# AIM-SE/AC-TSR

Measured on AMD Instinct MI355X. Metric: user-sequences/sec fwd+bwd, AC-SASRec L=50 d=64, 1/2/4/8 MI355X, higher is better.
Workload: dtype f32; 1 GPU; ACSASRec full training step (spatial + adversarial calibrators, BASELINE configs[2]), synthetic 100000-item catalogue, B=512/GPU L=50 d=64 h=2 2 layers inner=256, CE loss, two-pass backward + Adam; global_batch=512, seq_len=50, hidden=64, heads=2, parallelism=dp1, launch=hipGraph replay per step, backward=two walks (reference protocol, trainer.py:672-686)

## Files before the change

### ac_tsr_amd/_lib.py

```python
from __future__ import annotations

import ctypes as C
import os
import subprocess

_HERE = os.path.dirname(os.path.abspath(__file__))
CSRC = os.path.join(_HERE, "csrc")
LIB_PATH = os.environ.get("ACATTN_LIB") or os.path.join(CSRC, "libacattn.so")
HEADER_PATH = os.path.join(os.path.dirname(_HERE), "include", "acattn.h")

ABI_VERSION = 32
MAX_MASKS = 8
NSTAT = 8
MASK_STRUCTURED, MASK_DENSE_LL, MASK_DENSE_L = 0, 1, 2
COMBINE = {"fixed": 0, "gate": 1, "annealing": 2}
RICH = {"none": 0, "fixed": 1, "trainable": 2}
RNG_EXPLICIT, RNG_COUNTER = 0, 1
FWD_AUTO, FWD_STREAM, FWD_STAGED, FWD_GENERAL = 0, 1, 2, 3
BWD_AUTO, BWD_STREAM, BWD_ROW = 0, 1, 2

_f = C.c_void_p


class Problem(C.Structure):
    _fields_ = [
        ("B", C.c_int32), ("L", C.c_int32), ("H", C.c_int32), ("n_heads", C.c_int32),
        ("q", _f), ("k", _f), ("v", _f), ("qa", _f), ("ka", _f), ("gate_logits", _f),
        ("mask_mode", C.c_int32), ("causal", C.c_int32), ("key_valid", _f), ("mask", _f),
        ("w_order", _f), ("b_order", _f), ("w_dist", _f), ("b_dist", _f), ("scalar", _f),
        ("adversarial", C.c_int32), ("combine_option", C.c_int32), ("anneal_rate", C.c_float),
        ("two_level", C.c_int32), ("rich_combine", C.c_int32), ("rich_ratio", _f),
        ("rng_mode", C.c_int32), ("p_drop", C.c_float), ("noise", _f), ("keep_after", _f), ("keep_before", _f),
        ("keep_mask", _f), ("seed", C.c_uint64), ("seed_device", _f), ("affine", _f), ("gate_is_prob", C.c_int32),
    ]


class FwdOut(C.Structure):
    _fields_ = [
        ("ctx_attacked", _f), ("ctx_calibrated", _f), ("attack_mask", _f), ("row_stats", _f),
        ("after_spatial", _f), ("before_spatial", _f), ("perturbed_attention", _f), ("calibrated_attention", _f),
        ("penalty_part", _f),
    ]


class BwdIO(C.Structure):
    _fields_ = [
        ("attack_mask", _f), ("row_stats", _f),
        ("d_ctx_attacked", _f), ("d_ctx_calibrated", _f), ("d_attack_mask", _f),
        ("dq", _f), ("dk", _f), ("dv", _f), ("dqa", _f), ("dka", _f), ("dgate_logits", _f),
        ("dw_order_part", _f), ("dw_dist_part", _f), ("dsmall_part", _f), ("part_stride", C.c_int32),
        ("active_qblocks", _f), ("attack_only", C.c_int32), ("workspace", _f), ("read_rows", _f),
        ("n_read_rows", C.c_int32), ("d_penalty_part", _f), ("dgate_summed", C.c_int32),
        ("d_ctx_calibrated2", _f), ("d_penalty_part2", _f), ("dqa2", _f), ("dka2", _f),
    ]


class SpatialBwdIO(C.Structure):
    _fields_ = [
        ("d_ctx", _f), ("dq", _f), ("dk", _f), ("dv", _f),
        ("dw_order_part", _f), ("dw_dist_part", _f), ("dsmall_part", _f), ("part_stride", C.c_int32),
        ("n_read_rows", C.c_int32), ("read_rows", _f), ("workspace", _f),
    ]


class CeProblem(C.Structure):
    _fields_ = [("B", C.c_int32), ("N", C.c_int32), ("H", C.c_int32), ("out", _f), ("table", _f), ("target", _f),
                ("coef_is_scalar", C.c_int32), ("coef_scale", C.c_float)]


class LnProblem(C.Structure):
    _fields_ = [("rows", C.c_int32), ("H", C.c_int32), ("residual_rows", C.c_int32), ("z", _f), ("residual", _f),
                ("gamma", _f), ("beta", _f), ("eps", C.c_float), ("p_drop", C.c_float), ("keep", _f),
                ("seed", C.c_uint64), ("seed_device", _f)]


LN_BWD_GRID = 512


class ProjProblem(C.Structure):
    _fields_ = [("rows", C.c_int32), ("H", C.c_int32), ("G", C.c_int32), ("x", _f), ("wq", _f), ("bq", _f), ("wk", _f),
                ("bk", _f), ("wv", _f), ("bv", _f), ("waq", _f), ("baq", _f), ("wak", _f), ("bak", _f), ("wg", _f),
                ("bg", _f), ("w_order", _f), ("b_order", _f), ("w_dist", _f), ("b_dist", _f), ("n_heads", C.c_int32),
                ("L", C.c_int32)]


class ProjOut(C.Structure):
    _fields_ = [("mq", _f), ("mk", _f), ("mv", _f), ("qa", _f), ("ka", _f), ("gate", _f), ("affine", _f),
                ("gate_prob", C.c_int32)]


class ProjBwdIO(C.Structure):
    _fields_ = [("dmq", _f), ("dmk", _f), ("dmv", _f), ("dqa", _f), ("dka", _f), ("dgate", _f), ("dmq_total", _f),
                ("dmk_total", _f), ("dx", _f), ("dx_init", _f), ("workspace", _f)]


ADAM_MAX_TENSORS = 64


class AdamGroup(C.Structure):
    _fields_ = [("n_tensors", C.c_int32), ("param", _f * ADAM_MAX_TENSORS), ("grad", _f * ADAM_MAX_TENSORS),
                ("exp_avg", _f * ADAM_MAX_TENSORS), ("exp_avg_sq", _f * ADAM_MAX_TENSORS), ("step", _f * ADAM_MAX_TENSORS),
                ("numel", C.c_int64 * ADAM_MAX_TENSORS)]


class TailProblem(C.Structure):
    _fields_ = [("rows", C.c_int32), ("H", C.c_int32), ("I", C.c_int32), ("ctx", _f), ("x", _f), ("wd", _f), ("bd", _f),
                ("g1", _f), ("b1", _f), ("w1", _f), ("bb1", _f), ("w2", _f), ("bb2", _f), ("g2", _f), ("b2", _f),
                ("eps1", C.c_float), ("eps2", C.c_float), ("p1", C.c_float), ("p2", C.c_float), ("keep1", _f),
                ("keep2", _f), ("seed1", C.c_uint64), ("seed2", C.c_uint64), ("seed_device", _f), ("src_index", _f),
                ("src_R", C.c_int32), ("src_L", C.c_int32), ("split_planes", _f)]


class TailSaved(C.Structure):
    _fields_ = [("h1", _f), ("st1", _f), ("a", _f), ("act", _f), ("h3", _f), ("st2", _f), ("out", _f),
                ("gelu_grad", _f)]


class TailBwdIO(C.Structure):
    _fields_ = [("d_out", _f), ("d_ctx", _f), ("d_x", _f), ("d_h1", _f), ("d_h2", _f), ("d_h3", _f), ("dgb_part", _f),
                ("workspace", _f)]


class EmbedProblem(C.Structure):
    _fields_ = [("rows", C.c_int32), ("L", C.c_int32), ("H", C.c_int32), ("n_table_rows", C.c_int64), ("idx", _f),
                ("table", _f), ("pos", _f), ("gamma", _f), ("beta", _f), ("eps", C.c_float), ("p_drop", C.c_float),
                ("keep", _f), ("seed", C.c_uint64), ("seed_device", _f), ("nonzero_out", _f), ("hot_id_plus1", C.c_int64)]


EMBED_BWD_CHUNKS = 8
PENALTY_WS_FLOATS = 1024
WGRAD_MAX_GROUP = 8
WGRAD_MAX_REDUCE = 32
SUMROWS_MAX_DEFER = 8

SYMBOLS = {
    "acattn_abi_version": (C.c_int, []),
    "acattn_calibrated_attention_bwd_gate_summed": (C.c_int, [C.POINTER(Problem), C.POINTER(BwdIO)]),
    "acattn_calibrated_attention_bwd_pair_supported": (C.c_int, [C.POINTER(Problem), C.POINTER(BwdIO)]),
    "acattn_last_error": (C.c_char_p, []),
    "acattn_fwd_algorithmic_bytes": (C.c_int64, [C.POINTER(Problem)]),
    "acattn_calibrated_attention_fwd": (C.c_int, [C.POINTER(Problem), C.POINTER(FwdOut), C.c_void_p]),
    "acattn_calibrated_attention_bwd": (C.c_int, [C.POINTER(Problem), C.POINTER(BwdIO), C.c_void_p]),
    "acattn_spatial_attention_bwd": (C.c_int, [C.POINTER(Problem), C.POINTER(SpatialBwdIO), C.c_void_p]),
    "acattn_spatial_attention_bwd_workspace_bytes": (C.c_int64, [C.POINTER(Problem)]),
    "acattn_spatial_affines": (C.c_int, [C.POINTER(Problem), _f, C.c_void_p]),
    "acattn_full_sort_ce_workspace_bytes": (C.c_int64, [C.POINTER(CeProblem)]),
    "acattn_full_sort_ce_fwd": (C.c_int, [C.POINTER(CeProblem), _f, _f, _f, C.c_void_p]),
    "acattn_full_sort_ce_fwd_dir": (C.c_int, [C.POINTER(CeProblem), _f, _f, _f, _f, C.c_void_p]),
    "acattn_full_sort_ce_bwd": (C.c_int, [C.POINTER(CeProblem), _f, _f, _f, _f, _f, C.c_void_p]),
    "acattn_full_sort_ce_products": (C.c_int, [C.c_int]),
    "acattn_linear_products": (C.c_int, [C.c_int]),
    "acattn_dropout_add_layernorm_fwd": (C.c_int, [C.POINTER(LnProblem), _f, _f, C.c_void_p]),
    "acattn_dropout_add_layernorm_bwd": (C.c_int, [C.POINTER(LnProblem), _f, _f, _f, _f, _f, C.c_void_p]),
    "acattn_embed_layernorm_fwd": (C.c_int, [C.POINTER(EmbedProblem), _f, _f, C.c_void_p]),
    "acattn_embed_layernorm_bwd": (C.c_int, [C.POINTER(EmbedProblem), _f, _f, C.c_int64, _f, _f, _f, C.c_void_p]),
    "acattn_projections_supported": (C.c_int, [C.c_int32, C.c_int32]),
    "acattn_projections_bwd_workspace_bytes": (C.c_int64, [C.POINTER(ProjProblem)]),
    "acattn_projections_fwd": (C.c_int, [C.POINTER(ProjProblem), C.POINTER(ProjOut), C.c_void_p]),
    "acattn_projections_qkv_supported": (C.c_int, [C.c_int32]),
    "acattn_projections_qkv_fwd": (C.c_int, [C.POINTER(ProjProblem), C.POINTER(ProjOut), C.c_void_p]),
    "acattn_projections_bwd": (C.c_int, [C.POINTER(ProjProblem), C.POINTER(ProjBwdIO), C.c_void_p]),
    "acattn_layer_tail_supported": (C.c_int, [C.c_int32, C.c_int32]),
    "acattn_layer_tail_fwd": (C.c_int, [C.POINTER(TailProblem), C.POINTER(TailSaved), C.c_void_p]),
    "acattn_layer_tail_bwd": (C.c_int, [C.POINTER(TailProblem), C.POINTER(TailSaved), C.POINTER(TailBwdIO), C.c_void_p]),
    "acattn_layer_tail_bwd_partial_rows": (C.c_int32, [C.c_int32]),
    "acattn_layer_tail_bwd_partial_rows_for": (C.c_int32, [C.c_int32, C.c_int32]),
    "acattn_layer_tail_bwd_workspace_bytes": (C.c_int64, [C.c_int32, C.c_int32]),
    "acattn_select_layer_tail_blocks": (C.c_int, [C.c_int]),
    "acattn_layer_tail_split_bytes": (C.c_int64, [C.c_int32, C.c_int32, C.c_int32]),
    "acattn_layer_tail_split_weights": (C.c_int, [C.POINTER(TailProblem), C.c_void_p, C.c_void_p]),
    "acattn_adam_step": (C.c_int, [C.POINTER(AdamGroup), C.c_double, C.c_double, C.c_double, C.c_double, C.c_double, _f,
                                   C.c_void_p]),
    "acattn_dense_ce_fwd": (C.c_int, [_f, C.c_int64, C.c_int64, _f, _f, _f, C.c_void_p]),
    "acattn_dense_ce_bwd": (C.c_int, [_f, _f, _f, _f, C.c_int64, C.c_int64, _f, C.c_void_p]),
    "acattn_step_inputs": (C.c_int, [C.POINTER(C.c_void_p), C.POINTER(C.c_void_p), C.POINTER(C.c_int64), C.c_int32, C.c_void_p,
                                     C.c_void_p, C.c_void_p, C.c_int32, C.c_void_p]),
    "acattn_sum_rows": (C.c_int, [_f, _f, C.c_int32, C.c_int32, C.c_int32, C.c_void_p]),
    "acattn_sum_rows_pair": (C.c_int, [_f, _f, C.c_int32, C.c_int32, C.c_int32, _f, _f, C.c_int32, C.c_int32, C.c_int32, C.c_void_p]),
    "acattn_mask_penalty_fwd": (C.c_int, [_f, C.c_int64, _f, _f, C.c_void_p]),
    "acattn_mask_penalty_partial": (C.c_int, [_f, C.c_int64, _f, C.c_void_p]),
    "acattn_mask_penalty_partial_multi": (C.c_int, [C.c_void_p, C.c_int32, C.c_int64, _f, C.c_void_p]),
    "acattn_mask_penalty_bwd_scaled_multi": (C.c_int, [C.c_void_p, _f, _f, C.c_float, C.c_int64, C.c_void_p, C.c_int32,
                                                       C.c_void_p]),
    "acattn_attacked_loss_finish": (C.c_int, [_f, C.c_int32, _f, C.c_int32, C.c_int64, C.c_float, _f, _f, C.c_int32,
                                              C.c_void_p]),
    "acattn_mask_penalty_rows": (C.c_int, [_f, C.c_int32, C.c_int32, C.c_int32, _f, C.c_void_p]),
    "acattn_attacked_loss_finish_rows": (C.c_int, [_f, C.c_int32, C.c_void_p, C.c_int32, C.c_int32, C.c_float, _f, _f, C.c_int32,
                                                  C.c_void_p]),
    "acattn_mask_penalty_drows": (C.c_int, [_f, _f, C.c_float, C.c_int32, C.c_void_p, C.c_int32, C.c_void_p]),
    "acattn_mask_penalty_drows_dir": (C.c_int, [_f, _f, C.c_float, C.c_int32, C.c_void_p, C.c_int32, _f, _f, C.c_int32, C.c_void_p]),
    "acattn_mask_penalty_bwd_scaled": (C.c_int, [_f, _f, _f, C.c_float, C.c_int64, _f, C.c_void_p]),
    "acattn_mask_penalty_bwd": (C.c_int, [_f, _f, _f, C.c_int64, _f, C.c_void_p]),
    "acattn_linear_wgrad_workspace_bytes": (C.c_int64, [C.c_int64, C.c_int32, C.c_int32]),
    "acattn_linear_wgrad_grouped": (C.c_int, [C.c_void_p, C.c_void_p, C.c_void_p, C.c_void_p, C.c_void_p, C.c_void_p,
                                               C.c_int32, C.c_int64, _f, C.c_void_p]),
    "acattn_linear_wgrad": (C.c_int, [_f, _f, C.c_int64, C.c_int32, C.c_int32, _f, _f, _f, C.c_void_p]),
    "acattn_linear_wgrad_grouped_partial": (C.c_int, [C.c_void_p, C.c_void_p, C.c_void_p, C.c_void_p, C.c_void_p, C.c_int32,
                                                       C.c_int64, C.c_void_p, C.c_void_p, C.c_void_p, C.c_void_p, C.c_void_p]),
    "acattn_linear_wgrad_reduce_many": (C.c_int, [C.c_void_p, C.c_void_p, C.c_void_p, C.c_void_p, C.c_void_p, C.c_void_p,
                                                   C.c_void_p, C.c_int32, C.c_void_p, C.c_void_p, C.c_void_p, C.c_void_p,
                                                   C.c_int32, C.c_void_p]),
    "acattn_select_forward_kernel": (C.c_int, [C.c_int]),
    "acattn_select_backward_kernel": (C.c_int, [C.c_int]),
    "acattn_calibrated_attention_bwd_workspace_bytes": (C.c_int64, [C.POINTER(Problem)]),
    "acattn_rng_materialize": (C.c_int, [C.c_int32, C.c_int32, C.c_int32, C.c_uint64, C.c_float, _f, _f, _f, _f,
                                         C.c_void_p]),
}

_lib = None


class AcattnError(RuntimeError):
    pass


def build(verbose: bool = False) -> str:
    jobs = str(min(8, os.cpu_count() or 1))
    res = subprocess.run(["make", "-C", CSRC, "-j", jobs], capture_output=not verbose, text=True)
    if res.returncode != 0:
        raise AcattnError("building libacattn.so failed:\n" + (res.stdout or "") + (res.stderr or ""))
    return LIB_PATH


def load() -> C.CDLL:
    global _lib
    if _lib is not None:
        return _lib
    if not os.path.exists(LIB_PATH):
        raise AcattnError(
            f"{LIB_PATH} is missing: the HIP extension has not been built. Run "
            "`make -C ac_tsr_amd/csrc` (or __graft_entry__.build()). There is no CPU / eager fallback.")
    lib = C.CDLL(LIB_PATH)
    for name, (res, args) in SYMBOLS.items():
        fn = getattr(lib, name)
        fn.restype = res
        fn.argtypes = args
    got = lib.acattn_abi_version()
    if got != ABI_VERSION:
        raise AcattnError(f"libacattn.so ABI {got} != binding ABI {ABI_VERSION}; rebuild")
    _lib = lib
    return lib


def check(rc: int, what: str) -> None:
    if rc == 0:
        return
    msg = load().acattn_last_error().decode()
    if rc < 0 and "not a multiple of the number of attention" in msg:
        raise ValueError(msg)
    if rc < 0 and ("unknown combine_option" in msg or "unknown rich_calibrated_combine" in msg):
        raise KeyError(msg)
    raise AcattnError(f"{what} failed (rc={rc}): {msg}")
```

### ac_tsr_amd/csrc/acattn_api.hip

```cpp
#include <stdint.h>
#include <stdio.h>
#include <string.h>

#include <algorithm>

#include "acattn_common.h"

namespace {
thread_local char g_err[256] = "";

int fail(const char* msg) {
  snprintf(g_err, sizeof(g_err), "%s", msg);
  return -1;
}

int check_problem(const acattn_problem* p) {
  if (!p) return fail("problem is NULL");
  if (p->B < 1 || p->L < 1 || p->H < 1 || p->n_heads < 1) return fail("B, L, H, n_heads must be positive");
  if (p->H % p->n_heads != 0)
    return fail("The hidden size is not a multiple of the number of attention heads");
  const int dh = p->H / p->n_heads;
  if (dh != 16 && dh != 32 && dh != 64 && dh != 128) return fail("unsupported head size: dh must be 16, 32, 64 or 128");
  if (p->L > 208) return fail("unsupported sequence length: L must be <= 208");
  if (!p->q || !p->k || !p->v) return fail("q, k, v must be non-NULL");
// ... 133 lines not shown
                                   (hipStream_t)stream);
  if (rc > 0) snprintf(g_err, sizeof(g_err), "HIP launch failed: %s", hipGetErrorString((hipError_t)rc));
  return rc;
}

static int check_ce(const acattn_ce_problem* p) {
  if (!p) return fail("ce problem is NULL");
  if (p->B < 1 || p->N < 1) return fail("B and N must be positive");
  if (p->H != 64 && p->H != 128 && p->H != 256) return fail("unsupported hidden size for the fused cross-entropy: H must be 64, 128 or 256");
  if (!p->out || !p->table || !p->target) return fail("out, table, target must be non-NULL");
  return 0;
}

int64_t acattn_full_sort_ce_workspace_bytes(const acattn_ce_problem* p) {
  if (!p || (p->H != 64 && p->H != 128 && p->H != 256)) return -1;
  return acattn_ce_ws_bytes(*p);
}

int acattn_full_sort_ce_fwd(const acattn_ce_problem* p, void* workspace, float* lse, float* row_loss, void* stream) {
  if (int rc = check_ce(p)) return rc;
  if (!workspace || !lse || !row_loss) return fail("workspace, lse, row_loss must be non-NULL");
  const int rc = acattn_launch_ce_fwd(*p, workspace, lse, row_loss, (hipStream_t)stream);
  if (rc > 0) snprintf(g_err, sizeof(g_err), "HIP launch failed: %s", hipGetErrorString((hipError_t)rc));
  return rc;
}

int acattn_full_sort_ce_fwd_dir(const acattn_ce_problem* p, void* workspace, float* lse, float* row_loss, float* dir,
                                void* stream) {
  if (int rc = check_ce(p)) return rc;
  if (!workspace || !lse || !row_loss || !dir) return fail("workspace, lse, row_loss, dir must be non-NULL");
  const int rc = acattn_launch_ce_fwd_dir(*p, workspace, lse, row_loss, dir, (hipStream_t)stream);
  if (rc > 0) snprintf(g_err, sizeof(g_err), "HIP launch failed: %s", hipGetErrorString((hipError_t)rc));
  return rc;
}

int acattn_full_sort_ce_bwd(const acattn_ce_problem* p, const float* lse, const float* coef, void* workspace,
                            float* d_out, float* d_table, void* stream) {
  if (int rc = check_ce(p)) return rc;
  if (!workspace || !lse || !coef || !d_out) return fail("workspace, lse, coef, d_out must be non-NULL");
  const int rc = acattn_launch_ce_bwd(*p, lse, coef, workspace, d_out, d_table, (hipStream_t)stream);
  if (rc > 0) snprintf(g_err, sizeof(g_err), "HIP launch failed: %s", hipGetErrorString((hipError_t)rc));
  return rc;
}

int acattn_full_sort_ce_products(int mode) { return acattn_ce_products_choice(mode); }

int acattn_linear_products(int mode) { return acattn_linear_products_choice(mode); }

static int check_ln(const acattn_ln_problem* p) {
  if (!p) return fail("ln problem is NULL");
  if (p->rows < 1) return fail("rows must be positive");
  if (p->H != 64 && p->H != 128 && p->H != 256) return fail("unsupported hidden size for the fused LayerNorm: H must be 64, 128 or 256");
  if (p->residual_rows < 1 || p->rows % p->residual_rows != 0) return fail("residual_rows must divide rows");
  if (!p->z || !p->residual || !p->gamma || !p->beta) return fail("z, residual, gamma, beta must be non-NULL");
  if (p->p_drop < 0.f || p->p_drop >= 1.f) return fail("p_drop must lie in [0, 1)");
  return 0;
}

int acattn_dropout_add_layernorm_fwd(const acattn_ln_problem* p, float* y, float* stats, void* stream) {
  if (int rc = check_ln(p)) return rc;
  if (!y || !stats) return fail("y and stats must be non-NULL");
  const int rc = acattn_launch_ln_fwd(*p, y, stats, (hipStream_t)stream);
  if (rc > 0) snprintf(g_err, sizeof(g_err), "HIP launch failed: %s", hipGetErrorString((hipError_t)rc));
  return rc;
}

int acattn_dropout_add_layernorm_bwd(const acattn_ln_problem* p, const float* dy, const float* stats, float* dz,
                                     float* dres, float* dgb_part, void* stream) {
  if (int rc = check_ln(p)) return rc;
  if (!dy || !stats) return fail("dy and stats must be non-NULL");
  const int rc = acattn_launch_ln_bwd(*p, dy, stats, dz, dres, dgb_part, (hipStream_t)stream);
  if (rc > 0) snprintf(g_err, sizeof(g_err), "HIP launch failed: %s", hipGetErrorString((hipError_t)rc));
  return rc;
}

static int check_proj(const acattn_proj_problem* p) {
  if (!p) return fail("problem must be non-NULL");
  if (p->rows < 1) return fail("rows must be positive");
  if (!acattn_proj_supported(p->H, p->G)) return fail("projections: hidden_size must be 64, 128 or 256 and the gate at most 256 wide");
  if (!p->x || !p->wq || !p->bq || !p->wk || !p->bk || !p->wv || !p->bv || !p->waq || !p->baq || !p->wak || !p->bak)
    return fail("projections: input and parameters must be non-NULL");
  if ((p->wg != nullptr) != (p->bg != nullptr) || (p->wg != nullptr) != (p->G > 0))
    return fail("projections: gate weight, bias and width go together");
  return 0;
}

int acattn_projections_supported(int32_t H, int32_t G) { return acattn_proj_supported(H, G) ? 1 : 0; }

int64_t acattn_projections_bwd_workspace_bytes(const acattn_proj_problem* p) {
  if (!p || !acattn_proj_supported(p->H, p->G)) return -1;
  return acattn_proj_bwd_ws_bytes(*p);
}

int acattn_projections_fwd(const acattn_proj_problem* p, const acattn_proj_out* out, void* stream) {
  if (int rc = check_proj(p)) return rc;
  if (!out || !out->mq || !out->mk || !out->mv || !out->qa || !out->ka) return fail("projections: outputs must be non-NULL");
  if ((p->wg != nullptr) != (out->gate != nullptr)) return fail("projections: gate output goes with the gate parameters");
  if (out->affine) {
    if (!p->w_order || !p->b_order || !p->w_dist || !p->b_dist) return fail("projections: affine planes need the spatial calibrator's parameters");
    if (p->n_heads < 1 || p->H % p->n_heads != 0 || (p->H / p->n_heads) % 16 != 0) return fail("projections: affine planes need a head size that is a multiple of 16");
    if (p->L < 1 || p->rows % p->L != 0) return fail("projections: affine planes need rows = B * L");
  }
  const int rc = acattn_launch_proj_fwd(*p, *out, (hipStream_t)stream);
  if (rc > 0) snprintf(g_err, sizeof(g_err), "HIP launch failed: %s", hipGetErrorString((hipError_t)rc));
  return rc;
}

int acattn_projections_qkv_supported(int32_t H) { return acattn_proj_qkv_supported(H) ? 1 : 0; }

int acattn_projections_qkv_fwd(const acattn_proj_problem* p, const acattn_proj_out* out, void* stream) {
  if (!p) return fail("problem must be non-NULL");
  if (p->rows < 1) return fail("rows must be positive");
  if (!acattn_proj_qkv_supported(p->H)) return fail("projections (q, k, v only): hidden_size must be 64 with the split products on");
  if (!p->x || !p->wq || !p->bq || !p->wk || !p->bk || !p->wv || !p->bv) return fail("projections: input and parameters must be non-NULL");
  if (!out || !out->mq || !out->mk || !out->mv) return fail("projections: outputs must be non-NULL");
  if (out->qa || out->ka || out->gate) return fail("projections (q, k, v only): qa, ka and gate outputs must be NULL");
  if (out->affine) {
    if (!p->w_order || !p->b_order || !p->w_dist || !p->b_dist) return fail("projections: affine planes need the spatial calibrator's parameters");
    if (p->n_heads < 1 || p->H % p->n_heads != 0 || (p->H / p->n_heads) % 16 != 0) return fail("projections: affine planes need a head size that is a multiple of 16");
    if (p->L < 1 || p->rows % p->L != 0) return fail("projections: affine planes need rows = B * L");
  }
  const int rc = acattn_launch_proj_qkv_fwd(*p, *out, (hipStream_t)stream);
  if (rc > 0) snprintf(g_err, sizeof(g_err), "HIP launch failed: %s", hipGetErrorString((hipError_t)rc));
  return rc;
}

int acattn_projections_bwd(const acattn_proj_problem* p, const acattn_proj_bwd_io* io, void* stream) {
  if (int rc = check_proj(p)) return rc;
  if (!io) return fail("io must be non-NULL");
  if (!io->dmq_total && !io->dmk_total && !io->dx) return fail("projections backward: nothing to compute");
  const int rc = acattn_launch_proj_bwd(*p, *io, (hipStream_t)stream);
  if (rc > 0) snprintf(g_err, sizeof(g_err), "HIP launch failed: %s", hipGetErrorString((hipError_t)rc));
  return rc;
}

static int check_tail(const acattn_tail_problem* p, const acattn_tail_saved* s) {
  if (!p || !s) return fail("problem and saved must be non-NULL");
  if (p->rows < 1) return fail("rows must be positive");
  if (!acattn_tail_supported(p->H, p->I)) return fail("layer tail: (hidden_size, inner_size) must be (64, 256), (64, 128), (128, 512), (128, 256) or (256, 1024)");
  if (!p->ctx || !p->x || !p->wd || !p->bd || !p->g1 || !p->b1 || !p->w1 || !p->bb1 || !p->w2 || !p->bb2 || !p->g2 || !p->b2)
    return fail("layer tail: inputs and parameters must be non-NULL");
  if (!(p->p1 >= 0.f && p->p1 < 1.f) || !(p->p2 >= 0.f && p->p2 < 1.f)) return fail("dropout probabilities must be in [0, 1)");
  if (!s->h1 || !s->st1 || !s->a || !s->h3 || !s->st2) return fail("layer tail: saved tensors must be non-NULL");
  if (p->src_index && (p->src_R < 1 || p->src_L < 1)) return fail("layer tail: src_index needs src_R, src_L >= 1");
  if (p->split_planes && p->H != 64) return fail("layer tail: split_planes is for hidden 64 only");
  if (((uintptr_t)p->split_planes & 15) != 0) return fail("layer tail: split_planes must be 16-byte aligned");
  return 0;
}

int acattn_layer_tail_supported(int32_t H, int32_t I) { return acattn_tail_supported(H, I) ? 1 : 0; }

int32_t acattn_layer_tail_bwd_partial_rows(int32_t rows) { return acattn_tail_bwd_partial_rows(rows); }
int32_t acattn_layer_tail_bwd_partial_rows_for(int32_t rows, int32_t H) { return acattn_tail_bwd_partial_rows_h(rows, H); }
int64_t acattn_layer_tail_bwd_workspace_bytes(int32_t H, int32_t I) {
  return acattn_tail_supported(H, I) ? acattn_tail_bwd_ws_bytes(H, I) : -1;
}

int64_t acattn_layer_tail_split_bytes(int32_t H, int32_t I, int32_t rows) {
  return acattn_tail_supported(H, I) && rows > 0 ? acattn_tail_split_bytes(H, I, rows) : 0;
}

int acattn_layer_tail_split_weights(const acattn_tail_problem* p, void* planes, void* stream) {
  if (!p || !planes || !p->wd || !p->w1 || !p->w2) return fail("layer tail split planes: problem, weights and planes must be non-NULL");
  if (p->H != 64 || (p->I != 256 && p->I != 128)) return fail("layer tail split planes: hidden 64, inner 256 or 128 only");
  if (((uintptr_t)planes & 15) != 0) return fail("layer tail split planes: planes must be 16-byte aligned");
  const int rc = acattn_launch_tail_split(*p, planes, (hipStream_t)stream);
  if (rc > 0) snprintf(g_err, sizeof(g_err), "HIP launch failed: %s", hipGetErrorString((hipError_t)rc));
  return rc;
}

int acattn_select_layer_tail_blocks(int nb) {
  if (nb < 0 || nb > 2) return fail("rows per wave: 0 (automatic), 1 or 2 blocks of 16");
  return acattn_select_tail_nb(nb);
}

int acattn_layer_tail_fwd(const acattn_tail_problem* p, const acattn_tail_saved* saved, void* stream) {
  if (int rc = check_tail(p, saved)) return rc;
  if (!saved->act || !saved->out) return fail("layer tail forward: act and out must be non-NULL");
  const int rc = acattn_launch_tail_fwd(*p, *saved, (hipStream_t)stream);
  if (rc > 0) snprintf(g_err, sizeof(g_err), "HIP launch failed: %s", hipGetErrorString((hipError_t)rc));
  return rc;
}

int acattn_layer_tail_bwd(const acattn_tail_problem* p, const acattn_tail_saved* saved, const acattn_tail_bwd_io* io,
                          void* stream) {
  if (int rc = check_tail(p, saved)) return rc;
  if (!io || !io->d_out) return fail("layer tail backward: d_out must be non-NULL");
  const int rc = acattn_launch_tail_bwd(*p, *saved, *io, (hipStream_t)stream);
  if (rc > 0) snprintf(g_err, sizeof(g_err), "HIP launch failed: %s", hipGetErrorString((hipError_t)rc));
  return rc;
}

int acattn_dense_ce_fwd(const float* logits, int64_t rows, int64_t N, const int64_t* target, float* lse, float* row_loss,
                        void* stream) {
  if (!logits || !target || !lse || !row_loss) return fail("dense CE: logits, target, lse, row_loss must be non-NULL");
  if (rows < 1 || N < 1) return fail("dense CE: rows and N must be positive");
  const int rc = acattn_launch_dense_ce_fwd(logits, rows, N, target, lse, row_loss, (hipStream_t)stream);
  if (rc > 0) snprintf(g_err, sizeof(g_err), "HIP launch failed: %s", hipGetErrorString((hipError_t)rc));
  return rc;
}
int acattn_dense_ce_bwd(const float* logits, const float* lse, const int64_t* target, const float* coef, int64_t rows, int64_t N,
                        float* d_logits, void* stream) {
  if (!logits || !lse || !target || !coef || !d_logits) return fail("dense CE backward: every pointer must be non-NULL");
  if (rows < 1 || N < 1) return fail("dense CE: rows and N must be positive");
  const int rc = acattn_launch_dense_ce_bwd(logits, lse, target, coef, rows, N, d_logits, (hipStream_t)stream);
  if (rc > 0) snprintf(g_err, sizeof(g_err), "HIP launch failed: %s", hipGetErrorString((hipError_t)rc));
  return rc;
}

int acattn_step_inputs(const void* const* src, void* const* dst, const int64_t* bytes, int32_t n_copies, int64_t* counter,
                       const int64_t* item_length, int64_t* last_row, int32_t n_rows, void* stream) {
  if (n_copies < 0 || n_copies > ACATTN_MAX_COPIES) return fail("step inputs: 0 .. ACATTN_MAX_COPIES copies");
  if (n_copies > 0 && (!src || !dst || !bytes)) return fail("step inputs: src, dst, bytes must be non-NULL");
  for (int k = 0; k < n_copies; ++k)
    if (bytes[k] > 0 && (!src[k] || !dst[k])) return fail("step inputs: NULL copy operand");
  if ((item_length == nullptr) != (last_row == nullptr)) return fail("step inputs: item_length and last_row come together");
  if (last_row && n_rows < 1) return fail("step inputs: n_rows must be positive");
  const int rc = acattn_launch_step_inputs(src, dst, bytes, n_copies, counter, item_length, last_row, n_rows, (hipStream_t)stream);
  if (rc > 0) snprintf(g_err, sizeof(g_err), "HIP launch failed: %s", hipGetErrorString((hipError_t)rc));
  return rc;
}

int acattn_sum_rows(const float* x, float* out, int32_t batch, int32_t R, int32_t C, void* stream) {
  if (!x || !out) return fail("x and out must be non-NULL");
  if (batch < 1 || R < 1 || C < 1) return fail("batch, R, C must be positive");
  const int rc = acattn_launch_sum_rows(x, out, batch, R, C, (hipStream_t)stream);
  if (rc > 0) snprintf(g_err, sizeof(g_err), "HIP launch failed: %s", hipGetErrorString((hipError_t)rc));
  return rc;
}

int acattn_sum_rows_pair(const float* x1, float* out1, int32_t batch1, int32_t R1, int32_t C1, const float* x2, float* out2,
                         int32_t batch2, int32_t R2, int32_t C2, void* stream) {
  if (!x1 || !out1 || !x2 || !out2) return fail("x and out must be non-NULL");
  if (batch1 < 1 || R1 < 1 || C1 < 1 || batch2 < 1 || R2 < 1 || C2 < 1) return fail("batch, R, C must be positive");
  const int rc = acattn_launch_sum_rows_pair(x1, out1, batch1, R1, C1, x2, out2, batch2, R2, C2, (hipStream_t)stream);
  if (rc > 0) snprintf(g_err, sizeof(g_err), "HIP launch failed: %s", hipGetErrorString((hipError_t)rc));
  return rc;
}

static int check_embed(const acattn_embed_problem* p) {
  if (!p) return fail("embed problem is NULL");
  if (p->rows < 1 || p->L < 1 || p->rows % p->L != 0) return fail("rows must be a positive multiple of L");
  if (p->H != 64 && p->H != 128 && p->H != 256) return fail("unsupported hidden size for the fused embedding front end: H must be 64, 128 or 256");
  if (p->n_table_rows < 1) return fail("n_table_rows must be positive");
  if (!p->idx || !p->table || !p->gamma || !p->beta) return fail("idx, table, gamma, beta must be non-NULL");
  if (p->p_drop < 0.f || p->p_drop >= 1.f) return fail("p_drop must lie in [0, 1)");
  return 0;
}

int acattn_embed_layernorm_fwd(const acattn_embed_problem* p, float* y, float* stats, void* stream) {
  if (const int rc = check_embed(p)) return rc;
  if (!y || !stats) return fail("y and stats must be non-NULL");
  const int rc = acattn_launch_embed_fwd(*p, y, stats, (hipStream_t)stream);
  if (rc > 0) snprintf(g_err, sizeof(g_err), "HIP launch failed: %s", hipGetErrorString((hipError_t)rc));
  return rc;
}

int acattn_embed_layernorm_bwd(const acattn_embed_problem* p, const float* dy, const float* stats, int64_t padding_idx,
                               float* d_table, float* d_pos_part, float* dgb_part, void* stream) {
  if (const int rc = check_embed(p)) return rc;
  if (!dy || !stats) return fail("dy and stats must be non-NULL");
  const int rc = acattn_launch_embed_bwd(*p, dy, stats, padding_idx, d_table, d_pos_part, dgb_part, (hipStream_t)stream);
  if (rc > 0) snprintf(g_err, sizeof(g_err), "HIP launch failed: %s", hipGetErrorString((hipError_t)rc));
  return rc;
}

int acattn_mask_penalty_fwd(const float* m, int64_t n, float* workspace, float* norm, void* stream) {
  if (!m || !workspace || !norm) return fail("m, workspace and norm must be non-NULL");
  if (n < 1) return fail("n must be positive");
  if (((uintptr_t)m & 15) != 0) return fail("m must be 16-byte aligned");
  const int rc = acattn_launch_penalty_fwd(m, n, workspace, norm, (hipStream_t)stream);
  if (rc > 0) snprintf(g_err, sizeof(g_err), "HIP launch failed: %s", hipGetErrorString((hipError_t)rc));
  return rc;
}

int acattn_mask_penalty_bwd(const float* m, const float* norm, const float* d_norm, int64_t n, float* d_m, void* stream) {
  if (!m || !norm || !d_norm || !d_m) return fail("m, norm, d_norm and d_m must be non-NULL");
  if (n < 1) return fail("n must be positive");
  if ((((uintptr_t)m | (uintptr_t)d_m) & 15) != 0) return fail("m and d_m must be 16-byte aligned");
  const int rc = acattn_launch_penalty_bwd(m, norm, d_norm, n, d_m, (hipStream_t)stream);
  if (rc > 0) snprintf(g_err, sizeof(g_err), "HIP launch failed: %s", hipGetErrorString((hipError_t)rc));
  return rc;
}

int acattn_mask_penalty_partial(const float* m, int64_t n, float* part, void* stream) {
  if (!m || !part) return fail("m and part must be non-NULL");
  if (n < 1) return fail("n must be positive");
  if (((uintptr_t)m & 15) != 0) return fail("m must be 16-byte aligned");
  const int rc = acattn_launch_penalty_partial(m, n, part, (hipStream_t)stream);
  if (rc > 0) snprintf(g_err, sizeof(g_err), "HIP launch failed: %s", hipGetErrorString((hipError_t)rc));
  return rc;
}

int acattn_attacked_loss_finish(const float* row_loss, int32_t B, const float* part, int32_t n_masks, int64_t mask_numel,
                                float weight, float* out, float* scale_buf, int32_t n_scale, void* stream) {
  if (!row_loss || !part || !out) return fail("row_loss, part and out must be non-NULL");
  if (B < 1 || n_masks < 1 || mask_numel < 1) return fail("B, n_masks and mask_numel must be positive");
  if (n_scale < 0 || (n_scale > 0 && !scale_buf)) return fail("scale_buf must be given with n_scale > 0");
  const int rc = acattn_launch_attacked_loss_finish(row_loss, B, part, n_masks, mask_numel, weight, out, scale_buf, n_scale,
                                                    (hipStream_t)stream);
  if (rc > 0) snprintf(g_err, sizeof(g_err), "HIP launch failed: %s", hipGetErrorString((hipError_t)rc));
  return rc;
}

int acattn_mask_penalty_rows(const float* m, int32_t B, int32_t n_heads, int32_t L, float* pen, void* stream) {
  if (!m || !pen) return fail("m and pen must be non-NULL");
// ... 172 lines not shown
```

### ac_tsr_amd/csrc/acattn_bwd_stream.hip

```cpp
#include <stdlib.h>

#include <algorithm>

#include "acattn_common.h"

namespace {

constexpr float kLog2e = 1.44269504088896340736f;
constexpr float kLn2 = 0.69314718055994530942f;

__device__ __forceinline__ float ex2(float x) { return __builtin_amdgcn_exp2f(x); }
__device__ __forceinline__ float and_bits(float x, int m) { return __uint_as_float(__float_as_uint(x) & (uint32_t)m); }
__device__ __forceinline__ float hsum(const f4 v) { return (v[0] + v[1]) + (v[2] + v[3]); }
__device__ __forceinline__ float row16_sum(float v) {
  v += __builtin_bit_cast(float, __builtin_amdgcn_update_dpp(0, __builtin_bit_cast(int, v), 0xB1, 0xF, 0xF, false));
  v += __builtin_bit_cast(float, __builtin_amdgcn_update_dpp(0, __builtin_bit_cast(int, v), 0x4E, 0xF, 0xF, false));
  v += __builtin_bit_cast(float, __builtin_amdgcn_update_dpp(0, __builtin_bit_cast(int, v), 0x141, 0xF, 0xF, false));
  v += __builtin_bit_cast(float, __builtin_amdgcn_update_dpp(0, __builtin_bit_cast(int, v), 0x140, 0xF, 0xF, false));
  return v;
}

#ifndef ACATTN_BWD_ONE_WAVE_DH
#define ACATTN_BWD_ONE_WAVE_DH 64
#endif
// ... 692 lines not shown
      load_mask_row<DH>(P, IO, F, rowbase, bh, hoff, qb, c, g, R);
      float qac[4][DT];
      col_frag<DH>(P.qa, rowbase, H, hoff, i0, L, c, g, qac);
      const float sM = ws[(bh * L + (R.row_ok ? R.i : 0)) * NSC + 4];
      const uint32_t prow = prow_base + (uint32_t)(R.row_ok ? R.i : 0) * (uint32_t)L;
      const int j0 = 16 * t + 4 * g;
      f4 aM = {0.f, 0.f, 0.f, 0.f};
#pragma unroll
      for (int s4 = 0; s4 < KS / 4; ++s4)
#pragma unroll
        for (int e = 0; e < 4; ++e) aM = mfma16(ka4[s4][e], R.qaf[4 * s4 + e], aM);
      uint32_t eb4, ab4;
      tile_bits(F, t, g, R.i, L, causal, R.row_ok, R.dead, eb4, ab4);
      const f4 dMext = IO.d_attack_mask ? load_seg(IO.d_attack_mask + prow, j0, L, R.row_ok) : f4{0.f, 0.f, 0.f, 0.f};
      const float dpen2 = IO.d_penalty_part ? 2.0f * IO.d_penalty_part[(size_t)bh * nT + qb] : 0.f;
      f4 Mt, dM;
      mask_tile(R, K, aM, t, g, eb4, dMext, dpen2, Mt, dM);
      const f4 dSa = (Mt * (dM - sM)) * K.inv_sqrt;
      asm volatile("s_waitcnt lgkmcnt(0)" ::: "memory");
      *(f4*)(&tr[1][c * TS + 4 * g]) = dSa;
      asm volatile("s_waitcnt lgkmcnt(0)" ::: "memory");
#pragma unroll
      for (int s = 0; s < 4; ++s) {
        const float b_sa = tr[1][(4 * g + s) * TS + c];
#pragma unroll
        for (int dt = 0; dt < DT; ++dt) aKa[dt] = mfma16(qac[s][dt], b_sa, aKa[dt]);
      }
      continue;
    }
#endif
    Row<DH> R;
    load_row<DH>(P, IO, F, rowbase, bh, hoff, qb, c, g, R);
    const bool order_select = !causal || __ballot(R.dead) != 0ull;
    const float* wrow = ws + (bh * L + (R.row_ok ? R.i : 0)) * NSC;
    const f4 w0 = *(const f4*)wrow;
    const float sM = wrow[4];
    const uint32_t prow = prow_base + (uint32_t)(R.row_ok ? R.i : 0) * (uint32_t)L;
    const int j0 = 16 * t + 4 * g;
    const f4 gl = load_seg(P.gate_logits + (rowbase + (R.row_ok ? R.i : 0)) * L, j0, L, R.row_ok);
    f4 dMout = IO.d_attack_mask ? load_seg(IO.d_attack_mask + prow, j0, L, R.row_ok) : f4{0.f, 0.f, 0.f, 0.f};
    uint32_t eb4, ab4;
    tile_bits(F, t, g, R.i, L, causal, R.row_ok, R.dead, eb4, ab4);
    Tile T;
    tile_forward<DH, DCA, TWO>(R, K, k4, ka4, v4, co4, cd4, gl, t, g, eb4, ab4, order_select, T);
    if (IO.d_penalty_part) dMout += (T.M - 1.0f) * (2.0f * IO.d_penalty_part[(size_t)bh * nT + qb]);
    f4 dS, dSa, dgl, d_o, d_d;
    float dsc;
    tile_backward<DCA>(T, K, w0[0], w0[1], w0[2], w0[3], sM, dMout, R.i, j0, dS, dSa, dgl, d_o, d_d, dsc);
    dco += d_o;
    dcd += d_d;
    asm volatile("s_waitcnt lgkmcnt(0)" ::: "memory");
    *(f4*)(&tr[0][c * TS + 4 * g]) = dS;
    *(f4*)(&tr[1][c * TS + 4 * g]) = dSa;
    if constexpr (DCA) *(f4*)(&tr[2][c * TS + 4 * g]) = T.Ap;
    if constexpr (TWO && !DCA) {
      const float dpen2_2 = IO.d_penalty_part2 ? 2.0f * IO.d_penalty_part2[(size_t)bh * nT + qb] : 0.f;
      *(f4*)(&tr[2][c * TS + 4 * g]) = second_set_dsa(T, K, wrow[5], wrow[6], wrow[7], (T.M - 1.0f) * dpen2_2);
    }
    *(f4*)(&tr[3][c * TS + 4 * g]) = T.Aw;
    float qc[4][DT], qac[4][DT], gac[4][DT], gcc[4][DT];
    if (full) col_frag<DH>(P.q, rowbase, H, hoff, i0, L, c, g, qc);
    col_frag<DH>(P.qa, rowbase, H, hoff, i0, L, c, g, qac);
    if constexpr (DCA)
      if (full) col_frag<DH>(IO.d_ctx_attacked, rowbase, H, hoff, i0, L, c, g, gac);
    if (full) col_frag<DH>(IO.d_ctx_calibrated, rowbase, H, hoff, i0, L, c, g, gcc);
    asm volatile("s_waitcnt lgkmcnt(0)" ::: "memory");
#pragma unroll
    for (int s = 0; s < 4; ++s) {
      const float b_s = tr[0][(4 * g + s) * TS + c], b_sa = tr[1][(4 * g + s) * TS + c];
      const float b_aw = tr[3][(4 * g + s) * TS + c];
      float b_ap = 0.f;
      if constexpr (DCA) b_ap = tr[2][(4 * g + s) * TS + c];
#pragma unroll
      for (int dt = 0; dt < DT; ++dt) {
        if (full) {
          aK[dt] = mfma16(qc[s][dt], b_s, aK[dt]);
          if constexpr (DCA) aV[dt] = mfma16(gac[s][dt], b_ap, aV[dt]);
          aV[dt] = mfma16(gcc[s][dt], b_aw, aV[dt]);
        }
        aKa[dt] = mfma16(qac[s][dt], b_sa, aKa[dt]);
        if constexpr (TWO && !DCA) aKa2[dt] = mfma16(qac[s][dt], tr[2][(4 * g + s) * TS + c], aKa2[dt]);
      }
    }
  }

  asm volatile("s_waitcnt lgkmcnt(0)" ::: "memory");
#pragma unroll
  for (int r = 0; r < 4; ++r) {
    const float so = row16_sum(dco[r]), sd = row16_sum(dcd[r]);
    if (c == 0) {
      tr[0][4 * g + r] = so;
      tr[1][4 * g + r] = sd;
    }
  }
  asm volatile("s_waitcnt lgkmcnt(0)" ::: "memory");
  const float dco_c = tr[0][c], dcd_c = tr[1][c];
  const int key = 16 * t + c;
  if (key < L) {
    const size_t o = (rowbase + key) * H + hoff + 4 * g;
#pragma unroll
    for (int dt = 0; dt < DT; ++dt) {
      *(f4*)(IO.dka + o + 16 * dt) = aKa[dt];
      if constexpr (TWO) *(f4*)(IO.dka2 + o + 16 * dt) = aKa2[dt];
      if (full) {
        const f4 wo_hi = *(const f4*)(P.w_order + DH + 16 * dt + 4 * g), wd_hi = *(const f4*)(P.w_dist + DH + 16 * dt + 4 * g);
        *(f4*)(IO.dk + o + 16 * dt) = aK[dt] + dco_c * wo_hi + dcd_c * wd_hi;
        *(f4*)(IO.dv + o + 16 * dt) = aV[dt];
      }
    }
  }
  if (!full) return;
  const int stride_w = IO.part_stride ? IO.part_stride : 2 * DH;
  const float okk = key < L ? 1.0f : 0.0f;
#pragma unroll
  for (int s4 = 0; s4 < KS / 4; ++s4)
#pragma unroll
    for (int e = 0; e < 4; ++e) {
      const float vo = row16_sum(dco_c * k4[s4][e] * okk), vd = row16_sum(dcd_c * k4[s4][e] * okk);
      if (c == 0) {
        atomicAdd(IO.dw_order_part + bh * stride_w + DH + KS * g + 4 * s4 + e, vo);
        atomicAdd(IO.dw_dist_part + bh * stride_w + DH + KS * g + 4 * s4 + e, vd);
      }
    }
}

struct RowScalars {
  float ao2, ad, lx2, ly2, lu2, lv2, lw2;
  int i;
  uint32_t rng_row;
};

__device__ __forceinline__ float wave_sum(float v) {
  v = row16_sum(v);
  v += __shfl_xor(v, 16);
  v += __shfl_xor(v, 32);
  return v;
}

#ifdef ACATTN_ONEROW_STAMPS
__device__ unsigned long long g_onerow_stamps[2048 * 8];
#define OR_STAMP(k)                                                                \
  do {                                                                             \
    __builtin_amdgcn_sched_barrier(0);                                             \
    unsigned long long now_;                                                       \
    asm volatile("s_waitcnt vmcnt(0) lgkmcnt(0)\n\ts_memtime %0\n\ts_waitcnt lgkmcnt(0)" : "=s"(now_)::"memory"); \
    if ((k) >= 0) cyc_[(k) >= 0 ? (k) : 0] += now_ - last_;                        \
    last_ = now_;                                                                  \
    __builtin_amdgcn_sched_barrier(0);                                             \
  } while (0)
#else
#define OR_STAMP(k)
#endif

template <int DH, bool ACC, bool SLICED>
__global__ void __launch_bounds__(64) acattn_bwd_onerow_kernel(const acattn_problem P, const acattn_bwd_io IO) {
#ifdef ACATTN_ONEROW_STAMPS
  unsigned long long cyc_[8] = {}, last_ = 0;
#endif
  OR_STAMP(-1);
  constexpr int D4 = DH / 4;
  __shared__ __attribute__((aligned(16))) float vec[8][DH];
  __shared__ __attribute__((aligned(16))) float col[4][256];
  const int L = P.L, H = P.H, nh = P.n_heads;
  const int nT = (L + 15) >> 4;
  const bool causal = P.causal != 0;
  int b, h;
  decode_block(blockIdx.x, P.B, nh, b, h);
  const int lane = threadIdx.x;
  const size_t rowbase = (size_t)b * L, bh = (size_t)b * nh + h;
  const int hoff = h * DH;
  const int i = min(max((int)IO.read_rows[b], 0), L - 1);
  const KeyFlags F = load_key_flags(P.key_valid, rowbase, L, nT, lane);
  const Consts K = make_consts(P, DH);

  for (int d = lane; d < DH; d += 64) {
    const size_t o = (rowbase + i) * H + hoff + d;
    vec[0][d] = P.q[o];
    vec[1][d] = P.qa[o];
    vec[2][d] = IO.d_ctx_attacked ? IO.d_ctx_attacked[o] : 0.f;
    vec[3][d] = IO.d_ctx_calibrated ? IO.d_ctx_calibrated[o] : 0.f;
    vec[4][d] = P.w_order[DH + d] * -kLog2e;
    vec[5][d] = P.w_dist[DH + d];
    vec[6][d] = P.w_order[d];
    vec[7][d] = P.w_dist[d];
  }
  __syncthreads();
  OR_STAMP(0);
  RowScalars R;
  {
    float ao = 0.f, adv = 0.f;
#pragma unroll
    for (int d = 0; d < DH; ++d) {
      ao += vec[0][d] * vec[6][d];
      adv += vec[0][d] * vec[7][d];
    }
    R.ao2 = -kLog2e * (ao + P.b_order[0]);
    R.ad = adv + P.b_dist[0];
  }
  const bool dead = causal ? F.first_valid > i : !F.any_valid;
  {
    const float sh = dead ? ACATTN_MASK_FILL : 0.f;
    const float* sp = IO.row_stats + (bh * L + i) * ACATTN_NSTAT;
    R.lx2 = (sp[0] - sh) * kLog2e;
    R.ly2 = (sp[1] - sh) * kLog2e;
    R.lu2 = (sp[2] - sh) * kLog2e;
    R.lv2 = (sp[3] - sh) * kLog2e;
    R.lw2 = (sp[4] - sh) * kLog2e;
  }
  R.i = i;
  R.rng_row = (uint32_t)(bh * L + i);
  const bool order_select = !causal || dead;

  constexpr bool sliced = SLICED;
  constexpr int N4 = SLICED ? D4 / 4 : D4;
  const int kgrp = sliced ? (lane & 15) : lane;
  const int slice = sliced ? (lane >> 4) : 0;
  const int d_lo = slice * N4;
  const float lead = slice == 0 ? 1.0f : 0.0f;
  const int t = kgrp >> 2, g = kgrp & 3, j0 = 4 * kgrp;
  f4 aS = {0.f, 0.f, 0.f, 0.f}, aM = aS, aP = aS, aW = aS, co4 = aS, cd4 = aS;
  if constexpr (SLICED) {
#pragma unroll
    for (int r = 0; r < 4; ++r) {
      const size_t o = (rowbase + min(j0 + r, L - 1)) * H + hoff;
#pragma unroll
      for (int k4 = 0; k4 < N4; ++k4) {
        const int d4 = d_lo + k4;
        const f4 kv = *(const f4*)(P.k + o + 4 * d4), kav = *(const f4*)(P.ka + o + 4 * d4), vv = *(const f4*)(P.v + o + 4 * d4);
        const f4 q4 = *(const f4*)(&vec[0][4 * d4]), qa4 = *(const f4*)(&vec[1][4 * d4]);
        const f4 ga4 = *(const f4*)(&vec[2][4 * d4]), gc4 = *(const f4*)(&vec[3][4 * d4]);
        const f4 wo4 = *(const f4*)(&vec[4][4 * d4]), wd4 = *(const f4*)(&vec[5][4 * d4]);
        aS[r] += hsum(kv * q4);
        aM[r] += hsum(kav * qa4);
        aP[r] += hsum(vv * ga4);
        aW[r] += hsum(vv * gc4);
        co4[r] += hsum(kv * wo4);
        cd4[r] += hsum(kv * wd4);
      }
    }
  } else {
    size_t o4[4];
#pragma unroll
    for (int r = 0; r < 4; ++r) o4[r] = (rowbase + min(j0 + r, L - 1)) * H + hoff;
#pragma unroll 2
    for (int k4 = 0; k4 < N4; ++k4) {
      const f4 q4 = *(const f4*)(&vec[0][4 * k4]), qa4 = *(const f4*)(&vec[1][4 * k4]);
      const f4 ga4 = *(const f4*)(&vec[2][4 * k4]), gc4 = *(const f4*)(&vec[3][4 * k4]);
      const f4 wo4 = *(const f4*)(&vec[4][4 * k4]), wd4 = *(const f4*)(&vec[5][4 * k4]);
      f4 kv[4], kav[4], vv[4];
#pragma unroll
      for (int r = 0; r < 4; ++r) {
        kv[r] = *(const f4*)(P.k + o4[r] + 4 * k4);
        kav[r] = *(const f4*)(P.ka + o4[r] + 4 * k4);
        vv[r] = *(const f4*)(P.v + o4[r] + 4 * k4);
      }
#pragma unroll
      for (int r = 0; r < 4; ++r) {
        aS[r] += hsum(kv[r] * q4);
        aM[r] += hsum(kav[r] * qa4);
        aP[r] += hsum(vv[r] * ga4);
        aW[r] += hsum(vv[r] * gc4);
        co4[r] += hsum(kv[r] * wo4);
        cd4[r] += hsum(kv[r] * wd4);
      }
    }
    __builtin_amdgcn_sched_barrier(0);
  }
  if (sliced) {
#pragma unroll
    for (int r = 0; r < 4; ++r) {
      aS[r] = quad_sum(aS[r]);
      aM[r] = quad_sum(aM[r]);
      aP[r] = quad_sum(aP[r]);
      aW[r] = quad_sum(aW[r]);
      co4[r] = quad_sum(co4[r]);
      cd4[r] = quad_sum(cd4[r]);
    }
  }
  OR_STAMP(1);
  const f4 gl = load_seg(P.gate_logits + (rowbase + i) * L, j0, L, true);
  uint32_t eb4, ab4;
  tile_bits(F, t, g, i, L, causal, true, dead, eb4, ab4);
  if (j0 >= 16 * nT) eb4 = 0u;
  Tile T;
  tile_elementwise(R, K, aS, aM, aP, aW, co4, cd4, gl, t, g, eb4, ab4, order_select, T);

  const float da = wave_sum(lead * hsum(T.Ap * T.dAp)), dc = wave_sum(lead * hsum(T.Aw * T.dAw));
  const f4 dw = T.Aw * (T.dAw - dc);
  const f4 dac = (1.0f - T.gt) * dw;
  const float r1 = wave_sum(lead * hsum(T.Ac * dac));
  const f4 du = T.Ap * (T.dAp - da), dv = T.Ac * (dac - r1);
  f4 dP = T.gt * dw + dv * T.ex1 + du * T.M;
  f4 dM = du * (T.P - T.nz) - dv * (T.P * T.ex1);
#pragma unroll
  for (int r = 0; r < 4; ++r) {
    dP[r] = keep_and(dP[r] * K.keep_scale, T.ka, r);
    dM[r] = keep_and(dM[r] * K.keep_scale, T.km, r);
  }
  const float sP = wave_sum(lead * hsum(T.Pt * dP)), sM = wave_sum(lead * hsum(T.Mt * dM));
  f4 dS, dSa, dgl, d_o, d_d;
  float dsc;
  tile_backward(T, K, da, dc, r1, sP, sM, f4{0.f, 0.f, 0.f, 0.f}, i, j0, dS, dSa, dgl, d_o, d_d, dsc);
  const float da_o = wave_sum(lead * hsum(d_o)), da_d = wave_sum(lead * hsum(d_d)), dsc_sum = wave_sum(lead * dsc);
  if (slice == 0) {
    *(f4*)(&col[0][j0]) = dS;
    *(f4*)(&col[1][j0]) = dSa;
    *(f4*)(&col[2][j0]) = d_o;
    *(f4*)(&col[3][j0]) = d_d;
  }

  OR_STAMP(2);
  if constexpr (SLICED) {
#pragma unroll
    for (int r = 0; r < 4; ++r) {
      const int j = j0 + r;
      if (j < L) {
        const size_t o = (rowbase + j) * H + hoff;
#pragma unroll
        for (int k4 = 0; k4 < N4; ++k4) {
          const int d4 = d_lo + k4;
          const f4 q4 = *(const f4*)(&vec[0][4 * d4]), qa4 = *(const f4*)(&vec[1][4 * d4]);
          const f4 ga4 = *(const f4*)(&vec[2][4 * d4]), gc4 = *(const f4*)(&vec[3][4 * d4]);
          const f4 wo_hi = *(const f4*)(P.w_order + DH + 4 * d4), wd_hi = *(const f4*)(P.w_dist + DH + 4 * d4);
          *(f4*)(IO.dk + o + 4 * d4) = q4 * dS[r] + wo_hi * d_o[r] + wd_hi * d_d[r];
          if (ACC)
            *(f4*)(IO.dka + o + 4 * d4) += qa4 * dSa[r];
          else
            *(f4*)(IO.dka + o + 4 * d4) = qa4 * dSa[r];
          *(f4*)(IO.dv + o + 4 * d4) = ga4 * T.Ap[r] + gc4 * T.Aw[r];
        }
      }
    }
  } else {
#pragma unroll 2
    for (int k4 = 0; k4 < N4; ++k4) {
      const f4 q4 = *(const f4*)(&vec[0][4 * k4]), qa4 = *(const f4*)(&vec[1][4 * k4]);
      const f4 ga4 = *(const f4*)(&vec[2][4 * k4]), gc4 = *(const f4*)(&vec[3][4 * k4]);
      const f4 wo_hi = *(const f4*)(P.w_order + DH + 4 * k4), wd_hi = *(const f4*)(P.w_dist + DH + 4 * k4);
#pragma unroll
      for (int r = 0; r < 4; ++r) {
        const int j = j0 + r;
        if (j < L) {
          const size_t o = (rowbase + j) * H + hoff;
          *(f4*)(IO.dk + o + 4 * k4) = q4 * dS[r] + wo_hi * d_o[r] + wd_hi * d_d[r];
          if (ACC)
            *(f4*)(IO.dka + o + 4 * k4) += qa4 * dSa[r];
          else
            *(f4*)(IO.dka + o + 4 * k4) = qa4 * dSa[r];
          *(f4*)(IO.dv + o + 4 * k4) = ga4 * T.Ap[r] + gc4 * T.Aw[r];
        }
      }
    }
    __builtin_amdgcn_sched_barrier(0);
  }
  OR_STAMP(3);
  if (IO.dgate_logits && IO.dgate_summed) {
    if (slice == 0) {
      float* grow = IO.dgate_logits + ((size_t)b * L + i) * L;
#pragma unroll
      for (int r = 0; r < 4; ++r)
        if (j0 + r < L) atomicAdd(grow + j0 + r, dgl[r]);
    }
  } else if (IO.dgate_logits) {
    float* gbase = IO.dgate_logits + bh * (size_t)L * L;
    for (int row = 0; row < L; ++row) {
      if (row == i) continue;
      for (int j = lane; j < L; j += 64) gbase[(size_t)row * L + j] = 0.f;
    }
    if (slice == 0) store_seg(gbase + (size_t)i * L, j0, L, true, dgl);
  }
  __syncthreads();
  OR_STAMP(4);

  const int stride_w = IO.part_stride ? IO.part_stride : 2 * DH, stride_s = IO.part_stride ? IO.part_stride : 4;
  constexpr int PARTS = DH <= 32 ? 64 / DH : 1;
  constexpr int NCH = DH > 64 ? DH / 64 : 1;
#pragma unroll 1
  for (int ch = 0; ch < NCH; ++ch) {
    const int d = (DH > 64 ? lane : lane % DH) + 64 * ch, part = DH > 64 ? 0 : lane / DH;
    float sq = 0.f, sqa = 0.f, so = 0.f, sd = 0.f;
    constexpr int UJ = 8;
    for (int jb = part; jb < L; jb += PARTS * UJ) {
      float kv[UJ], kav[UJ];
#pragma unroll
      for (int u = 0; u < UJ; ++u) {
        const int j = min(jb + u * PARTS, L - 1);
        const size_t o = (rowbase + j) * H + hoff + d;
        kv[u] = P.k[o];
        kav[u] = P.ka[o];
      }
#pragma unroll
      for (int u = 0; u < UJ; ++u) {
        const int j = jb + u * PARTS;
        const float w = j < L ? 1.0f : 0.0f;
        const int jc = min(j, L - 1);
        sq += w * col[0][jc] * kv[u];
        sqa += w * col[1][jc] * kav[u];
        so += w * col[2][jc] * kv[u];
        sd += w * col[3][jc] * kv[u];
      }
    }
#pragma unroll
    for (int off = DH; off < 64; off <<= 1) {
      sq += __shfl_xor(sq, off);
      sqa += __shfl_xor(sqa, off);
      so += __shfl_xor(so, off);
      sd += __shfl_xor(sd, off);
    }
    if (ch == 0) {
      constexpr int LPR = DH / 4, RPI = 64 / LPR;
      const f4 z4 = {0.f, 0.f, 0.f, 0.f};
      for (int row = lane / LPR; row < L; row += RPI) {
        if (row == i) continue;
        const size_t o = (rowbase + row) * H + hoff + 4 * (lane % LPR);
        *(f4*)(IO.dq + o) = z4;
        if (!ACC) *(f4*)(IO.dqa + o) = z4;
      }
    }
    if (part == 0) {
      const size_t o = (rowbase + i) * H + hoff + d;
      IO.dq[o] = sq + da_o * vec[6][d] + da_d * vec[7][d];
      if (ACC) IO.dqa[o] += sqa;
      else IO.dqa[o] = sqa;
    }
    if (part != 0) continue;
    IO.dw_order_part[bh * stride_w + d] = da_o * vec[0][d];
    IO.dw_dist_part[bh * stride_w + d] = da_d * vec[0][d];
    IO.dw_order_part[bh * stride_w + DH + d] = so;
    IO.dw_dist_part[bh * stride_w + DH + d] = sd;
  }
  if (lane == 0) {
    float* sm = IO.dsmall_part + bh * stride_s;
    sm[0] = da_o;
    sm[1] = da_d;
    sm[2] = dsc_sum;
    sm[3] = 0.f;
  }
  OR_STAMP(5);
#ifdef ACATTN_ONEROW_STAMPS
  if (lane == 0 && blockIdx.x < 2048)
    for (int k = 0; k < 8; ++k) g_onerow_stamps[blockIdx.x * 8 + k] = cyc_[k];
#endif
}

#ifdef ACATTN_ONEROW_STAMPS
extern "C" int acattn_debug_onerow_stamps(unsigned long long* host, int n_words) {
  return (int)hipMemcpyFromSymbol(host, HIP_SYMBOL(g_onerow_stamps), (size_t)n_words * 8);
}
#endif

template <int DH>
int launch_onerow(const acattn_problem& p, const acattn_bwd_io& io, bool accumulate, hipStream_t stream) {
  const dim3 grid(p.B * p.n_heads), block(64);
  if (io.dgate_logits && io.dgate_summed) {
    const int rc = acattn_launch_zero(io.dgate_logits, (size_t)p.B * p.L * p.L, stream);
    if (rc) return rc;
  }
  if (p.L <= 64) {
    if (accumulate)
      hipLaunchKernelGGL((acattn_bwd_onerow_kernel<DH, true, true>), grid, block, 0, stream, p, io);
    else
      hipLaunchKernelGGL((acattn_bwd_onerow_kernel<DH, false, true>), grid, block, 0, stream, p, io);
  } else if (accumulate) {
    hipLaunchKernelGGL((acattn_bwd_onerow_kernel<DH, true, false>), grid, block, 0, stream, p, io);
  } else {
    hipLaunchKernelGGL((acattn_bwd_onerow_kernel<DH, false, false>), grid, block, 0, stream, p, io);
  }
  return (int)hipGetLastError();
}

template <int DH>
int launch_stream(const acattn_problem& p, const acattn_bwd_io& io, float* ws, hipStream_t stream) {
  const int nT = (p.L + 15) / 16, dh = DH;
  const size_t rows = (size_t)p.B * p.n_heads;
  if (!io.attack_only) {
    int rc = 0;
    auto zero = [&](float* ptr, size_t n) { if (!rc) rc = acattn_launch_zero(ptr, n, stream); };
    if (io.part_stride) {
      float* lo = std::min(io.dw_order_part, std::min(io.dw_dist_part, io.dsmall_part));
      zero(lo, rows * io.part_stride);
    } else {
      zero(io.dw_order_part, rows * 2 * dh);
      zero(io.dw_dist_part, rows * 2 * dh);
      zero(io.dsmall_part, rows * 4);
    }
    if (rc) return rc;
  }
  const dim3 grid(p.B * p.n_heads * nT), block(64);
  static const bool no_dca_form = getenv("ACATTN_BWD_DCA_ALWAYS") ? atoi(getenv("ACATTN_BWD_DCA_ALWAYS")) == 0 : true;
  if (io.d_ctx_attacked || !no_dca_form) {
    hipLaunchKernelGGL((acattn_bwd_row_kernel<DH, true>), grid, block, 0, stream, p, io, ws);
    hipLaunchKernelGGL((acattn_bwd_key_kernel<DH, true>), grid, block, 0, stream, p, io, (const float*)ws);
  } else if (io.dqa2) {
    hipLaunchKernelGGL((acattn_bwd_row_kernel<DH, false, true>), grid, block, 0, stream, p, io, ws);
    hipLaunchKernelGGL((acattn_bwd_key_kernel<DH, false, true>), grid, block, 0, stream, p, io, (const float*)ws);
  } else {
    hipLaunchKernelGGL((acattn_bwd_row_kernel<DH, false>), grid, block, 0, stream, p, io, ws);
    hipLaunchKernelGGL((acattn_bwd_key_kernel<DH, false>), grid, block, 0, stream, p, io, (const float*)ws);
  }
  return (int)hipGetLastError();
}

}

int64_t acattn_bwd_stream_ws_bytes(const acattn_problem& p) { return (int64_t)p.B * p.n_heads * p.L * NSC * sizeof(float); }

bool acattn_bwd_onerow_applies(const acattn_problem& p, const acattn_bwd_io& io) {
  static const bool enabled = getenv("ACATTN_ONEROW") ? atoi(getenv("ACATTN_ONEROW")) != 0 : true;
  const int dh = p.n_heads > 0 ? p.H / p.n_heads : 0;
  return enabled && io.read_rows && io.n_read_rows == 1 && !io.active_qblocks && !io.d_attack_mask && !io.d_penalty_part && !io.attack_only &&
         p.L <= 208 && (int64_t)p.B * p.n_heads * p.L * p.L < (1LL << 30) && (int64_t)p.B * p.L * p.H < (1LL << 30) &&
         p.mask_mode == ACATTN_MASK_STRUCTURED && p.rng_mode == ACATTN_RNG_COUNTER && p.w_order && p.w_dist &&
         p.adversarial && p.combine_option == ACATTN_COMBINE_GATE && p.two_level && (dh == 16 || dh == 32 || dh == 64 || dh == 128);
}

int acattn_launch_bwd_onerow(const acattn_problem& p, const acattn_bwd_io& io, bool accumulate, hipStream_t stream) {
  if (!acattn_bwd_onerow_applies(p, io)) return -100;
  switch (p.H / p.n_heads) {
    case 16: return launch_onerow<16>(p, io, accumulate, stream);
    case 32: return launch_onerow<32>(p, io, accumulate, stream);
    case 64: return launch_onerow<64>(p, io, accumulate, stream);
    case 128: return launch_onerow<128>(p, io, accumulate, stream);
  }
  return -100;
}

bool acattn_bwd_stream_pair_applies(const acattn_problem& p, const acattn_bwd_io& io) {
  const int dh = p.n_heads > 0 ? p.H / p.n_heads : 0;
  return io.workspace && p.L <= 208 && (int64_t)p.B * p.n_heads * p.L * p.L < (1LL << 30) && (int64_t)p.B * p.L * p.H < (1LL << 30) &&
         p.mask_mode == ACATTN_MASK_STRUCTURED && p.rng_mode == ACATTN_RNG_COUNTER && p.w_order && p.w_dist && p.adversarial &&
         p.combine_option == ACATTN_COMBINE_GATE && p.two_level && (dh == 16 || dh == 32 || dh == 64) && !io.d_ctx_attacked &&
         !io.attack_only && !io.read_rows && !io.active_qblocks && io.dqa2 && io.dka2 &&
         (io.d_ctx_calibrated2 || io.d_penalty_part2);
}

int acattn_launch_bwd_stream(const acattn_problem& p, const acattn_bwd_io& io, hipStream_t stream) {
  const bool ok = io.workspace && p.L <= 208 && (int64_t)p.B * p.n_heads * p.L * p.L < (1LL << 30) &&
                  (int64_t)p.B * p.L * p.H < (1LL << 30) && p.mask_mode == ACATTN_MASK_STRUCTURED &&
                  p.rng_mode == ACATTN_RNG_COUNTER && p.w_order && p.w_dist && p.adversarial &&
                  p.combine_option == ACATTN_COMBINE_GATE && p.two_level;
  if (!ok) return -100;
  float* ws = (float*)io.workspace;
  switch (p.H / p.n_heads) {
    case 16: return launch_stream<16>(p, io, ws, stream);
    case 32: return launch_stream<32>(p, io, ws, stream);
    case 64: return launch_stream<64>(p, io, ws, stream);
    case 128: return launch_stream<128>(p, io, ws, stream);
  }
  return -100;
}
```

### ac_tsr_amd/csrc/acattn_common.h

```cpp
#pragma once
#include <hip/hip_runtime.h>
#include <stdint.h>

#include <type_traits>

#include "acattn.h"

typedef float f4 __attribute__((ext_vector_type(4)));
typedef float f4u __attribute__((ext_vector_type(4), aligned(4)));

#define ACATTN_NEG_INF (-__builtin_inff())
#define ACATTN_MASK_FILL (-10000.0f)
#define ACATTN_LOG_EPS (1e-24f)

__device__ __forceinline__ float quad_sum(float x) {
  auto r = __builtin_amdgcn_permlane16_swap(__float_as_uint(x), __float_as_uint(x), false, false);
  x = __uint_as_float(r[0]) + __uint_as_float(r[1]);
  auto s = __builtin_amdgcn_permlane32_swap(__float_as_uint(x), __float_as_uint(x), false, false);
  return __uint_as_float(s[0]) + __uint_as_float(s[1]);
}

__device__ __forceinline__ float quad_max(float x) {
  auto r = __builtin_amdgcn_permlane16_swap(__float_as_uint(x), __float_as_uint(x), false, false);
  x = fmaxf(__uint_as_float(r[0]), __uint_as_float(r[1]));
// ... 113 lines not shown
}

__device__ __forceinline__ RngGroup rng_group_half(const RngKey key, uint32_t row_id, uint32_t grp) {
  uint32_t x = (row_id * 64u + grp) ^ key.a;
  x *= 0x7feb352dU;
  x ^= x >> 15;
  x *= 0x846ca68bU;
  x ^= x >> 16;
  x += key.b;
  const uint32_t wn[2] = {x, rng_word(x, 0x68E31DA4u, 0x9E3779B1u)};
  RngGroup o;
#pragma unroll
  for (int pair = 0; pair < 2; ++pair) {
    const float u1 = fmaf((float)(wn[pair] >> 16), 1.0f / 65536.0f, 0.5f / 65536.0f);
    const float u2 = (float)(wn[pair] & 0xFFFFu) * (1.0f / 65536.0f);
    const float rad = __builtin_amdgcn_sqrtf(__builtin_amdgcn_logf(u1) * (-2.0f * 0.69314718055994530942f));
    o.n[2 * pair] = rad * __builtin_amdgcn_cosf(u2);
    o.n[2 * pair + 1] = rad * __builtin_amdgcn_sinf(u2);
  }
  const uint32_t w2 = rng_word(x, 0xB5297A4Du, 0x85EBCA77u);
  o.keep_after = (w2 >> 4) & 0xFu;
  o.keep_mask = (w2 >> 12) & 0xFu;
  o.keep_before = (w2 >> 20) & 0xFu;
  return o;
}

typedef float acattn_f2 __attribute__((ext_vector_type(2)));
struct RngDraw {
  acattn_f2 n01, n23;
  uint32_t keep_after, keep_mask, keep_before;
};
__device__ __forceinline__ RngDraw rng_draw_half(const RngKey key, uint32_t row_id, uint32_t grp, float scale) {
  uint32_t x = (row_id * 64u + grp) ^ key.a;
  x *= 0x7feb352dU;
  x ^= x >> 15;
  x *= 0x846ca68bU;
  x ^= x >> 16;
  x += key.b;
  const uint32_t wn[2] = {x, rng_word(x, 0x68E31DA4u, 0x9E3779B1u)};
  RngDraw o;
  acattn_f2 n[2];
#pragma unroll
  for (int pair = 0; pair < 2; ++pair) {
    const float u1 = fmaf((float)(wn[pair] >> 16), 1.0f / 65536.0f, 0.5f / 65536.0f);
    const float u2 = (float)(wn[pair] & 0xFFFFu) * (1.0f / 65536.0f);
    const float rad = __builtin_amdgcn_sqrtf(__builtin_amdgcn_logf(u1) * (-2.0f * 0.69314718055994530942f)) * scale;
    acattn_f2 cs = {__builtin_amdgcn_cosf(u2), __builtin_amdgcn_sinf(u2)};
    asm("" : "+v"(cs));
    n[pair] = cs * rad;
  }
  o.n01 = n[0];
  o.n23 = n[1];
  const uint32_t w2 = rng_word(x, 0xB5297A4Du, 0x85EBCA77u);
  o.keep_after = (w2 >> 4) & 0xFu;
  o.keep_mask = (w2 >> 12) & 0xFu;
  o.keep_before = (w2 >> 20) & 0xFu;
  return o;
}

__device__ __forceinline__ uint32_t rng_keep_mask_half(const RngKey key, uint32_t row_id, uint32_t grp) {
  uint32_t x = (row_id * 64u + grp) ^ key.a;
  x *= 0x7feb352dU;
  x ^= x >> 15;
  x *= 0x846ca68bU;
  x ^= x >> 16;
  x += key.b;
  return (rng_word(x, 0xB5297A4Du, 0x85EBCA77u) >> 12) & 0xFu;
}

__device__ __forceinline__ f4 keep_scale4(uint32_t bits, float keep_scale) {
  f4 s;
#pragma unroll
  for (int r = 0; r < 4; ++r) s[r] = ((bits >> r) & 1u) ? keep_scale : 0.f;
  return s;
}
__device__ __forceinline__ int sbit(uint32_t bits, int idx) {
  int m = __builtin_amdgcn_sbfe(bits, idx, 1);
  asm("" : "+v"(m));
  return m;
}
__device__ __forceinline__ float keep_and(float x, uint32_t bits, int r) {
  return __uint_as_float(__float_as_uint(x) & (uint32_t)sbit(bits, r));
}

__device__ __forceinline__ void store_out4(float* p, const f4 v) { __builtin_nontemporal_store(v, (f4*)p); }
__device__ __forceinline__ void store_out1(float* p, const float v) { __builtin_nontemporal_store(v, p); }

__device__ __forceinline__ bool qblock_has_ctx(const acattn_bwd_io& IO, int b, int qb) {
  if (IO.active_qblocks) return (IO.active_qblocks[b] >> qb) & 1u;
  if (IO.read_rows) {
    for (int r = 0; r < IO.n_read_rows; ++r)
      if ((int)(IO.read_rows[(size_t)b * IO.n_read_rows + r] >> 4) == qb) return true;
    return false;
  }
  return true;
}

__device__ __forceinline__ bool qblock_active(const acattn_bwd_io& IO, int b, int qb) {
  if (IO.d_attack_mask || IO.d_penalty_part) return true;
  if (IO.active_qblocks) return (IO.active_qblocks[b] >> qb) & 1u;
  if (IO.read_rows) {
    for (int r = 0; r < IO.n_read_rows; ++r)
      if ((int)(IO.read_rows[(size_t)b * IO.n_read_rows + r] >> 4) == qb) return true;
    return false;
  }
  return true;
}

__device__ __forceinline__ void decode_block(int bid, int B, int nh, int& b, int& h) {
  if ((B & 7) == 0) {
    const int grp = bid / (8 * nh), rem = bid - grp * 8 * nh;
    h = rem >> 3;
    b = grp * 8 + (rem & 7);
  } else {
    b = bid / nh;
    h = bid - b * nh;
  }
}

int acattn_launch_fwd(const acattn_problem& p, const acattn_fwd_out& o, hipStream_t stream);
int acattn_fwd_kernel_choice(int which);
int acattn_bwd_kernel_choice(int which);
int64_t acattn_bwd_stream_ws_bytes(const acattn_problem& p);
int acattn_launch_bwd(const acattn_problem& p, const acattn_bwd_io& io, hipStream_t stream);
bool acattn_bwd_gate_summed(const acattn_problem& p, const acattn_bwd_io& io);
bool acattn_bwd_pair_supported(const acattn_problem& p, const acattn_bwd_io& io);
int64_t acattn_spatial_bwd_ws_bytes(const acattn_problem& p);
int acattn_launch_spatial_bwd(const acattn_problem& p, const acattn_spatial_bwd_io& io, hipStream_t stream);
int acattn_launch_spatial_affines(const acattn_problem& p, float* affine, hipStream_t stream);
int acattn_launch_rng(int B, int nh, int L, uint64_t seed, float p_drop, float* noise, uint8_t* keep_after,
                      uint8_t* keep_mask, uint8_t* keep_before, hipStream_t stream);
int64_t acattn_ce_ws_bytes(const acattn_ce_problem& p);
int acattn_launch_ce_fwd(const acattn_ce_problem& p, void* ws, float* lse, float* row_loss, hipStream_t stream);
int acattn_launch_ce_fwd_dir(const acattn_ce_problem& p, void* ws, float* lse, float* row_loss, float* dir,
                             hipStream_t stream);
int acattn_launch_ce_bwd(const acattn_ce_problem& p, const float* lse, const float* coef, void* ws, float* d_out,
                         float* d_table, hipStream_t stream);
int acattn_launch_ln_fwd(const acattn_ln_problem& p, float* y, float* stats, hipStream_t stream);
int acattn_launch_ln_bwd(const acattn_ln_problem& p, const float* dy, const float* stats, float* dz, float* dres,
                         float* dgb_part, hipStream_t stream);
int acattn_launch_sum_rows(const float* x, float* out, int batch, int R, int C, hipStream_t stream);
int acattn_launch_sum_rows_pair(const float* x1, float* out1, int batch1, int R1, int C1, const float* x2, float* out2,
                                int batch2, int R2, int C2, hipStream_t stream);
void acattn_set_error(const char* msg);
bool acattn_proj_supported(int H, int G);
int64_t acattn_proj_bwd_ws_bytes(const acattn_proj_problem& p);
int acattn_launch_proj_fwd(const acattn_proj_problem& p, const acattn_proj_out& o, hipStream_t stream);
bool acattn_proj_qkv_supported(int H);
int acattn_launch_proj_qkv_fwd(const acattn_proj_problem& p, const acattn_proj_out& o, hipStream_t stream);
int acattn_launch_proj_bwd(const acattn_proj_problem& p, const acattn_proj_bwd_io& io, hipStream_t stream);
bool acattn_tail_supported(int H, int I);
int acattn_tail_bwd_partial_rows(int rows);
int acattn_tail_bwd_partial_rows_h(int rows, int H);
int64_t acattn_tail_bwd_ws_bytes(int H, int I);
int acattn_select_tail_nb(int nb);
int64_t acattn_tail_split_bytes(int H, int I, int rows);
int acattn_launch_tail_split(const acattn_tail_problem& p, void* planes, hipStream_t stream);
int acattn_launch_tail_fwd(const acattn_tail_problem& p, const acattn_tail_saved& s, hipStream_t stream);
int acattn_launch_tail_bwd(const acattn_tail_problem& p, const acattn_tail_saved& s, const acattn_tail_bwd_io& io,
                           hipStream_t stream);
int64_t acattn_linear_wgrad_ws_bytes(int64_t M, int K, int N);
int acattn_launch_linear_wgrad(const float* const* x, const float* const* dy, const int* K, const int* N,
                               float* const* dw, float* const* db, int n_items, int64_t M, void* ws, hipStream_t stream,
                               int* P_out = nullptr, long long* w_off_out = nullptr, long long* b_off_out = nullptr);
int acattn_launch_linear_wgrad_reduce_many(const float* const* part_w, const float* const* part_b, const int* K, const int* N,
                                           const int* P, float* const* dw, float* const* db, int n_items,
                                           const float* const* sr_x, float* const* sr_out, const int* sr_R, const int* sr_C,
                                           int n_sr, hipStream_t stream);
int acattn_launch_embed_fwd(const acattn_embed_problem& p, float* y, float* stats, hipStream_t stream);
int acattn_launch_embed_bwd(const acattn_embed_problem& p, const float* dy, const float* stats, int64_t padding_idx,
                            float* d_table, float* d_pos_part, float* dgb_part, hipStream_t stream);
int acattn_launch_penalty_fwd(const float* m, int64_t n, float* ws, float* norm, hipStream_t stream);
int acattn_launch_penalty_partial(const float* m, int64_t n, float* part, hipStream_t stream);
void acattn_penalty_written_set(bool v);
bool acattn_penalty_written();
int acattn_launch_penalty_rows(const float* m, int B, int nh, int L, float* pen, hipStream_t stream);
int acattn_launch_attacked_loss_finish_rows(const float* row_loss, int B, const float* const* pen, int n_masks, int count,
                                            float weight, float* out, float* scale_buf, int n_scale, hipStream_t stream);
int acattn_launch_penalty_drows(const float* norms, const float* d_loss, float scale, int count, float* const* d_pen,
                                int n_masks, hipStream_t stream, const float* dir = nullptr, float* d_out = nullptr, int n_dir = 0);
int acattn_launch_attacked_loss_finish(const float* row_loss, int B, const float* part, int n_masks, int64_t mask_numel,
                                       float weight, float* out, float* scale_buf, int n_scale, hipStream_t stream);
int acattn_launch_penalty_bwd_scaled(const float* m, const float* norm, const float* d_loss, float scale, int64_t n,
                                     float* d_m, hipStream_t stream);
int acattn_launch_penalty_bwd(const float* m, const float* norm, const float* d_norm, int64_t n, float* d_m,
                              hipStream_t stream);
int acattn_launch_zero(float* p, size_t n, hipStream_t stream);
int64_t acattn_ce6_rows_bytes(const acattn_ce_problem& p);
int acattn_launch_ce6_sweep(const acattn_ce_problem& p, const float* lse, const float* coef, float* slab, float* d_table,
                            float2* part, void* rows_ws, int n_wg, int n_left, bool dir, hipStream_t stream);
int acattn_launch_ce6_onehot_reduce(const acattn_ce_problem& p, const float* coef, const float* slab, int n_slabs, float* d_out,
                                    float* d_table, hipStream_t stream);
int acattn_launch_ce6_fwd_sweep(const acattn_ce_problem& p, float2* part, void* rows_ws, int n_wg, int n_left, hipStream_t stream);
int acattn_ce_products_choice(int mode);
int acattn_linear_products_choice(int mode);
int acattn_launch_dense_ce_fwd(const float* logits, int64_t rows, int64_t N, const int64_t* target, float* lse, float* row_loss,
                               hipStream_t stream);
int acattn_launch_dense_ce_bwd(const float* logits, const float* lse, const int64_t* target, const float* coef, int64_t rows,
                               int64_t N, float* d_logits, hipStream_t stream);
int acattn_launch_step_inputs(const void* const* src, void* const* dst, const int64_t* bytes, int n, int64_t* counter,
                              const int64_t* item_length, int64_t* last_row, int n_rows, hipStream_t stream);
int acattn_launch_penalty_partial_multi(const float* const* m, int n_masks, int64_t n, float* part, hipStream_t stream);
int acattn_launch_penalty_bwd_scaled_multi(const float* const* m, const float* norms, const float* d_loss, float scale,
                                           int64_t n, float* const* d_m, int n_masks, hipStream_t stream);
int acattn_launch_adam_step(const acattn_adam_group& g, double lr, double beta1, double beta2, double eps,
                            double weight_decay, int* done, hipStream_t stream);
```

### ac_tsr_amd/csrc/acattn_tail.hip

```cpp
#include <stdlib.h>
#include <string.h>

#include <algorithm>

#include "acattn_common.h"
#include "acattn_rowops.h"
#include "acattn_split.h"
#include "acattn_wstage.h"

int acattn_tail_bwd_partial_rows(int rows);
int acattn_tail_bwd_partial_rows_h(int rows, int H);

namespace {

int g_tail_nb = getenv("ACATTN_TAIL_BLOCKS") ? atoi(getenv("ACATTN_TAIL_BLOCKS")) : 0;
bool split_slabs(int rows) {
  static const int limit = getenv("ACATTN_TAIL_SPLIT_ROWS") ? atoi(getenv("ACATTN_TAIL_SPLIT_ROWS")) : 4096;
  return g_tail_nb == 0 && rows <= limit;
}
#ifndef ACATTN_TAIL64_WAVES
#define ACATTN_TAIL64_WAVES 3
#endif
bool staged64(int rows) {
  static const bool per_wave = getenv("ACATTN_TAIL_PER_WAVE") != nullptr;
// ... 147 lines not shown
  load_slab(wave + NW, sl[1]);
  PIN_ORDER();

  f4 h1[NB][DT], a[NB][DT];
#pragma unroll
  for (int nt = 0; nt < DT; ++nt)
#pragma unroll
    for (int nb = 0; nb < NB; ++nb) h1[nb][nt] = bd[nt];
#pragma unroll
  for (int t = 0; t < DT; ++t)
#pragma unroll
    for (int r = 0; r < 4; ++r)
#pragma unroll
      for (int nt = 0; nt < DT; ++nt)
#pragma unroll
        for (int nb = 0; nb < NB; ++nb) h1[nb][nt] = mfma16(wd[nt][t][r], cb[nb][t][r], h1[nb][nt]);
#pragma unroll
  for (int nb = 0; nb < NB; ++nb) {
    f4 keep[DT];
#pragma unroll
    for (int t = 0; t < DT; ++t) keep[t] = row_keep_scale(P.p1, P.keep1, P.seed1 + step, W.row[nb], 4 * t + g, H);
    float mean, rstd;
    ln_forward<DT>(h1[nb], res[nb], keep, g1, b1, P.eps1, a[nb], mean, rstd);
    if (W.ok[nb] && wave == 0) {
#pragma unroll
      for (int t = 0; t < DT; ++t) {
        const size_t o = (size_t)W.row[nb] * H + 16 * t + 4 * g;
        *(f4*)(S.h1 + o) = h1[nb][t];
        *(f4*)(S.a + o) = a[nb][t];
      }
      if (g == 0) *(float2*)(S.st1 + 2 * (size_t)W.row[nb]) = float2{mean, rstd};
    }
  }

  f4 h3[NB][DT], bb2[DT], g2[DT], b2[DT];
  load_cols<DT>(P.bb2, g, bb2);
  load_cols<DT>(P.g2, g, g2);
  load_cols<DT>(P.b2, g, b2);
  auto first_product = [&](const Slab& s, f4 (&h2)[NB][2]) {
#pragma unroll
    for (int nb = 0; nb < NB; ++nb) h2[nb][0] = h2[nb][1] = f4{0.f, 0.f, 0.f, 0.f};
#pragma unroll
    for (int t = 0; t < DT; ++t)
#pragma unroll
      for (int r = 0; r < 4; ++r)
#pragma unroll
        for (int nb = 0; nb < NB; ++nb) h2[nb][r & 1] = mfma16(s.w1[t][r], a[nb][t][r], h2[nb][r & 1]);
  };
  f4 h2[2][NB][2];
  first_product(sl[0], h2[0]);
#pragma unroll
  for (int nt = 0; nt < DT; ++nt)
#pragma unroll
    for (int nb = 0; nb < NB; ++nb) h3[nb][nt] = wave == 0 ? bb2[nt] : f4{0.f, 0.f, 0.f, 0.f};
  static_for<NS>([&](auto jc) {
    constexpr int J = decltype(jc)::value;
    const int mt = wave + NW * J;
    if (J + 2 < NS) load_slab(mt + 2 * NW, sl[(J + 2) % 3]);
    PIN_ORDER();
    const Slab& cur = sl[J % 3];
    if (J + 1 < NS) first_product(sl[(J + 1) % 3], h2[(J + 1) & 1]);
#pragma unroll
    for (int nb = 0; nb < NB; ++nb) {
      const f4 pre = (h2[J & 1][nb][0] + h2[J & 1][nb][1]) + cur.b1;
      f4 act;
#pragma unroll
      for (int r = 0; r < 4; ++r) act[r] = gelu_erf(pre[r]);
      if (W.ok[nb]) *(f4*)(S.act + (size_t)W.row[nb] * I + 16 * mt + 4 * g) = act;
#pragma unroll
      for (int r = 0; r < 4; ++r)
#pragma unroll
        for (int nt = 0; nt < DT; ++nt) h3[nb][nt] = mfma16(cur.w2[nt][r], act[r], h3[nb][nt]);
    }
    PIN_ORDER();
  });

  if (NW > 1) {
    __shared__ f4 red[NW > 1 ? NW - 1 : 1][DT][64];
    if (wave > 0) {
#pragma unroll
      for (int t = 0; t < DT; ++t) red[wave - 1][t][threadIdx.x & 63] = h3[0][t];
    }
    __syncthreads();
    if (wave > 0) return;
#pragma unroll
    for (int w = 0; w < NW - 1; ++w)
#pragma unroll
      for (int t = 0; t < DT; ++t) h3[0][t] += red[w][t][threadIdx.x & 63];
  }

#pragma unroll
  for (int nb = 0; nb < NB; ++nb) {
    f4 keep[DT], y[DT];
#pragma unroll
    for (int t = 0; t < DT; ++t) keep[t] = row_keep_scale(P.p2, P.keep2, P.seed2 + step, W.row[nb], 4 * t + g, H);
    float mean, rstd;
    ln_forward<DT>(h3[nb], a[nb], keep, g2, b2, P.eps2, y, mean, rstd);
    if (W.ok[nb]) {
#pragma unroll
      for (int t = 0; t < DT; ++t) {
        const size_t o = (size_t)W.row[nb] * H + 16 * t + 4 * g;
        *(f4*)(S.h3 + o) = h3[nb][t];
        *(f4*)(S.out + o) = y[t];
      }
      if (g == 0) *(float2*)(S.st2 + 2 * (size_t)W.row[nb]) = float2{mean, rstd};
    }
  }
}

template <int DT>
__device__ __forceinline__ void ln_backward(const f4 (&z)[DT], const f4 (&res)[DT], const f4 (&keep)[DT], const float* gamma,
                                            float mean, float rstd, const f4 (&dy)[DT], bool ok, int g, f4 (&dz)[DT],
                                            f4 (&acc_g)[DT], f4 (&acc_b)[DT]) {
  constexpr float inv_h = 1.0f / (16 * DT);
  f4 xh[DT], gg[DT];
  float m1 = 0.f, m2 = 0.f;
#pragma unroll
  for (int t = 0; t < DT; ++t) {
    xh[t] = ((z[t] * keep[t] + res[t]) - mean) * rstd;
    gg[t] = dy[t] * *(const f4*)(gamma + 16 * t + 4 * g);
    m1 += (gg[t][0] + gg[t][1]) + (gg[t][2] + gg[t][3]);
    m2 += (gg[t][0] * xh[t][0] + gg[t][1] * xh[t][1]) + (gg[t][2] * xh[t][2] + gg[t][3] * xh[t][3]);
    if (ok) {
      acc_g[t] += dy[t] * xh[t];
      acc_b[t] += dy[t];
    }
  }
  m1 = quad_sum(m1) * inv_h;
  m2 = quad_sum(m2) * inv_h;
#pragma unroll
  for (int t = 0; t < DT; ++t) dz[t] = (gg[t] - m1 - xh[t] * m2) * rstd;
}

template <int DT>
__device__ __forceinline__ void store_partial(float* part, const f4 (&acc)[DT], int c, int g) {
#pragma unroll
  for (int t = 0; t < DT; ++t) {
    f4 v;
#pragma unroll
    for (int r = 0; r < 4; ++r) v[r] = dpp_row_sum(acc[t][r]);
    if (c == 0) *(f4*)(part + 16 * t + 4 * g) = v;
  }
}

__device__ __forceinline__ void store_grad(float* dst, f4 v, bool accumulate) {
  if (accumulate) {
#pragma unroll
    for (int e = 0; e < 4; ++e) atomicAdd(dst + e, v[e]);
  } else {
    *(f4*)dst = v;
  }
}

template <int H, int I, int NB, int NW = 1>
__global__ void __launch_bounds__(64 * NW) tail_bwd_kernel(const acattn_tail_problem P, const acattn_tail_saved S,
                                                           const acattn_tail_bwd_io IO) {
  static_assert(NW == 1 || NB == 1, "the slab split works on one row block");
  constexpr int DT = H / 16, IT = I / 16;
  const int c = threadIdx.x & 15, g = (threadIdx.x >> 4) & 3;
  const int wave = NW > 1 ? __builtin_amdgcn_readfirstlane(threadIdx.x >> 6) : 0;
  const Rows<NB> W = wave_rows<NB>(P);
  const uint64_t step = P.seed_device ? *P.seed_device : 0ull;
  float* part = IO.dgb_part ? IO.dgb_part + (size_t)blockIdx.x * 4 * H : nullptr;

  f4 a[NB][DT], dh3[NB][DT], da[NB][DT];
  {
    f4 acc_g[DT], acc_b[DT];
#pragma unroll
    for (int t = 0; t < DT; ++t) acc_g[t] = acc_b[t] = f4{0.f, 0.f, 0.f, 0.f};
#pragma unroll
    for (int nb = 0; nb < NB; ++nb) {
      f4 z[DT], keep[DT], dy[DT];
#pragma unroll
      for (int t = 0; t < DT; ++t) {
        const size_t o = (size_t)W.row[nb] * H + 16 * t + 4 * g;
        z[t] = *(const f4*)(S.h3 + o);
        a[nb][t] = *(const f4*)(S.a + o);
        dy[t] = *(const f4*)(IO.d_out + o);
        keep[t] = row_keep_scale(P.p2, P.keep2, P.seed2 + step, W.row[nb], 4 * t + g, H);
      }
      const float2 st = *(const float2*)(S.st2 + 2 * (size_t)W.row[nb]);
      ln_backward<DT>(z, a[nb], keep, P.g2, st.x, st.y, dy, W.ok[nb], g, da[nb], acc_g, acc_b);
#pragma unroll
      for (int t = 0; t < DT; ++t) {
        dh3[nb][t] = da[nb][t] * keep[t];
        if (IO.d_h3 && W.ok[nb] && wave == 0) *(f4*)(IO.d_h3 + (size_t)W.row[nb] * H + 16 * t + 4 * g) = dh3[nb][t];
        if (wave > 0) da[nb][t] = f4{0.f, 0.f, 0.f, 0.f};
      }
    }
    if (part && wave == 0) {
      store_partial<DT>(part + 2 * H, acc_g, c, g);
      store_partial<DT>(part + 3 * H, acc_b, c, g);
    }
  }

  struct Slab {
    f4 w1[DT];
    f4 w2t[DT];
    f4 w1t[DT];
    f4 b1;
  };
  auto load_slab = [&](int mt, Slab& s) {
#pragma unroll
    for (int t = 0; t < DT; ++t) {
      s.w1[t] = *(const f4*)(P.w1 + (size_t)(16 * mt + c) * H + 16 * t + 4 * g);
#pragma unroll
      for (int r = 0; r < 4; ++r) {
        s.w2t[t][r] = P.w2[(size_t)(16 * t + 4 * g + r) * I + 16 * mt + c];
        s.w1t[t][r] = P.w1[(size_t)(16 * mt + 4 * g + r) * H + 16 * t + c];
      }
    }
    s.b1 = *(const f4*)(P.bb1 + 16 * mt + 4 * g);
  };
  Slab cur, nxt;
  load_slab(wave, cur);
#pragma unroll 2
  for (int mt = wave; mt < IT; mt += NW) {
    load_slab(mt + NW < IT ? mt + NW : mt, nxt);
#pragma unroll
    for (int nb = 0; nb < NB; ++nb) {
      f4 h2[2] = {f4{0.f, 0.f, 0.f, 0.f}, f4{0.f, 0.f, 0.f, 0.f}}, dact[2] = {f4{0.f, 0.f, 0.f, 0.f}, f4{0.f, 0.f, 0.f, 0.f}};
#pragma unroll
      for (int t = 0; t < DT; ++t)
#pragma unroll
        for (int r = 0; r < 4; ++r) {
          h2[r & 1] = mfma16(cur.w1[t][r], a[nb][t][r], h2[r & 1]);
          dact[r & 1] = mfma16(cur.w2t[t][r], dh3[nb][t][r], dact[r & 1]);
        }
      const f4 pre = (h2[0] + h2[1]) + cur.b1, dac = dact[0] + dact[1];
      f4 dh2;
#pragma unroll
      for (int r = 0; r < 4; ++r) dh2[r] = dac[r] * gelu_erf_grad(pre[r]);
      if (IO.d_h2 && W.ok[nb]) *(f4*)(IO.d_h2 + (size_t)W.row[nb] * I + 16 * mt + 4 * g) = dh2;
#pragma unroll
      for (int r = 0; r < 4; ++r)
#pragma unroll
        for (int nt = 0; nt < DT; ++nt) da[nb][nt] = mfma16(cur.w1t[nt][r], dh2[r], da[nb][nt]);
    }
    cur = nxt;
  }

  if (NW > 1) {
    __shared__ f4 red[NW > 1 ? NW - 1 : 1][DT][64];
    if (wave > 0) {
#pragma unroll
      for (int t = 0; t < DT; ++t) red[wave - 1][t][threadIdx.x & 63] = da[0][t];
    }
    __syncthreads();
    if (wave > 0) return;
#pragma unroll
    for (int w = 0; w < NW - 1; ++w)
#pragma unroll
      for (int t = 0; t < DT; ++t) da[0][t] += red[w][t][threadIdx.x & 63];
  }

  f4 dh1[NB][DT];
  {
    f4 acc_g[DT], acc_b[DT];
#pragma unroll
    for (int t = 0; t < DT; ++t) acc_g[t] = acc_b[t] = f4{0.f, 0.f, 0.f, 0.f};
#pragma unroll
    for (int nb = 0; nb < NB; ++nb) {
      f4 z[DT], res[DT], keep[DT], dz[DT];
#pragma unroll
      for (int t = 0; t < DT; ++t) {
        const size_t o = (size_t)W.row[nb] * H + 16 * t + 4 * g;
        z[t] = *(const f4*)(S.h1 + o);
        res[t] = *(const f4*)(P.x + (size_t)W.src[nb] * H + 16 * t + 4 * g);
        keep[t] = row_keep_scale(P.p1, P.keep1, P.seed1 + step, W.row[nb], 4 * t + g, H);
      }
      const float2 st = *(const float2*)(S.st1 + 2 * (size_t)W.row[nb]);
      ln_backward<DT>(z, res, keep, P.g1, st.x, st.y, da[nb], W.ok[nb], g, dz, acc_g, acc_b);
#pragma unroll
      for (int t = 0; t < DT; ++t) {
        const size_t o = (size_t)W.row[nb] * H + 16 * t + 4 * g;
        dh1[nb][t] = dz[t] * keep[t];
        if (W.ok[nb]) {
          if (IO.d_x) store_grad(IO.d_x + (size_t)W.src[nb] * H + 16 * t + 4 * g, dz[t], P.src_index != nullptr);
          if (IO.d_h1) *(f4*)(IO.d_h1 + o) = dh1[nb][t];
        }
      }
    }
    if (part) {
      store_partial<DT>(part, acc_g, c, g);
      store_partial<DT>(part + H, acc_b, c, g);
    }
  }
  if (IO.d_ctx) {
    f4 dc[NB][DT];
#pragma unroll
    for (int nb = 0; nb < NB; ++nb)
#pragma unroll
      for (int nt = 0; nt < DT; ++nt) dc[nb][nt] = f4{0.f, 0.f, 0.f, 0.f};
    f4 wdt[DT][DT];
#pragma unroll
    for (int nt = 0; nt < DT; ++nt)
#pragma unroll
      for (int t = 0; t < DT; ++t)
#pragma unroll
        for (int r = 0; r < 4; ++r) wdt[nt][t][r] = P.wd[(size_t)(16 * t + 4 * g + r) * H + 16 * nt + c];
#pragma unroll
    for (int t = 0; t < DT; ++t)
#pragma unroll
      for (int r = 0; r < 4; ++r)
#pragma unroll
        for (int nt = 0; nt < DT; ++nt)
#pragma unroll
          for (int nb = 0; nb < NB; ++nb) dc[nb][nt] = mfma16(wdt[nt][t][r], dh1[nb][t][r], dc[nb][nt]);
#pragma unroll
    for (int nb = 0; nb < NB; ++nb)
      if (W.ok[nb])
#pragma unroll
        for (int nt = 0; nt < DT; ++nt) store_grad(IO.d_ctx + (size_t)W.src[nb] * H + 16 * nt + 4 * g, dc[nb][nt], P.src_index != nullptr);
  }
}


template <int I>
struct TailPlanes {
  static constexpr int SQ = 64 * 64 * 3 / 8, RECT = I * 64 * 3 / 8;
  static constexpr int FWD_D = 0, FWD_1 = SQ, FWD_2 = SQ + RECT;
  static constexpr int BWD_D = SQ + 2 * RECT, BWD_1 = 2 * SQ + 2 * RECT, BWD_2 = 2 * SQ + 3 * RECT;
  static constexpr int TOTAL = 2 * SQ + 4 * RECT;
};

__device__ __forceinline__ int tail_kperm(int s, int g, int j) { return 32 * s + 16 * (j >> 2) + 4 * g + (j & 3); }

template <int I>
__global__ void __launch_bounds__(256) tail_split_planes_kernel(const float* wd, const float* w1, const float* w2, b8* planes) {
  using L = TailPlanes<I>;
  const int mtx = blockIdx.y, which = mtx % 3;
  const bool T = mtx >= 3;
  const float* w = which == 0 ? wd : which == 1 ? w1 : w2;
  const int M = which == 0 ? 64 : ((which == 1) != T ? I : 64), K = (which == 0 ? 64 * 64 : 64 * I) / M, KS = K / 32;
  b8* dst = planes + (mtx == 0 ? L::FWD_D : mtx == 1 ? L::FWD_1 : mtx == 2 ? L::FWD_2 : mtx == 3 ? L::BWD_D : mtx == 4 ? L::BWD_1 : L::BWD_2);
  const int idx = blockIdx.x * 256 + threadIdx.x;
  if (idx >= (M / 16) * KS * 64) return;
  const int lane = idx & 63, f = idx >> 6, mt = f / KS, s = f % KS, c = lane & 15, g = lane >> 4, m = 16 * mt + c;
  float x[8];
#pragma unroll
  for (int j = 0; j < 8; ++j) {
    const int k = tail_kperm(s, g, j);
    x[j] = T ? w[(size_t)k * M + m] : w[(size_t)m * K + k];
  }
  b8 p[3];
  split8(x, p[0], p[1], p[2]);
#pragma unroll
  for (int q = 0; q < 3; ++q) dst[((size_t)f * 3 + q) * 64 + lane] = p[q];
}

template <int KS>
__device__ __forceinline__ void load_frag(const b8* mat, int mt, int s, int lane, b8 (&a)[3]) {
#pragma unroll
  for (int q = 0; q < 3; ++q) a[q] = mat[((mt * KS + s) * 3 + q) * 64 + lane];
}

__device__ __forceinline__ void split_tiles(const f4 lo, const f4 hi, b8 (&b)[3]) {
  float x[8];
#pragma unroll
  for (int r = 0; r < 4; ++r) {
    x[r] = lo[r];
    x[4 + r] = hi[r];
  }
  split8(x, b[0], b[1], b[2]);
}

template <int NB>
__device__ __forceinline__ void split_rows64(const f4 (&v)[NB][4], b8 (&b)[NB][2][3]) {
#pragma unroll
  for (int nb = 0; nb < NB; ++nb)
#pragma unroll
    for (int s = 0; s < 2; ++s) split_tiles(v[nb][2 * s], v[nb][2 * s + 1], b[nb][s]);
}

template <int NB>
__device__ __forceinline__ void split_square(const b8* mat, int lane, const b8 (&b)[NB][2][3], f4 (&acc)[NB][4]) {
#pragma unroll
  for (int nt = 0; nt < 4; ++nt)
#pragma unroll
    for (int s = 0; s < 2; ++s) {
      b8 w[3];
      load_frag<2>(mat, nt, s, lane, w);
#pragma unroll
      for (int nb = 0; nb < NB; ++nb) acc[nb][nt] = mfma_split(w, b[nb][s], acc[nb][nt]);
    }
}

template <int H, int I, int NB, int NW = 1>
__global__ void __launch_bounds__(64 * NW) tail_split_fwd_kernel(const acattn_tail_problem P, const acattn_tail_saved S) {
  static_assert(H == 64 && (NW == 1 || NB == 1), "hidden 64; the slab split works on one row block");
  using L = TailPlanes<I>;
  constexpr int DT = 4, NP = I / 32, NJ = NP / NW;
  static_assert(NP % NW == 0 && NJ >= 1, "whole pairs per wave");
  const int lane = threadIdx.x & 63, c = lane & 15, g = lane >> 4;
  const int wave = NW > 1 ? __builtin_amdgcn_readfirstlane(threadIdx.x >> 6) : 0;
  const Rows<NB> W = wave_rows<NB>(P);
  const uint64_t step = P.seed_device ? *P.seed_device : 0ull;
  const b8* planes = (const b8*)P.split_planes;
  const b8 *pw1 = planes + L::FWD_1, *pw2 = planes + L::FWD_2;

  struct W1Pair {
    b8 w[2][2][3];
    f4 b[2];
  };
  auto load_w1 = [&](int p, W1Pair& d) {
#pragma unroll
    for (int tt = 0; tt < 2; ++tt) {
#pragma unroll
      for (int s = 0; s < 2; ++s) load_frag<2>(pw1, 2 * p + tt, s, lane, d.w[tt][s]);
      d.b[tt] = *(const f4*)(P.bb1 + 32 * p + 16 * tt + 4 * g);
    }
  };
  W1Pair w1b[2];
  load_w1(wave, w1b[0]);

  f4 h1[NB][DT], a[NB][DT];
  {
    f4 cb[NB][DT], res[NB][DT], bd[DT], g1[DT], b1[DT];
#pragma unroll
    for (int nb = 0; nb < NB; ++nb)
#pragma unroll
      for (int t = 0; t < DT; ++t) {
        cb[nb][t] = *(const f4*)(P.ctx + (size_t)W.src[nb] * H + 16 * t + 4 * g);
        res[nb][t] = *(const f4*)(P.x + (size_t)W.src[nb] * H + 16 * t + 4 * g);
      }
    load_cols<DT>(P.bd, g, bd);
    load_cols<DT>(P.g1, g, g1);
    load_cols<DT>(P.b1, g, b1);
    b8 cs[NB][2][3];
    split_rows64<NB>(cb, cs);
#pragma unroll
    for (int nb = 0; nb < NB; ++nb)
#pragma unroll
      for (int nt = 0; nt < DT; ++nt) h1[nb][nt] = bd[nt];
    split_square<NB>(planes + L::FWD_D, lane, cs, h1);
#pragma unroll
    for (int nb = 0; nb < NB; ++nb) {
      f4 keep[DT];
#pragma unroll
      for (int t = 0; t < DT; ++t) keep[t] = row_keep_scale(P.p1, P.keep1, P.seed1 + step, W.row[nb], 4 * t + g, H);
      float mean, rstd;
      ln_forward<DT>(h1[nb], res[nb], keep, g1, b1, P.eps1, a[nb], mean, rstd);
      if (W.ok[nb] && wave == 0) {
#pragma unroll
        for (int t = 0; t < DT; ++t) {
          const size_t o = (size_t)W.row[nb] * H + 16 * t + 4 * g;
          *(f4*)(S.h1 + o) = h1[nb][t];
          *(f4*)(S.a + o) = a[nb][t];
        }
        if (g == 0) *(float2*)(S.st1 + 2 * (size_t)W.row[nb]) = float2{mean, rstd};
      }
    }
  }

  b8 as[NB][2][3];
  split_rows64<NB>(a, as);
  f4 h3[NB][DT];
#pragma unroll
  for (int nt = 0; nt < DT; ++nt) {
    const f4 bb2 = *(const f4*)(P.bb2 + 16 * nt + 4 * g);
#pragma unroll
    for (int nb = 0; nb < NB; ++nb) h3[nb][nt] = wave == 0 ? bb2 : f4{0.f, 0.f, 0.f, 0.f};
  }
  static_for<NJ>([&](auto jc) {
    constexpr int J = decltype(jc)::value;
    const int p = wave + NW * J;
    b8 w2[DT][3];
#pragma unroll
    for (int nt = 0; nt < DT; ++nt) load_frag<NP>(pw2, nt, p, lane, w2[nt]);
    if constexpr (J + 1 < NJ) load_w1(p + NW, w1b[(J + 1) & 1]);
    PIN_ORDER();
    const W1Pair& cur = w1b[J & 1];
    f4 h2[NB][2];
#pragma unroll
    for (int tt = 0; tt < 2; ++tt)
#pragma unroll
      for (int nb = 0; nb < NB; ++nb) h2[nb][tt] = f4{0.f, 0.f, 0.f, 0.f};
#pragma unroll
    for (int tt = 0; tt < 2; ++tt)
#pragma unroll
      for (int s = 0; s < 2; ++s)
#pragma unroll
        for (int nb = 0; nb < NB; ++nb) h2[nb][tt] = mfma_split(cur.w[tt][s], as[nb][s], h2[nb][tt]);
#pragma unroll
    for (int nb = 0; nb < NB; ++nb) {
      f4 act[2];
#pragma unroll
      for (int tt = 0; tt < 2; ++tt) {
        const f4 pre = h2[nb][tt] + cur.b[tt];
#pragma unroll
        for (int r = 0; r < 4; ++r) act[tt][r] = gelu_erf(pre[r]);
        if (W.ok[nb]) *(f4*)(S.act + (size_t)W.row[nb] * I + 32 * p + 16 * tt + 4 * g) = act[tt];
      }
      b8 ap[3];
      split_tiles(act[0], act[1], ap);
#pragma unroll
      for (int nt = 0; nt < DT; ++nt) h3[nb][nt] = mfma_split(w2[nt], ap, h3[nb][nt]);
    }
    PIN_ORDER();
  });

  if (NW > 1) {
    __shared__ f4 red[NW > 1 ? NW - 1 : 1][DT][64];
    if (wave > 0) {
#pragma unroll
      for (int t = 0; t < DT; ++t) red[wave - 1][t][lane] = h3[0][t];
    }
    __syncthreads();
    if (wave > 0) return;
#pragma unroll
    for (int w = 0; w < NW - 1; ++w)
#pragma unroll
      for (int t = 0; t < DT; ++t) h3[0][t] += red[w][t][lane];
  }

  f4 g2[DT], b2[DT];
  load_cols<DT>(P.g2, g, g2);
  load_cols<DT>(P.b2, g, b2);
#pragma unroll
  for (int nb = 0; nb < NB; ++nb) {
    f4 keep[DT], y[DT];
#pragma unroll
    for (int t = 0; t < DT; ++t) keep[t] = row_keep_scale(P.p2, P.keep2, P.seed2 + step, W.row[nb], 4 * t + g, H);
    float mean, rstd;
    ln_forward<DT>(h3[nb], a[nb], keep, g2, b2, P.eps2, y, mean, rstd);
    if (W.ok[nb]) {
#pragma unroll
      for (int t = 0; t < DT; ++t) {
        const size_t o = (size_t)W.row[nb] * H + 16 * t + 4 * g;
        *(f4*)(S.h3 + o) = h3[nb][t];
        *(f4*)(S.out + o) = y[t];
      }
      if (g == 0) *(float2*)(S.st2 + 2 * (size_t)W.row[nb]) = float2{mean, rstd};
    }
  }
}

template <int H, int I, int NB, int NW = 1>
__global__ void __launch_bounds__(64 * NW) tail_split_bwd_kernel(const acattn_tail_problem P, const acattn_tail_saved S,
                                                                 const acattn_tail_bwd_io IO) {
  static_assert(H == 64 && (NW == 1 || NB == 1), "hidden 64; the slab split works on one row block");
  using L = TailPlanes<I>;
  constexpr int DT = 4, NP = I / 32, NJ = NP / NW;
  static_assert(NP % NW == 0 && NJ >= 1, "whole pairs per wave");
  const int lane = threadIdx.x & 63, c = lane & 15, g = lane >> 4;
  const int wave = NW > 1 ? __builtin_amdgcn_readfirstlane(threadIdx.x >> 6) : 0;
  const Rows<NB> W = wave_rows<NB>(P);
  const uint64_t step = P.seed_device ? *P.seed_device : 0ull;
  float* part = IO.dgb_part ? IO.dgb_part + (size_t)blockIdx.x * 4 * H : nullptr;
  const b8* planes = (const b8*)P.split_planes;
  const b8 *pw1 = planes + L::FWD_1, *pw1t = planes + L::BWD_1, *pw2t = planes + L::BWD_2;

  struct Pair {
    b8 w1[2][2][3], w2t[2][2][3];
    f4 b[2];
  };
  auto load_pair = [&](int p, Pair& d) {
#pragma unroll
    for (int tt = 0; tt < 2; ++tt) {
#pragma unroll
      for (int s = 0; s < 2; ++s) {
        load_frag<2>(pw1, 2 * p + tt, s, lane, d.w1[tt][s]);
        load_frag<2>(pw2t, 2 * p + tt, s, lane, d.w2t[tt][s]);
      }
      d.b[tt] = *(const f4*)(P.bb1 + 32 * p + 16 * tt + 4 * g);
    }
  };
  Pair pb[2];
  load_pair(wave, pb[0]);

  f4 a[NB][DT], dh3[NB][DT], da[NB][DT];
  {
    f4 acc_g[DT], acc_b[DT];
#pragma unroll
    for (int t = 0; t < DT; ++t) acc_g[t] = acc_b[t] = f4{0.f, 0.f, 0.f, 0.f};
#pragma unroll
    for (int nb = 0; nb < NB; ++nb) {
      f4 z[DT], keep[DT], dy[DT];
#pragma unroll
      for (int t = 0; t < DT; ++t) {
        const size_t o = (size_t)W.row[nb] * H + 16 * t + 4 * g;
        z[t] = *(const f4*)(S.h3 + o);
        a[nb][t] = *(const f4*)(S.a + o);
        dy[t] = *(const f4*)(IO.d_out + o);
        keep[t] = row_keep_scale(P.p2, P.keep2, P.seed2 + step, W.row[nb], 4 * t + g, H);
      }
      const float2 st = *(const float2*)(S.st2 + 2 * (size_t)W.row[nb]);
      ln_backward<DT>(z, a[nb], keep, P.g2, st.x, st.y, dy, W.ok[nb], g, da[nb], acc_g, acc_b);
#pragma unroll
      for (int t = 0; t < DT; ++t) {
        dh3[nb][t] = da[nb][t] * keep[t];
        if (IO.d_h3 && W.ok[nb] && wave == 0) *(f4*)(IO.d_h3 + (size_t)W.row[nb] * H + 16 * t + 4 * g) = dh3[nb][t];
        if (wave > 0) da[nb][t] = f4{0.f, 0.f, 0.f, 0.f};
      }
    }
    if (part && wave == 0) {
      store_partial<DT>(part + 2 * H, acc_g, c, g);
      store_partial<DT>(part + 3 * H, acc_b, c, g);
    }
  }

  {
    b8 as[NB][2][3], ds[NB][2][3];
    split_rows64<NB>(a, as);
    split_rows64<NB>(dh3, ds);
    static_for<NJ>([&](auto jc) {
      constexpr int J = decltype(jc)::value;
      const int p = wave + NW * J;
      b8 w1t[DT][3];
#pragma unroll
      for (int nt = 0; nt < DT; ++nt) load_frag<NP>(pw1t, nt, p, lane, w1t[nt]);
      if constexpr (J + 1 < NJ) load_pair(p + NW, pb[(J + 1) & 1]);
      PIN_ORDER();
      const Pair& cur = pb[J & 1];
      f4 h2[NB][2], dact[NB][2];
#pragma unroll
      for (int tt = 0; tt < 2; ++tt)
#pragma unroll
        for (int nb = 0; nb < NB; ++nb) h2[nb][tt] = dact[nb][tt] = f4{0.f, 0.f, 0.f, 0.f};
#pragma unroll
      for (int tt = 0; tt < 2; ++tt)
#pragma unroll
        for (int s = 0; s < 2; ++s)
#pragma unroll
          for (int nb = 0; nb < NB; ++nb) {
            h2[nb][tt] = mfma_split(cur.w1[tt][s], as[nb][s], h2[nb][tt]);
            dact[nb][tt] = mfma_split(cur.w2t[tt][s], ds[nb][s], dact[nb][tt]);
          }
#pragma unroll
      for (int nb = 0; nb < NB; ++nb) {
        f4 dh2[2];
#pragma unroll
        for (int tt = 0; tt < 2; ++tt) {
          const f4 pre = h2[nb][tt] + cur.b[tt];
#pragma unroll
          for (int r = 0; r < 4; ++r) dh2[tt][r] = dact[nb][tt][r] * gelu_erf_grad(pre[r]);
          if (IO.d_h2 && W.ok[nb]) *(f4*)(IO.d_h2 + (size_t)W.row[nb] * I + 32 * p + 16 * tt + 4 * g) = dh2[tt];
        }
        b8 dp[3];
        split_tiles(dh2[0], dh2[1], dp);
#pragma unroll
        for (int nt = 0; nt < DT; ++nt) da[nb][nt] = mfma_split(w1t[nt], dp, da[nb][nt]);
      }
      PIN_ORDER();
    });
  }

  if (NW > 1) {
    __shared__ f4 red[NW > 1 ? NW - 1 : 1][DT][64];
    if (wave > 0) {
#pragma unroll
      for (int t = 0; t < DT; ++t) red[wave - 1][t][lane] = da[0][t];
    }
    __syncthreads();
    if (wave > 0) return;
#pragma unroll
    for (int w = 0; w < NW - 1; ++w)
#pragma unroll
      for (int t = 0; t < DT; ++t) da[0][t] += red[w][t][lane];
  }

  f4 dh1[NB][DT];
  {
    f4 acc_g[DT], acc_b[DT];
#pragma unroll
    for (int t = 0; t < DT; ++t) acc_g[t] = acc_b[t] = f4{0.f, 0.f, 0.f, 0.f};
#pragma unroll
    for (int nb = 0; nb < NB; ++nb) {
      f4 z[DT], res[DT], keep[DT], dz[DT];
#pragma unroll
      for (int t = 0; t < DT; ++t) {
        const size_t o = (size_t)W.row[nb] * H + 16 * t + 4 * g;
        z[t] = *(const f4*)(S.h1 + o);
        res[t] = *(const f4*)(P.x + (size_t)W.src[nb] * H + 16 * t + 4 * g);
        keep[t] = row_keep_scale(P.p1, P.keep1, P.seed1 + step, W.row[nb], 4 * t + g, H);
      }
      const float2 st = *(const float2*)(S.st1 + 2 * (size_t)W.row[nb]);
      ln_backward<DT>(z, res, keep, P.g1, st.x, st.y, da[nb], W.ok[nb], g, dz, acc_g, acc_b);
#pragma unroll
      for (int t = 0; t < DT; ++t) {
        const size_t o = (size_t)W.row[nb] * H + 16 * t + 4 * g;
        dh1[nb][t] = dz[t] * keep[t];
        if (W.ok[nb]) {
          if (IO.d_x) store_grad(IO.d_x + (size_t)W.src[nb] * H + 16 * t + 4 * g, dz[t], P.src_index != nullptr);
          if (IO.d_h1) *(f4*)(IO.d_h1 + o) = dh1[nb][t];
        }
      }
    }
    if (part) {
      store_partial<DT>(part, acc_g, c, g);
      store_partial<DT>(part + H, acc_b, c, g);
    }
  }
  if (IO.d_ctx) {
    f4 dc[NB][DT];
#pragma unroll
    for (int nb = 0; nb < NB; ++nb)
#pragma unroll
      for (int nt = 0; nt < DT; ++nt) dc[nb][nt] = f4{0.f, 0.f, 0.f, 0.f};
    b8 hs[NB][2][3];
    split_rows64<NB>(dh1, hs);
    split_square<NB>(planes + L::BWD_D, lane, hs, dc);
#pragma unroll
    for (int nb = 0; nb < NB; ++nb)
      if (W.ok[nb])
#pragma unroll
        for (int nt = 0; nt < DT; ++nt) store_grad(IO.d_ctx + (size_t)W.src[nb] * H + 16 * nt + 4 * g, dc[nb][nt], P.src_index != nullptr);
  }
}

template <int DT, class Emit>
__device__ __forceinline__ void stream_square(const float* w, const float* bias, int c, int g, const f4 (&in)[DT], Emit&& emit) {
  constexpr int H = 16 * DT;
  f4 wbuf[2][DT], bb[2];
  auto load = [&](int nt, f4 (&dst)[DT], f4& b) {
    b = bias ? *(const f4*)(bias + 16 * nt + 4 * g) : f4{0.f, 0.f, 0.f, 0.f};
#pragma unroll
    for (int t = 0; t < DT; ++t) dst[t] = *(const f4*)(w + (size_t)(16 * nt + c) * H + 16 * t + 4 * g);
  };
  load(0, wbuf[0], bb[0]);
  static_for<DT>([&](auto k) {
    constexpr int NT = decltype(k)::value;
    if constexpr (NT + 1 < DT) load(NT + 1, wbuf[(NT + 1) & 1], bb[(NT + 1) & 1]);
    PIN_ORDER();
    f4 acc[2] = {bb[NT & 1], f4{0.f, 0.f, 0.f, 0.f}};
#pragma unroll
    for (int t = 0; t < DT; ++t)
#pragma unroll
      for (int r = 0; r < 4; ++r) acc[r & 1] = mfma16(wbuf[NT & 1][t][r], in[t][r], acc[r & 1]);
    emit(k, acc[0] + acc[1]);
  });
}

template <int H, int I, int NW>
__global__ void __launch_bounds__(64 * NW, NW == 1 ? 2 : 1) tail_wide_fwd_kernel(const acattn_tail_problem P, const acattn_tail_saved S) {
  constexpr int DT = H / 16, IT = I / 16, NS = IT / NW;
  static_assert(NS >= 2, "two slabs are requested ahead");
  const int c = threadIdx.x & 15, g = (threadIdx.x >> 4) & 3;
  const int wave = NW > 1 ? __builtin_amdgcn_readfirstlane(threadIdx.x >> 6) : 0;
  const Rows<1> W = wave_rows<1>(P);
  const uint64_t step = P.seed_device ? *P.seed_device : 0ull;
  const int row = W.row[0];
  const bool ok = W.ok[0];

  f4 a[DT];
  {
    f4 cb[DT], res[DT], h1[DT];
#pragma unroll
    for (int t = 0; t < DT; ++t) {
      cb[t] = *(const f4*)(P.ctx + (size_t)W.src[0] * H + 16 * t + 4 * g);
      res[t] = *(const f4*)(P.x + (size_t)W.src[0] * H + 16 * t + 4 * g);
    }
    stream_square<DT>(P.wd, P.bd, c, g, cb, [&](auto k, f4 v) { h1[decltype(k)::value] = v; });
    f4 keep[DT];
#pragma unroll
    for (int t = 0; t < DT; ++t) keep[t] = row_keep_scale(P.p1, P.keep1, P.seed1 + step, row, 4 * t + g, H);
    float mean, rstd;
    ln_forward_mem<DT>(h1, res, keep, P.g1, P.b1, g, P.eps1, a, mean, rstd);
    if (ok && wave == 0) {
#pragma unroll
      for (int t = 0; t < DT; ++t) {
        const size_t o = (size_t)row * H + 16 * t + 4 * g;
        *(f4*)(S.h1 + o) = h1[t];
        *(f4*)(S.a + o) = a[t];
      }
      if (g == 0) *(float2*)(S.st1 + 2 * (size_t)row) = float2{mean, rstd};
    }
  }

  f4 w1b[2][DT], w2b[DT], b1b[3];
  auto load_w1 = [&](int mt, f4 (&dst)[DT], f4& b) {
    b = *(const f4*)(P.bb1 + 16 * mt + 4 * g);
#pragma unroll
    for (int t = 0; t < DT; ++t) dst[t] = *(const f4*)(P.w1 + (size_t)(16 * mt + c) * H + 16 * t + 4 * g);
  };
  auto load_w2 = [&](int mt, f4 (&dst)[DT]) {
#pragma unroll
    for (int t = 0; t < DT; ++t) dst[t] = *(const f4*)(P.w2 + (size_t)(16 * t + c) * I + 16 * mt + 4 * g);
  };
  load_w1(wave, w1b[0], b1b[0]);
  load_w1(wave + NW, w1b[1], b1b[1]);
  load_w2(wave, w2b);
  f4 h3[DT];
#pragma unroll
  for (int nt = 0; nt < DT; ++nt) h3[nt] = wave == 0 ? *(const f4*)(P.bb2 + 16 * nt + 4 * g) : f4{0.f, 0.f, 0.f, 0.f};
  PIN_ORDER();
  auto first_product = [&](const f4 (&w1)[DT], f4 (&h2)[2]) {
    h2[0] = h2[1] = f4{0.f, 0.f, 0.f, 0.f};
#pragma unroll
    for (int t = 0; t < DT; ++t)
#pragma unroll
      for (int r = 0; r < 4; ++r) h2[r & 1] = mfma16(w1[t][r], a[t][r], h2[r & 1]);
  };
  f4 h2[2][2];
  first_product(w1b[0], h2[0]);
  static_for<NS>([&](auto jc) {
    constexpr int J = decltype(jc)::value;
    const int mt = wave + NW * J;
    if constexpr (J + 2 < NS) load_w1(mt + 2 * NW, w1b[J & 1], b1b[(J + 2) % 3]);
    PIN_ORDER();
    if constexpr (J + 1 < NS) first_product(w1b[(J + 1) & 1], h2[(J + 1) & 1]);
    const f4 pre = (h2[J & 1][0] + h2[J & 1][1]) + b1b[J % 3];
    f4 act, dact;
#pragma unroll
    for (int r = 0; r < 4; ++r) {
      const PhiExp pe = phi_exp(pre[r]);
      act[r] = pre[r] * pe.phi;
      dact[r] = fmaf(pre[r] * kInvSqrt2Pi, pe.e, pe.phi);
    }
    if (ok) {
      *(f4*)(S.act + (size_t)row * I + 16 * mt + 4 * g) = act;
      if (S.gelu_grad) *(f4*)(S.gelu_grad + (size_t)row * I + 16 * mt + 4 * g) = dact;
    }
#pragma unroll
    for (int r = 0; r < 4; ++r)
#pragma unroll
      for (int nt = 0; nt < DT; ++nt) h3[nt] = mfma16(w2b[nt][r], act[r], h3[nt]);
    PIN_ORDER();
    if constexpr (J + 1 < NS) load_w2(mt + NW, w2b);
  });

  if (NW > 1) {
    __shared__ f4 red[NW > 1 ? NW - 1 : 1][DT][64];
    if (wave > 0) {
#pragma unroll
      for (int t = 0; t < DT; ++t) red[wave - 1][t][threadIdx.x & 63] = h3[t];
    }
    __syncthreads();
    if (wave > 0) return;
#pragma unroll
    for (int w = 0; w < NW - 1; ++w)
#pragma unroll
      for (int t = 0; t < DT; ++t) h3[t] += red[w][t][threadIdx.x & 63];
  }

  {
    f4 keep[DT], y[DT];
#pragma unroll
    for (int t = 0; t < DT; ++t) keep[t] = row_keep_scale(P.p2, P.keep2, P.seed2 + step, row, 4 * t + g, H);
    float mean, rstd;
    ln_forward_mem<DT>(h3, a, keep, P.g2, P.b2, g, P.eps2, y, mean, rstd);
    if (ok) {
#pragma unroll
      for (int t = 0; t < DT; ++t) {
        const size_t o = (size_t)row * H + 16 * t + 4 * g;
        *(f4*)(S.h3 + o) = h3[t];
        *(f4*)(S.out + o) = y[t];
      }
      if (g == 0) *(float2*)(S.st2 + 2 * (size_t)row) = float2{mean, rstd};
    }
  }
}

__global__ void __launch_bounds__(256) tail_transpose_kernel(const float* w1, const float* w2, const float* wd, int H, int I, float* ws) {
  __shared__ float tile[16][17];
  const int mtx = blockIdx.z;
  const float* src = mtx == 0 ? w1 : mtx == 1 ? w2 : wd;
  const int R = mtx == 0 ? I : H, Cn = mtx == 1 ? I : H;
  float* dst = ws + (mtx == 0 ? 0 : mtx == 1 ? (size_t)H * I : 2 * (size_t)H * I);
  const int r0 = blockIdx.x * 16, c0 = blockIdx.y * 16;
// ... 741 lines not shown
      if constexpr (!last) st.commit();
    });
    if (IO.d_ctx && ok) store_grad(IO.d_ctx + (size_t)W.src[0] * H + 16 * NT + 4 * g, acc[0] + acc[1], P.src_index != nullptr);
  });
}

template <int H, int I>
int launch_wide_fwd(const acattn_tail_problem& p, const acattn_tail_saved& s, hipStream_t stream) {
  const int blocks = (p.rows + 15) / 16;
  static const bool per_wave = getenv("ACATTN_TAIL_PER_WAVE") != nullptr;
  static const bool chunked = getenv("ACATTN_TAIL_CHUNKED") != nullptr;
  if (H > 128 || chunked) {
    hipLaunchKernelGGL((tail_chunked_fwd_kernel<H, I>), dim3((blocks + NWV - 1) / NWV), dim3(64 * NWV), 0, stream, p, s);
    return (int)hipGetLastError();
  }
  if constexpr (H <= 128) {
  if (wide_split(p.rows))
    hipLaunchKernelGGL((tail_wide_fwd_kernel<H, I, 4>), dim3(blocks), dim3(256), 0, stream, p, s);
  else if (per_wave)
    hipLaunchKernelGGL((tail_wide_fwd_kernel<H, I, 1>), dim3(blocks), dim3(64), 0, stream, p, s);
  else
    hipLaunchKernelGGL((tail_staged_fwd_kernel<H, I>), dim3((blocks + NWV - 1) / NWV), dim3(64 * NWV), 0, stream, p, s);
  }
  return (int)hipGetLastError();
}

template <int H, int I>
int launch_wide_bwd(const acattn_tail_problem& p, const acattn_tail_saved& s, const acattn_tail_bwd_io& io, hipStream_t stream) {
  if (!io.workspace) {
    acattn_set_error("layer tail backward at hidden 128 / 256 needs acattn_tail_bwd_io.workspace");
    return -1;
  }
  float* ws = (float*)io.workspace;
  hipLaunchKernelGGL(tail_transpose_kernel, dim3(I / 16, I / 16, 3), dim3(256), 0, stream, p.w1, p.w2, p.wd, H, I, ws);
  const int blocks = (p.rows + 15) / 16;
  const bool split = wide_split(p.rows);
  static const bool per_wave = getenv("ACATTN_TAIL_PER_WAVE") != nullptr;
  static const bool chunked = getenv("ACATTN_TAIL_CHUNKED") != nullptr;
  if (H > 128 || chunked) {
    const int wgs = (blocks + NWV - 1) / NWV;
    if (s.gelu_grad)
      hipLaunchKernelGGL((tail_chunked_bwd_kernel<H, I, true>), dim3(wgs), dim3(64 * NWV), 0, stream, p, s, io, (const float*)ws);
    else
      hipLaunchKernelGGL((tail_chunked_bwd_kernel<H, I, false>), dim3(wgs), dim3(64 * NWV), 0, stream, p, s, io, (const float*)ws);
    return (int)hipGetLastError();
  }
  if constexpr (H <= 128) {
  if (!split && !per_wave) {
    const int wgs = (blocks + NWV - 1) / NWV;
    if (s.gelu_grad)
      hipLaunchKernelGGL((tail_staged_bwd_kernel<H, I, true>), dim3(wgs), dim3(64 * NWV), 0, stream, p, s, io, (const float*)ws);
    else
      hipLaunchKernelGGL((tail_staged_bwd_kernel<H, I, false>), dim3(wgs), dim3(64 * NWV), 0, stream, p, s, io, (const float*)ws);
    return (int)hipGetLastError();
  }
  if (s.gelu_grad) {
    if (split)
      hipLaunchKernelGGL((tail_wide_bwd_kernel<H, I, 4, true>), dim3(blocks), dim3(256), 0, stream, p, s, io, (const float*)ws);
    else
      hipLaunchKernelGGL((tail_wide_bwd_kernel<H, I, 1, true>), dim3(blocks), dim3(64), 0, stream, p, s, io, (const float*)ws);
  } else {
    if (split)
      hipLaunchKernelGGL((tail_wide_bwd_kernel<H, I, 4, false>), dim3(blocks), dim3(256), 0, stream, p, s, io, (const float*)ws);
    else
      hipLaunchKernelGGL((tail_wide_bwd_kernel<H, I, 1, false>), dim3(blocks), dim3(64), 0, stream, p, s, io, (const float*)ws);
  }
  }
  return (int)hipGetLastError();
}

bool tail_split_products(int H, int I, int rows) {
  static const char* e = getenv("ACATTN_TAIL_PRODUCTS");
  static const bool fp32 = e && !strcmp(e, "fp32");
  return H == 64 && (I == 256 || I == 128) && !fp32 && acattn_linear_products_choice(-1) == 1 && !staged64(rows);
}

template <int I>
int launch_split_planes(const acattn_tail_problem& p, void* planes, hipStream_t stream) {
  hipLaunchKernelGGL(tail_split_planes_kernel<I>, dim3(I / 32, 6), dim3(256), 0, stream, p.wd, p.w1, p.w2, (b8*)planes);
  return (int)hipGetLastError();
}

template <int H, int I>
int launch_fwd(const acattn_tail_problem& p, const acattn_tail_saved& s, hipStream_t stream) {
  if (staged64(p.rows)) {
    const int wgs = (p.rows + 16 * NWV - 1) / (16 * NWV);
    hipLaunchKernelGGL((tail_chunked_fwd_kernel<H, I>), dim3(wgs), dim3(64 * NWV), 0, stream, p, s);
    return (int)hipGetLastError();
  }
  const int nb = rows_per_wave(p.rows) / 16;
  const int blocks = (p.rows + 16 * nb - 1) / (16 * nb);
  if (p.split_planes) {
    if (nb == 1 && split_slabs(p.rows))
      hipLaunchKernelGGL((tail_split_fwd_kernel<H, I, 1, 4>), dim3(blocks), dim3(256), 0, stream, p, s);
    else if (nb == 2)
      hipLaunchKernelGGL((tail_split_fwd_kernel<H, I, 2>), dim3(blocks), dim3(64), 0, stream, p, s);
    else
      hipLaunchKernelGGL((tail_split_fwd_kernel<H, I, 1>), dim3(blocks), dim3(64), 0, stream, p, s);
    return (int)hipGetLastError();
  }
  if (nb == 1 && split_slabs(p.rows)) {
    hipLaunchKernelGGL((tail_fwd_kernel<H, I, 1, 4>), dim3(blocks), dim3(256), 0, stream, p, s);
    return (int)hipGetLastError();
  }
  if (nb == 2)
    hipLaunchKernelGGL((tail_fwd_kernel<H, I, 2>), dim3(blocks), dim3(64), 0, stream, p, s);
  else
    hipLaunchKernelGGL((tail_fwd_kernel<H, I, 1>), dim3(blocks), dim3(64), 0, stream, p, s);
  return (int)hipGetLastError();
}

template <int H, int I>
int launch_bwd(const acattn_tail_problem& p, const acattn_tail_saved& s, const acattn_tail_bwd_io& io, hipStream_t stream) {
  if (staged64(p.rows)) {
    if (!io.workspace) {
      acattn_set_error("layer tail backward: this row count needs acattn_tail_bwd_io.workspace (acattn_layer_tail_bwd_workspace_bytes)");
      return -1;
    }
    float* ws = (float*)io.workspace;
    hipLaunchKernelGGL(tail_transpose_kernel, dim3(I / 16, I / 16, 3), dim3(256), 0, stream, p.w1, p.w2, p.wd, H, I, ws);
    const int wgs = (p.rows + 16 * NWV - 1) / (16 * NWV);
    if (s.gelu_grad)
      hipLaunchKernelGGL((tail_chunked_bwd_kernel<H, I, true>), dim3(wgs), dim3(64 * NWV), 0, stream, p, s, io, (const float*)ws);
    else
      hipLaunchKernelGGL((tail_chunked_bwd_kernel<H, I, false>), dim3(wgs), dim3(64 * NWV), 0, stream, p, s, io, (const float*)ws);
    return (int)hipGetLastError();
  }
  const int nb = rows_per_wave(p.rows) / 16;
  const int blocks = acattn_tail_bwd_partial_rows(p.rows);
  if (p.split_planes && !(nb == 1 && split_slabs(p.rows))) {
    if (nb == 2)
      hipLaunchKernelGGL((tail_split_bwd_kernel<H, I, 2>), dim3(blocks), dim3(64), 0, stream, p, s, io);
    else
      hipLaunchKernelGGL((tail_split_bwd_kernel<H, I, 1>), dim3(blocks), dim3(64), 0, stream, p, s, io);
    return (int)hipGetLastError();
  }
  if (nb == 1 && split_slabs(p.rows)) {
    hipLaunchKernelGGL((tail_bwd_kernel<H, I, 1, 4>), dim3(blocks), dim3(256), 0, stream, p, s, io);
    return (int)hipGetLastError();
  }
  if (nb == 2)
    hipLaunchKernelGGL((tail_bwd_kernel<H, I, 2>), dim3(blocks), dim3(64), 0, stream, p, s, io);
  else
    hipLaunchKernelGGL((tail_bwd_kernel<H, I, 1>), dim3(blocks), dim3(64), 0, stream, p, s, io);
  return (int)hipGetLastError();
}

}

bool acattn_tail_supported(int H, int I) {
  return (H == 64 && (I == 256 || I == 128)) || (H == 128 && (I == 512 || I == 256)) || (H == 256 && I == 1024);
}

int acattn_tail_bwd_partial_rows(int rows) { return (rows + rows_per_wave(rows) - 1) / rows_per_wave(rows); }
int acattn_tail_bwd_partial_rows_h(int rows, int H) {
  return (H > 64 || staged64(rows)) ? (rows + 15) / 16 : acattn_tail_bwd_partial_rows(rows);
}
int64_t acattn_tail_bwd_ws_bytes(int H, int I) { return ((int64_t)2 * H * I + (int64_t)H * H) * (int64_t)sizeof(float); }

int64_t acattn_tail_split_bytes(int H, int I, int rows) {
  if (!tail_split_products(H, I, rows)) return 0;
  return (int64_t)(I == 256 ? TailPlanes<256>::TOTAL : TailPlanes<128>::TOTAL) * (int64_t)sizeof(b8);
}

int acattn_launch_tail_split(const acattn_tail_problem& p, void* planes, hipStream_t stream) {
  if (p.H == 64 && p.I == 256) return launch_split_planes<256>(p, planes, stream);
  if (p.H == 64 && p.I == 128) return launch_split_planes<128>(p, planes, stream);
  acattn_set_error("layer tail split planes: hidden 64, inner 256 or 128 only");
  return -1;
}

int acattn_select_tail_nb(int nb) {
  const int prev = g_tail_nb;
  g_tail_nb = nb;
  return prev;
}

int acattn_launch_tail_fwd(const acattn_tail_problem& p, const acattn_tail_saved& s, hipStream_t stream) {
  if (p.H == 64 && p.I == 256) return launch_fwd<64, 256>(p, s, stream);
  if (p.H == 64 && p.I == 128) return launch_fwd<64, 128>(p, s, stream);
  if (p.H == 128 && p.I == 512) return launch_wide_fwd<128, 512>(p, s, stream);
  if (p.H == 128 && p.I == 256) return launch_wide_fwd<128, 256>(p, s, stream);
  if (p.H == 256 && p.I == 1024) return launch_wide_fwd<256, 1024>(p, s, stream);
  acattn_set_error("layer tail: unsupported (hidden_size, inner_size)");
  return -1;
}

int acattn_launch_tail_bwd(const acattn_tail_problem& p, const acattn_tail_saved& s, const acattn_tail_bwd_io& io,
                           hipStream_t stream) {
  if (p.H == 64 && p.I == 256) return launch_bwd<64, 256>(p, s, io, stream);
  if (p.H == 64 && p.I == 128) return launch_bwd<64, 128>(p, s, io, stream);
  if (p.H == 128 && p.I == 512) return launch_wide_bwd<128, 512>(p, s, io, stream);
  if (p.H == 128 && p.I == 256) return launch_wide_bwd<128, 256>(p, s, io, stream);
  if (p.H == 256 && p.I == 1024) return launch_wide_bwd<256, 1024>(p, s, io, stream);
  acattn_set_error("layer tail: unsupported (hidden_size, inner_size)");
  return -1;
}
```

### ac_tsr_amd/csrc/acattn_util.hip

```cpp
#include <algorithm>

#include <stdlib.h>

#include "acattn_common.h"
#include "acattn_sumrows.h"

namespace {

template <bool ATOMIC>
__global__ void __launch_bounds__(256) sum_rows_kernel(const float* __restrict__ x, float* __restrict__ out, int R, int C,
                                                       int rows_per_chunk, int CT) {
  sum_rows_block<ATOMIC>(x, out, R, C, rows_per_chunk, CT, blockIdx.x, blockIdx.y, blockIdx.z);
}

__global__ void __launch_bounds__(256) sum_rows_pair_kernel(const SumRowsJob a, const SumRowsJob b) {
  const bool first = (int)blockIdx.x < a.n_wg;
  const SumRowsJob& j = first ? a : b;
  const int w = first ? blockIdx.x : blockIdx.x - a.n_wg;
  sum_rows_block<false>(j.x, j.out, j.R, j.C, j.R, j.CT, w % j.col_groups, 0, w / j.col_groups);
}

constexpr int kPenaltyGrid = 1024;

__global__ void __launch_bounds__(256) penalty_partial_kernel(const float* __restrict__ m, const int64_t n,
// ... 329 lines not shown
int acattn_launch_sum_rows_pair(const float* x1, float* out1, int batch1, int R1, int C1, const float* x2, float* out2,
                                int batch2, int R2, int C2, hipStream_t stream) {
  const SumRowsJob a = make_job(x1, out1, batch1, R1, C1), b = make_job(x2, out2, batch2, R2, C2);
  hipLaunchKernelGGL(sum_rows_pair_kernel, dim3(a.n_wg + b.n_wg), dim3(256), 0, stream, a, b);
  return (int)hipGetLastError();
}

int acattn_launch_sum_rows(const float* x, float* out, int batch, int R, int C, hipStream_t stream) {
  const int c4 = (C + 3) / 4;
  const int CT = pick_ct(batch, R, C);
  const int col_groups = (c4 + CT - 1) / CT;
  const dim3 grid(col_groups, 1, batch);
  hipLaunchKernelGGL(sum_rows_kernel<false>, grid, dim3(256), 0, stream, x, out, R, C, R, CT);
  return (int)hipGetLastError();
}

namespace {
__global__ void __launch_bounds__(256) zero_fill_kernel(float* __restrict__ p, size_t n) {
  const size_t i0 = ((size_t)blockIdx.x * 256 + threadIdx.x) * 4;
  if (i0 + 3 < n && (reinterpret_cast<uintptr_t>(p + i0) & 15) == 0) {
    *(f4*)(p + i0) = f4{0.f, 0.f, 0.f, 0.f};
  } else {
#pragma unroll
    for (int e = 0; e < 4; ++e)
      if (i0 + e < n) p[i0 + e] = 0.f;
  }
}
}

__global__ void __launch_bounds__(256) dense_ce_fwd_kernel(const float* __restrict__ logits, long long rows, long long N,
                                                           const long long* __restrict__ target, float* __restrict__ lse,
                                                           float* __restrict__ row_loss) {
  constexpr float kL2e = 1.44269504088896340736f, kLn2 = 0.69314718055994530942f;
  __shared__ float sm[256], ss[256];
  for (long long r = blockIdx.x; r < rows; r += gridDim.x) {
    const float* x = logits + r * N;
    float m = -__builtin_inff(), s = 0.f;
    for (long long n0 = threadIdx.x; n0 < N; n0 += 1024) {
      float v[4];
#pragma unroll
      for (int e = 0; e < 4; ++e) v[e] = n0 + 256 * e < N ? x[n0 + 256 * e] : -__builtin_inff();
      const float vm = fmaxf(fmaxf(v[0], v[1]), fmaxf(v[2], v[3]));
      if (vm > m) {
        s *= __builtin_amdgcn_exp2f((m - vm) * kL2e);
        m = vm;
      }
#pragma unroll
      for (int e = 0; e < 4; ++e) s += __builtin_amdgcn_exp2f((v[e] - m) * kL2e);
    }
    sm[threadIdx.x] = m;
    ss[threadIdx.x] = s;
    __syncthreads();
    for (int off = 128; off > 0; off >>= 1) {
      if ((int)threadIdx.x < off) {
        const float m1 = sm[threadIdx.x], m2 = sm[threadIdx.x + off];
        const float mn = fmaxf(m1, m2);
        const float a = m1 > -__builtin_inff() ? ss[threadIdx.x] * __builtin_amdgcn_exp2f((m1 - mn) * kL2e) : 0.f;
        const float b = m2 > -__builtin_inff() ? ss[threadIdx.x + off] * __builtin_amdgcn_exp2f((m2 - mn) * kL2e) : 0.f;
        sm[threadIdx.x] = mn;
        ss[threadIdx.x] = a + b;
      }
      __syncthreads();
    }
    if (threadIdx.x == 0) {
      const float l = sm[0] + __builtin_amdgcn_logf(ss[0]) * kLn2;
      const long long t = target[r];
      lse[r] = l;
      row_loss[r] = (t >= 0 && t < N) ? l - x[t] : __builtin_nanf("");
    }
    __syncthreads();
  }
}
__global__ void __launch_bounds__(256) dense_ce_bwd_kernel(const float* __restrict__ logits, const float* __restrict__ lse,
                                                           const long long* __restrict__ target, const float* __restrict__ coef,
                                                           long long rows, long long N, float* __restrict__ d_logits) {
  constexpr float kL2e = 1.44269504088896340736f;
  const long long c0 = (long long)blockIdx.x * 1024 + threadIdx.x;
  for (long long r = blockIdx.y; r < rows; r += gridDim.y) {
    const float l = lse[r], cf = coef[r];
    const long long t = target[r];
    const float* x = logits + r * N;
    float* d = d_logits + r * N;
#pragma unroll
    for (int e = 0; e < 4; ++e) {
      const long long n = c0 + 256 * e;
      if (n < N) d[n] = cf * (__builtin_amdgcn_exp2f((x[n] - l) * kL2e) - (n == t ? 1.0f : 0.0f));
    }
  }
}
int acattn_launch_dense_ce_fwd(const float* logits, int64_t rows, int64_t N, const int64_t* target, float* lse, float* row_loss,
                               hipStream_t stream) {
  const unsigned blocks = (unsigned)std::min<int64_t>(rows, 8192);
  hipLaunchKernelGGL(dense_ce_fwd_kernel, dim3(blocks), dim3(256), 0, stream, logits, (long long)rows, (long long)N,
                     (const long long*)target, lse, row_loss);
  return (int)hipGetLastError();
}
int acattn_launch_dense_ce_bwd(const float* logits, const float* lse, const int64_t* target, const float* coef, int64_t rows,
                               int64_t N, float* d_logits, hipStream_t stream) {
  const dim3 grid((unsigned)((N + 1023) / 1024), (unsigned)std::min<int64_t>(rows, 32768));
  hipLaunchKernelGGL(dense_ce_bwd_kernel, grid, dim3(256), 0, stream, logits, lse, (const long long*)target, coef,
                     (long long)rows, (long long)N, d_logits);
  return (int)hipGetLastError();
}

struct StepInputs {
  const unsigned char* src[ACATTN_MAX_COPIES];
  unsigned char* dst[ACATTN_MAX_COPIES];
  long long bytes[ACATTN_MAX_COPIES];
  int n;
  long long* counter;
  const long long* item_length;
  long long* last_row;
  int n_rows;
};
__global__ void __launch_bounds__(256) step_inputs_kernel(const StepInputs A) {
  const size_t tid = (size_t)blockIdx.x * 256 + threadIdx.x, stride = (size_t)gridDim.x * 256;
  for (int k = 0; k < A.n; ++k) {
    const unsigned char* s = A.src[k];
    unsigned char* d = A.dst[k];
    const size_t nb = (size_t)A.bytes[k];
    if (((reinterpret_cast<uintptr_t>(s) | reinterpret_cast<uintptr_t>(d) | nb) & 15) == 0) {
      for (size_t i = tid; i < nb / 16; i += stride) ((uint4*)d)[i] = ((const uint4*)s)[i];
    } else {
      for (size_t i = tid; i < nb; i += stride) d[i] = s[i];
    }
  }
  if (A.last_row)
    for (size_t i = tid; i < (size_t)A.n_rows; i += stride) A.last_row[i] = A.item_length[i] - 1;
  if (A.counter && tid == 0) *A.counter += 1;
}
int acattn_launch_step_inputs(const void* const* src, void* const* dst, const int64_t* bytes, int n, int64_t* counter,
                              const int64_t* item_length, int64_t* last_row, int n_rows, hipStream_t stream) {
  StepInputs a;
  a.n = 0;
  size_t most = (size_t)(last_row ? n_rows : 0) * 16;
  for (int k = 0; k < n; ++k) {
    if (src[k] == dst[k] || bytes[k] <= 0) continue;
    a.src[a.n] = (const unsigned char*)src[k];
    a.dst[a.n] = (unsigned char*)dst[k];
    a.bytes[a.n] = bytes[k];
    most = std::max(most, (size_t)bytes[k]);
    ++a.n;
  }
  a.counter = (long long*)counter;
  a.item_length = (const long long*)item_length;
  a.last_row = (long long*)last_row;
  a.n_rows = n_rows;
  if (a.n == 0 && !counter && !last_row) return 0;
  const unsigned blocks = (unsigned)std::min<size_t>(1024, std::max<size_t>(1, (most / 16 + 255) / 256));
  hipLaunchKernelGGL(step_inputs_kernel, dim3(blocks), dim3(256), 0, stream, a);
  return (int)hipGetLastError();
}

int acattn_launch_zero(float* p, size_t n, hipStream_t stream) {
  if (n == 0) return 0;
  static const bool use_memset = getenv("ACATTN_ZERO_MEMSET") && atoi(getenv("ACATTN_ZERO_MEMSET")) != 0;
  if (use_memset) return (int)hipMemsetAsync(p, 0, n * sizeof(float), stream);
  hipLaunchKernelGGL(zero_fill_kernel, dim3((unsigned)((n + 1023) / 1024)), dim3(256), 0, stream, p, n);
  return (int)hipGetLastError();
}

namespace {
__global__ void __launch_bounds__(256) spatial_affines_kernel(const acattn_problem P, float* affine) {
  const int L = P.L, H = P.H, nh = P.n_heads, dh = H / nh;
  const int LP = ((L + 15) >> 4) << 4;
  const long long total = (long long)P.B * nh * LP;
  const long long idx = blockIdx.x * 256LL + threadIdx.x;
  if (idx >= total) return;
  const int i = (int)(idx % LP);
  const long long bh = idx / LP;
  const int h = (int)(bh % nh);
  const long long b = bh / nh;
  float* pl = affine + bh * 4 * LP + i;
  if (i >= L) {
    pl[0] = pl[LP] = pl[2 * LP] = pl[3 * LP] = 0.f;
    return;
  }
  const float* q = P.q + ((size_t)b * L + i) * H + h * dh;
  const float* k = P.k + ((size_t)b * L + i) * H + h * dh;
  float ao = 0.f, ad = 0.f, co = 0.f, cd = 0.f;
  for (int d = 0; d < dh; d += 4) {
    const f4 qv = *(const f4*)(q + d), kv = *(const f4*)(k + d);
    const f4 wo = *(const f4*)(P.w_order + d), wd = *(const f4*)(P.w_dist + d);
    const f4 wok = *(const f4*)(P.w_order + dh + d), wdk = *(const f4*)(P.w_dist + dh + d);
#pragma unroll
    for (int e = 0; e < 4; ++e) {
      ao = fmaf(qv[e], wo[e], ao);
      ad = fmaf(qv[e], wd[e], ad);
      co = fmaf(kv[e], wok[e], co);
      cd = fmaf(kv[e], wdk[e], cd);
    }
  }
  constexpr float kL2e = 1.44269504088896340736f;
  pl[0] = -kL2e * (ao + P.b_order[0]);
  pl[LP] = ad + P.b_dist[0];
  pl[2 * LP] = -kL2e * co;
  pl[3 * LP] = cd;
}
}

int acattn_launch_spatial_affines(const acattn_problem& p, float* affine, hipStream_t stream) {
  const long long total = (long long)p.B * p.n_heads * (((p.L + 15) >> 4) << 4);
  hipLaunchKernelGGL(spatial_affines_kernel, dim3((unsigned)((total + 255) / 256)), dim3(256), 0, stream, p, affine);
  return (int)hipGetLastError();
}
```

### ac_tsr_amd/layers.py

```python
from __future__ import annotations

import copy
import math
from typing import List, Optional

import torch
import torch.nn as nn
import torch.nn.functional as F

from . import fused_ln, ops
from . import tail
from .linear import projections, projections_qkv, skinny_linear
from .ops import AttentionConfig, ExplicitRandomness, StructuredMask
from .state import state_of


class AttackRMultiHeadAttention(nn.Module):

    def __init__(self, n_heads, hidden_size, hidden_dropout_prob, attn_dropout_prob, layer_norm_eps, use_order,
                 use_distance):
        super().__init__()
        if hidden_size % n_heads != 0:
            raise ValueError(
                "The hidden size (%d) is not a multiple of the number of attention "
# ... 4 lines not shown
        self.sqrt_attention_head_size = math.sqrt(self.attention_head_size)

        self.query = nn.Linear(hidden_size, self.all_head_size)
        self.key = nn.Linear(hidden_size, self.all_head_size)
        self.value = nn.Linear(hidden_size, self.all_head_size)

        self.use_order = use_order
        self.use_distance = use_distance
        if self.use_order:
            self.order_affine = nn.Linear(2 * self.attention_head_size, 1)
        if self.use_distance:
            self.distance_affine = nn.Linear(2 * self.attention_head_size, 1)
            self.scalar = nn.Parameter(torch.randn(1))

        self.attack_query_transform = nn.Linear(self.all_head_size, self.all_head_size)
        self.attack_key_transform = nn.Linear(self.all_head_size, self.all_head_size)

        self.attn_dropout_prob = attn_dropout_prob
        self.dense = nn.Linear(hidden_size, hidden_size)
        self.LayerNorm = nn.LayerNorm(hidden_size, eps=layer_norm_eps)
        self.out_dropout = nn.Dropout(hidden_dropout_prob)

    def project(self, input_tensor):
        mq = skinny_linear(input_tensor, self.query)
        mk = skinny_linear(input_tensor, self.key)
        mv = skinny_linear(input_tensor, self.value)
        qa = skinny_linear(mq, self.attack_query_transform)
        ka = skinny_linear(mk, self.attack_key_transform)
        return mq, mk, mv, qa, ka

    def calibrator_params(self):
        p = {}
        if self.use_order:
            p.update(w_order=self.order_affine.weight, b_order=self.order_affine.bias)
        if self.use_distance:
            p.update(w_dist=self.distance_affine.weight, b_dist=self.distance_affine.bias, scalar=self.scalar)
        return p

    def output(self, context_layer, input_tensor, _keep=None):
        hidden_states = skinny_linear(context_layer, self.dense)
        if hidden_states.is_cuda and fused_ln.supported(hidden_states.shape[-1]):
            return fused_ln.dropout_add_layer_norm(hidden_states, input_tensor, self.LayerNorm, self.out_dropout.p,
                                                   self.training, _keep)
        if _keep is not None:
            hidden_states = hidden_states * (_keep.to(hidden_states.dtype) / (1.0 - self.out_dropout.p))
        else:
            hidden_states = self.out_dropout(hidden_states)
        return self.LayerNorm(hidden_states + input_tensor)


class FeedForward(nn.Module):

    def __init__(self, hidden_size, inner_size, hidden_dropout_prob, hidden_act, layer_norm_eps):
        super().__init__()
        self.dense_1 = nn.Linear(hidden_size, inner_size)
        self.intermediate_act_fn = self.get_hidden_act(hidden_act)
        self.dense_2 = nn.Linear(inner_size, hidden_size)
        self.LayerNorm = nn.LayerNorm(hidden_size, eps=layer_norm_eps)
        self.dropout = nn.Dropout(hidden_dropout_prob)

    def get_hidden_act(self, act):
        ACT2FN = {
            "gelu": self.gelu,
            "relu": F.relu,
            "swish": self.swish,
            "tanh": torch.tanh,
            "sigmoid": torch.sigmoid,
        }
        return ACT2FN[act]

    def gelu(self, x):
        return F.gelu(x)

    def swish(self, x):
        return x * torch.sigmoid(x)

    def forward(self, input_tensor, _keep=None):
        hidden_states = skinny_linear(self.intermediate_act_fn(skinny_linear(input_tensor, self.dense_1)), self.dense_2)
        if hidden_states.is_cuda and fused_ln.supported(hidden_states.shape[-1]):
            return fused_ln.dropout_add_layer_norm(hidden_states, input_tensor, self.LayerNorm, self.dropout.p,
                                                   self.training, _keep)
        if _keep is not None:
            hidden_states = hidden_states * (_keep.to(hidden_states.dtype) / (1.0 - self.dropout.p))
        else:
            hidden_states = self.dropout(hidden_states)
        return self.LayerNorm(hidden_states + input_tensor)


class AttackRTransformerLayer(nn.Module):

    def __init__(self, n_heads, hidden_size, intermediate_size, hidden_dropout_prob, attn_dropout_prob, hidden_act,
                 layer_norm_eps, combine_option='fixed', use_order=True, use_distance=True, two_level=True,
                 rich_calibrated_combine='fixed', seq_length=50, adversarial=True):
        super().__init__()
        self.adversarial = bool(adversarial)
        self.hidden_size = hidden_size
        self.attack_attention = AttackRMultiHeadAttention(
            n_heads, hidden_size, hidden_dropout_prob, attn_dropout_prob, layer_norm_eps,
            use_order=use_order, use_distance=use_distance)
        self.two_level = two_level
        self.rich_calibrated_combine = rich_calibrated_combine
        if self.rich_calibrated_combine == 'trainable':
            self.rich_calibrated_combine_ratio = torch.nn.Parameter(torch.FloatTensor([0.5]), requires_grad=True)
        self.combine_option = combine_option
        if self.combine_option == 'gate':
            self.gate = torch.nn.Linear(hidden_size, seq_length)
        self.combine_ratio = 0.5
        self.feed_forward = FeedForward(hidden_size, intermediate_size, hidden_dropout_prob, hidden_act, layer_norm_eps)
        self.anneal_step = 0

    def _config(self) -> AttentionConfig:
        rate = 1.0
        if self.combine_option == 'annealing':
            rate = math.exp(-self.anneal_step / 100000)
            self.anneal_step += 1
        return AttentionConfig(n_heads=self.attack_attention.num_attention_heads, combine_option=self.combine_option,
                               two_level=self.two_level, rich_calibrated_combine=self.rich_calibrated_combine,
                               adversarial=self.adversarial, anneal_rate=rate)

    def forward(self, hidden_states, attention_mask, return_attention_prob=False, return_all_attention_prob=False,
                _rnd=None, _need_attacked=True, _attack_upstream=True, _rows=None):
        att = self.attack_attention
        cal = att.calibrator_params()
        if not self.adversarial:
            return self._forward_spatial_only(hidden_states, attention_mask, return_attention_prob, return_all_attention_prob,
                                              _rnd, _rows)
        mq, mk, mv, qa, ka, gate_logits, hidden_res, extras = projections(
            hidden_states, att.query, att.key, att.value, att.attack_query_transform, att.attack_key_transform,
            self.gate if self.combine_option == 'gate' else None, attack_upstream=_attack_upstream,
            spatial=(cal.get("w_order"), cal.get("b_order"), cal.get("w_dist"), cal.get("b_dist"), att.num_attention_heads))
        cfg = self._config()
        core_rnd = None
        if _rnd is not None:
            core_rnd = ExplicitRandomness(noise=_rnd.noise, keep_after=getattr(_rnd, "keep_after", None),
                                          keep_mask=getattr(_rnd, "keep_mask", None),
                                          keep_before=getattr(_rnd, "keep_before", None))
        p_drop = att.attn_dropout_prob if (self.training or (core_rnd is not None and core_rnd.keep_after is not None)) else 0.0
        want_probs = return_all_attention_prob or return_attention_prob
        ctx_att, ctx_cal, attack_mask, probs = ops.calibrated_attention(
            mq, mk, mv, qa, ka, gate_logits, attention_mask, cfg, p_drop=p_drop, rnd=core_rnd, want_probs=want_probs,
            seed_tensor=state_of(self).seed_tensor if core_rnd is None else None, read_rows=_rows,
            attack_upstream=_attack_upstream, state=state_of(self), rich_ratio=getattr(self, "rich_calibrated_combine_ratio", None),
            **extras, **cal)
        residual = hidden_res
        if _rows is not None:
            index = _rows.unsqueeze(-1).expand(-1, -1, hidden_states.shape[-1])
            pick = lambda t: None if t is None else t.gather(1, index)
            picks_itself = ctx_cal.is_cuda and tail.supported(att, self.feed_forward) and tail.fused_supported(att, self.feed_forward)
            if not picks_itself:
                residual = pick(hidden_res)
        else:
            pick = lambda t: t

        def branch(ctx_layer, keep_out, keep_ffn):
            one_launch = ctx_layer.is_cuda and tail.supported(att, self.feed_forward) and tail.fused_supported(att, self.feed_forward)
            fused = one_launch or (ctx_layer.is_cuda and torch.is_grad_enabled() and tail.supported(att, self.feed_forward))
            if one_launch and _rows is not None:
                return tail.layer_tail(ctx_layer, hidden_res, att, self.feed_forward, pick(keep_out), pick(keep_ffn),
                                       pick=_rows)
            ctx_layer, keep_out, keep_ffn = pick(ctx_layer), pick(keep_out), pick(keep_ffn)
            if fused:
                return tail.layer_tail(ctx_layer, residual, att, self.feed_forward, keep_out, keep_ffn)
            return self.feed_forward(att.output(ctx_layer, residual, keep_out), keep_ffn)

        attacked_feedforward_output = None
        if _need_attacked:
            attacked_feedforward_output = branch(ctx_att, getattr(_rnd, "keep_out_att", None),
                                                 getattr(_rnd, "keep_ffn_att", None))
        calibrated_feedforward_output = branch(ctx_cal, getattr(_rnd, "keep_out_cal", None),
                                               getattr(_rnd, "keep_ffn_cal", None))
        combined_attention_prob = probs.get("calibrated_attention")
        if return_all_attention_prob:
            all_attention_prob = {
                'before_spatial': probs["before_spatial"],
                'after_spatial': probs["after_spatial"],
                'perturbed_mask': attack_mask,
                'perturbed_attention': probs["perturbed_attention"],
                'calibrated_attention': probs["calibrated_attention"],
            }
            return (attacked_feedforward_output, calibrated_feedforward_output, attack_mask, combined_attention_prob,
                    all_attention_prob)
        return attacked_feedforward_output, calibrated_feedforward_output, attack_mask, combined_attention_prob

    def _forward_spatial_only(self, hidden_states, attention_mask, return_attention_prob, return_all_attention_prob, _rnd, _rows):
        if return_attention_prob or return_all_attention_prob:
            raise ValueError("adversarial=False: the spatial-only attention core has no probability dumps "
                             "(return_attention_prob / return_all_attention_prob need the adversarial calibrator)")
        att = self.attack_attention
        cal = att.calibrator_params()
        mq, mk, mv, hidden_res, extras = projections_qkv(
            hidden_states, att.query, att.key, att.value,
            spatial=(cal.get("w_order"), cal.get("b_order"), cal.get("w_dist"), cal.get("b_dist"), att.num_attention_heads))
        cfg = self._config()
        core_rnd = None
        if _rnd is not None:
            core_rnd = ExplicitRandomness(keep_after=getattr(_rnd, "keep_after", None))
        p_drop = att.attn_dropout_prob if (self.training or (core_rnd is not None and core_rnd.keep_after is not None)) else 0.0
        _, ctx_cal, _, _ = ops.calibrated_attention(
            mq, mk, mv, None, None, None, attention_mask, cfg, p_drop=p_drop, rnd=core_rnd,
            seed_tensor=state_of(self).seed_tensor if core_rnd is None else None, read_rows=_rows, attack_upstream=False,
            state=state_of(self), **extras, **cal)
        keep_out, keep_ffn = getattr(_rnd, "keep_out_cal", None), getattr(_rnd, "keep_ffn_cal", None)
        can_tail = ctx_cal.is_cuda and tail.supported(att, self.feed_forward)
        one_launch = can_tail and tail.fused_supported(att, self.feed_forward)
        if _rows is not None:
            index = _rows.unsqueeze(-1).expand(-1, -1, hidden_states.shape[-1])
            pick = lambda t: None if t is None else t.gather(1, index)
            if one_launch:
                out = tail.layer_tail(ctx_cal, hidden_res, att, self.feed_forward, pick(keep_out), pick(keep_ffn), pick=_rows)
                return None, out, None, None
            ctx_cal, hidden_res, keep_out, keep_ffn = pick(ctx_cal), pick(hidden_res), pick(keep_out), pick(keep_ffn)
        if one_launch or (can_tail and torch.is_grad_enabled()):
            out = tail.layer_tail(ctx_cal, hidden_res, att, self.feed_forward, keep_out, keep_ffn)
        else:
            out = self.feed_forward(att.output(ctx_cal, hidden_res, keep_out), keep_ffn)
        return None, out, None, None


class AttackRTransformerEncoder(nn.Module):

    def __init__(self, n_layers=2, n_heads=2, hidden_size=64, inner_size=256, hidden_dropout_prob=0.5,
                 attn_dropout_prob=0.5, hidden_act='gelu', layer_norm_eps=1e-12, combine_option='fixed', use_order=True,
                 use_distance=True, two_level=True, rich_calibrated_combine='fixed', seq_length=50, adversarial=True):
        super().__init__()
        self.adversarial = bool(adversarial)
        layer = AttackRTransformerLayer(
            n_heads, hidden_size, inner_size, hidden_dropout_prob, attn_dropout_prob, hidden_act, layer_norm_eps,
            combine_option, use_order=use_order, use_distance=use_distance, two_level=two_level,
            rich_calibrated_combine=rich_calibrated_combine, seq_length=seq_length, adversarial=adversarial)
        self.layer = nn.ModuleList([copy.deepcopy(layer) for _ in range(n_layers)])

    def forward(self, hidden_states, attention_mask, output_all_encoded_layers=True, return_attention_prob=False,
                return_all_attention_prob=False, _rnds: Optional[List] = None, _last_rows=None):
        if _last_rows is not None and output_all_encoded_layers:
            raise ValueError("_last_rows needs output_all_encoded_layers=False")
        all_encoder_layers = []
        attacked_hidden_states = None
        calibrated_hidden_states = None
        all_attack_masks = []
        all_attention_prob = [] if return_attention_prob else None
        all_probs = [] if return_all_attention_prob else None
        for layer_idx, layer_module in enumerate(self.layer):
            rnd = _rnds[layer_idx] if _rnds is not None else None
            need_attacked = output_all_encoded_layers or layer_idx == len(self.layer) - 1
            outs = layer_module(hidden_states, attention_mask, return_attention_prob, return_all_attention_prob,
                                _rnd=rnd, _need_attacked=need_attacked,
                                _attack_upstream=layer_idx > 0 or not state_of(self).prune_dead_work,
                                _rows=_last_rows if layer_idx == len(self.layer) - 1 else None)
            attacked_hidden_states, calibrated_hidden_states, attack_mask, combined_attention_prob = outs[:4]
            hidden_states = calibrated_hidden_states
            all_attack_masks.append(attack_mask)
            if output_all_encoded_layers:
                all_encoder_layers.append((attacked_hidden_states, calibrated_hidden_states))
            if return_attention_prob:
                all_attention_prob.append(combined_attention_prob)
            if return_all_attention_prob:
                all_probs.append(outs[4])
        if not output_all_encoded_layers:
            all_encoder_layers.append((attacked_hidden_states, calibrated_hidden_states))
        if return_all_attention_prob:
            return all_encoder_layers, all_attack_masks, all_probs
        if return_attention_prob:
            return all_encoder_layers, all_attack_masks, all_attention_prob
        return all_encoder_layers, all_attack_masks
```

### ac_tsr_amd/tail.py

```python
from __future__ import annotations

import ctypes as C

import torch
import torch.nn.functional as F

from . import _lib, fused_ln, ops
from .ops import _ptr, _stream
from .state import state_of

FUSED_KERNEL = True
FUSED_MAX_HIDDEN = 128


def _tail_problem(c, x, wd, bd, g1, b1, w1, bb1, w2, bb2, g2, b2, eps1, eps2, p1, p2, k1, k2, seed1, seed2, seed_t,
                  rows=None):
    p = _lib.TailProblem()
    H, I = wd.shape[0], w1.shape[0]
    p.rows, p.H, p.I = c.numel() // H, H, I
    if rows is not None:
        p.rows, p.src_index, p.src_R, p.src_L = rows.numel(), _ptr(rows), rows.shape[-1], c.shape[-2]
    p.ctx, p.x = _ptr(c), _ptr(x)
    p.wd, p.bd, p.g1, p.b1 = _ptr(wd), _ptr(bd), _ptr(g1), _ptr(b1)
    p.w1, p.bb1, p.w2, p.bb2, p.g2, p.b2 = _ptr(w1), _ptr(bb1), _ptr(w2), _ptr(bb2), _ptr(g2), _ptr(b2)
    p.eps1, p.eps2, p.p1, p.p2 = float(eps1), float(eps2), float(p1), float(p2)
    p.keep1, p.keep2 = _ptr(k1), _ptr(k2)
    p.seed1, p.seed2 = seed1 & 0xFFFFFFFFFFFFFFFF, seed2 & 0xFFFFFFFFFFFFFFFF
    p.seed_device = _ptr(seed_t)
    return p


class _FusedLayerTail(torch.autograd.Function):
    @staticmethod
    def forward(ctx, c, x, wd, bd, g1, b1, w1, bb1, w2, bb2, g2, b2, eps1, eps2, p1, p2, keep1, keep2, seed1, seed2,
                seed_tensor, state, pick=None):
        ctx.state = state
        c, x = c.contiguous(), x.contiguous()
        params = tuple(t.contiguous() for t in (wd, bd, g1, b1, w1, bb1, w2, bb2, g2, b2))
        k1 = None if keep1 is None else keep1.to(torch.uint8).contiguous()
        k2 = None if keep2 is None else keep2.to(torch.uint8).contiguous()
        H, I = c.shape[-1], w1.shape[0]
        if pick is not None:
            pick = pick.contiguous()
            assert c.dim() == 3 and x.shape == c.shape and pick.dtype == torch.int64 and pick.shape[0] == c.shape[0]
            out_shape = (*pick.shape, H)
        else:
            out_shape = c.shape
        rows = 1
        for d in out_shape[:-1]:
            rows *= d
        new = lambda *shape: torch.empty(*shape, device=c.device, dtype=torch.float32)
        h1, a, h3, out = (new(*out_shape) for _ in range(4))
        st1, st2, act = new(rows, 2), new(rows, 2), new(rows, I)
        dgelu = new(rows, I) if (H > 64 and any(ctx.needs_input_grad)) else None
        p = _tail_problem(c, x, *params, eps1, eps2, p1, p2, k1, k2, seed1, seed2, seed_tensor, pick)
        lib = _lib.load()
        planes = None
        nbytes = int(lib.acattn_layer_tail_split_bytes(H, I, rows))
        if nbytes > 0:
            planes = new(nbytes // 4)
            _lib.check(lib.acattn_layer_tail_split_weights(C.byref(p), _ptr(planes), _stream()), "layer_tail_split_weights")
            p.split_planes = _ptr(planes)
        sv = _lib.TailSaved()
        sv.h1, sv.st1, sv.a, sv.act, sv.h3, sv.st2, sv.out = (_ptr(t) for t in (h1, st1, a, act, h3, st2, out))
        sv.gelu_grad = _ptr(dgelu)
        _lib.check(lib.acattn_layer_tail_fwd(C.byref(p), C.byref(sv), _stream()), "layer_tail_fwd")
        empty = c.new_empty(0)
        ctx.save_for_backward(c, x, h1, st1, a, act, h3, st2, *params, k1 if k1 is not None else empty,
                              k2 if k2 is not None else empty, seed_tensor if seed_tensor is not None else empty,
                              pick if pick is not None else empty, dgelu if dgelu is not None else empty,
                              planes if planes is not None else empty)
        ctx.args = (eps1, eps2, p1, p2, k1 is not None, k2 is not None, seed1, seed2, seed_tensor is not None,
                    pick is not None)
        return out

    @staticmethod
    def backward(ctx, d_out):
        c, x, h1, st1, a, act, h3, st2 = ctx.saved_tensors[:8]
        params = ctx.saved_tensors[8:18]
        k1, k2, seed_t, pick, dgelu, planes = ctx.saved_tensors[18:]
        eps1, eps2, p1, p2, has_k1, has_k2, seed1, seed2, has_seed_t, has_pick = ctx.args
        k1, k2, seed_t = (k1 if has_k1 else None), (k2 if has_k2 else None), (seed_t if has_seed_t else None)
        pick = pick if has_pick else None
        want_params = not ctx.state.attack_pass_only
        need_c, need_x = ctx.needs_input_grad[0], ctx.needs_input_grad[1]
        lib = _lib.load()
        rows, H, I = act.shape[0], c.shape[-1], act.shape[-1]
        new = lambda *shape: torch.empty(*shape, device=c.device, dtype=torch.float32)
        d_out = d_out.contiguous()
        p = _tail_problem(c, x, *params, eps1, eps2, p1, p2, k1, k2, seed1, seed2, seed_t, pick)
        p.split_planes = _ptr(planes) if planes.numel() else None
        sv = _lib.TailSaved()
        sv.h1, sv.st1, sv.a, sv.act, sv.h3, sv.st2 = (_ptr(t) for t in (h1, st1, a, act, h3, st2))
        sv.gelu_grad = _ptr(dgelu) if dgelu.numel() else None
        io = _lib.TailBwdIO()
        if pick is not None and need_c and need_x:
            d_c, d_x = torch.zeros(2, *c.shape, device=c.device, dtype=c.dtype).unbind(0)
        else:
            alloc = torch.zeros_like if pick is not None else torch.empty_like
            d_c = alloc(c) if need_c else None
            d_x = alloc(x) if need_x else None
        io.d_out, io.d_ctx, io.d_x = _ptr(d_out), _ptr(d_c), _ptr(d_x)
        d_h1 = d_h2 = d_h3 = part = None
        if want_params:
            d_h1, d_h2, d_h3 = new(rows, H), new(rows, I), new(rows, H)
            part = new(int(lib.acattn_layer_tail_bwd_partial_rows_for(rows, H)), 4 * H)
            io.d_h1, io.d_h2, io.d_h3, io.dgb_part = _ptr(d_h1), _ptr(d_h2), _ptr(d_h3), _ptr(part)
        ws_bytes = int(lib.acattn_layer_tail_bwd_workspace_bytes(H, I))
        ws = new(ws_bytes // 4) if ws_bytes > 0 else None
        io.workspace = _ptr(ws)
        _lib.check(lib.acattn_layer_tail_bwd(C.byref(p), C.byref(sv), C.byref(io), _stream()), "layer_tail_bwd")
        grads = [None] * 10
        if want_params:
            two = lambda t: t.reshape(-1, t.shape[-1])
            c_rows = two(c) if pick is None else c.gather(1, pick.unsqueeze(-1).expand(-1, -1, H)).view(-1, H)
            (gwd, gbd), (gw1, gb1), (gw2, gb2) = ops.linear_wgrad_grouped(
                [(c_rows, d_h1, True), (two(a), d_h2, True), (act, d_h3, True)], ctx.state)
            gb = ops.sum_rows0(part, ctx.state).view(4, H)
            grads = [gwd, gbd, gb[0], gb[1], gw1, gb1, gw2, gb2, gb[2], gb[3]]
            ctx.state.watch(gb, grads[2], grads[3], grads[8], grads[9])
        return (d_c, d_x, *grads, None, None, None, None, None, None, None, None, None, None, None)



class _LayerTail(torch.autograd.Function):
    @staticmethod
    def forward(ctx, c, x, wd, bd, g1, b1, w1, bb1, w2, bb2, g2, b2, eps1, eps2, p1, p2, keep1, keep2, seed1, seed2,
                seed_tensor, state):
        ctx.state = state
        c, x = c.contiguous(), x.contiguous()
        k1 = None if keep1 is None else keep1.to(torch.uint8).contiguous()
        k2 = None if keep2 is None else keep2.to(torch.uint8).contiguous()
        h1 = F.linear(c, wd, bd)
        a, st1 = fused_ln.forward_raw(h1, x, g1, b1, eps1, p1, k1, seed1, seed_tensor)
        h2 = F.linear(a, w1, bb1)
        act = F.gelu(h2)
        h3 = F.linear(act, w2, bb2)
        out, st2 = fused_ln.forward_raw(h3, a, g2, b2, eps2, p2, k2, seed2, seed_tensor)
        empty = c.new_empty(0)
        ctx.save_for_backward(c, x, h1, st1, a, h2, act, h3, st2, wd, g1, b1, w1, w2, g2, b2,
                              k1 if k1 is not None else empty, k2 if k2 is not None else empty,
                              seed_tensor if seed_tensor is not None else empty)
        ctx.args = (eps1, eps2, p1, p2, k1 is not None, k2 is not None, seed1, seed2, seed_tensor is not None)
        return out

    @staticmethod
    def backward(ctx, d_out):
        (c, x, h1, st1, a, h2, act, h3, st2, wd, g1, b1, w1, w2, g2, b2, k1, k2, seed_t) = ctx.saved_tensors
        eps1, eps2, p1, p2, has_k1, has_k2, seed1, seed2, has_seed_t = ctx.args
        k1, k2, seed_t = (k1 if has_k1 else None), (k2 if has_k2 else None), (seed_t if has_seed_t else None)
        params = not ctx.state.attack_pass_only
        two = lambda t: t.reshape(-1, t.shape[-1])
        d_h3, d_a, part2 = fused_ln.backward_raw(h3, a, g2, b2, eps2, p2, k2, seed2, seed_t, st2, d_out, want_gb=params)
        d_act = two(d_h3) @ w2
        d_h2 = torch.ops.aten.gelu_backward(d_act.view_as(h2), h2)
        two(d_a).addmm_(two(d_h2), w1)
        need_c, need_x = ctx.needs_input_grad[0], ctx.needs_input_grad[1]
        d_h1, d_x, part1 = fused_ln.backward_raw(h1, x, g1, b1, eps1, p1, k1, seed1, seed_t, st1, d_a, want_dres=need_x,
                                                 want_gb=params)
        d_c = (two(d_h1) @ wd).view_as(c) if need_c else None
        grads = [None] * 10
        if params:
            (gwd, gbd), (gw1, gb1), (gw2, gb2) = ops.linear_wgrad_grouped(
                [(two(c), two(d_h1), True), (two(a), two(d_h2), True), (two(act), two(d_h3), True)], ctx.state)
            gb = ops.sum_rows(torch.stack((part1, part2)), 1)
            grads = [gwd, gbd, gb[0, 0], gb[0, 1], gw1, gb1, gw2, gb2, gb[1, 0], gb[1, 1]]
        return (d_c, d_x, *grads, None, None, None, None, None, None, None, None, None, None)


def supported(att, ffn) -> bool:
    return (ffn.intermediate_act_fn == ffn.gelu and fused_ln.supported(att.dense.out_features)
            and att.dense.bias is not None and ffn.dense_1.bias is not None and ffn.dense_2.bias is not None)


def fused_supported(att, ffn) -> bool:
    H = att.dense.out_features
    if H > FUSED_MAX_HIDDEN:
        return False
    return FUSED_KERNEL and bool(_lib.load().acattn_layer_tail_supported(H, ffn.dense_1.out_features))


def layer_tail(ctx_layer, input_tensor, att, ffn, keep_out=None, keep_ffn=None, pick=None):
    training = att.training
    p1 = att.out_dropout.p if (training or keep_out is not None) else 0.0
    p2 = ffn.dropout.p if (training or keep_ffn is not None) else 0.0
    state = state_of(att)
    seed1 = state.draw_seed() if (p1 > 0 and keep_out is None) else 0
    seed2 = state.draw_seed() if (p2 > 0 and keep_ffn is None) else 0
    seed_t = state.seed_tensor if (keep_out is None and keep_ffn is None) else None
    extra = ()
    node = _LayerTail
    if fused_supported(att, ffn):
        node, extra = _FusedLayerTail, (pick,)
    else:
        assert pick is None, "row selection inside the tail needs the fused node"
    return node.apply(ctx_layer, input_tensor, att.dense.weight, att.dense.bias, att.LayerNorm.weight,
                            att.LayerNorm.bias, ffn.dense_1.weight, ffn.dense_1.bias, ffn.dense_2.weight,
                            ffn.dense_2.bias, ffn.LayerNorm.weight, ffn.LayerNorm.bias, att.LayerNorm.eps,
                            ffn.LayerNorm.eps, p1, p2, keep_out, keep_ffn, seed1, seed2, seed_t, state, *extra)
```

### include/acattn.h

```cpp
#ifndef ACATTN_H_
#define ACATTN_H_

#include <stdint.h>

#ifdef __cplusplus
extern "C" {
#endif

#define ACATTN_ABI_VERSION 32

enum {
  ACATTN_MASK_STRUCTURED = 0,
  ACATTN_MASK_DENSE_LL = 1,
  ACATTN_MASK_DENSE_L = 2
};

enum { ACATTN_COMBINE_FIXED = 0, ACATTN_COMBINE_GATE = 1, ACATTN_COMBINE_ANNEALING = 2 };

enum { ACATTN_RICH_NONE = 0, ACATTN_RICH_FIXED = 1, ACATTN_RICH_TRAINABLE = 2 };

enum {
  ACATTN_RNG_EXPLICIT = 0,
  ACATTN_RNG_COUNTER = 1
};

#define ACATTN_NSTAT 8

typedef struct acattn_problem {
  int32_t B, L, H, n_heads;
  const float* q;
  const float* k;
  const float* v;
  const float* qa;
  const float* ka;
  const float* gate_logits;
  int32_t mask_mode;
  int32_t causal;
  const uint8_t* key_valid;
  const float* mask;
  const float* w_order;
  const float* b_order;
  const float* w_dist;
  const float* b_dist;
  const float* scalar;
  int32_t adversarial;
  int32_t combine_option;
  float anneal_rate;
  int32_t two_level;
  int32_t rich_combine;
  const float* rich_ratio;
  int32_t rng_mode;
  float p_drop;
  const float* noise;
  const uint8_t* keep_after;
  const uint8_t* keep_before;
  const uint8_t* keep_mask;
  uint64_t seed;
  const uint64_t* seed_device;
  const float* affine;
  int32_t gate_is_prob;
} acattn_problem;

typedef struct acattn_fwd_out {
  float* ctx_attacked;
  float* ctx_calibrated;
  float* attack_mask;
  float* row_stats;
  float* after_spatial;
  float* before_spatial;
  float* perturbed_attention;
  float* calibrated_attention;
  float* penalty_part;
} acattn_fwd_out;

typedef struct acattn_bwd_io {
  const float* attack_mask;
  const float* row_stats;
  const float* d_ctx_attacked;
  const float* d_ctx_calibrated;
  const float* d_attack_mask;
  float* dq;
  float* dk;
  float* dv;
  float* dqa;
  float* dka;
  float* dgate_logits;
  float* dw_order_part;
  float* dw_dist_part;
  float* dsmall_part;
  int32_t part_stride;
  const uint32_t* active_qblocks;
  int32_t attack_only;
  void* workspace;
  const int64_t* read_rows;
  int32_t n_read_rows;
  const float* d_penalty_part;
  int32_t dgate_summed;
  const float* d_ctx_calibrated2;
  const float* d_penalty_part2;
  float* dqa2;
  float* dka2;
} acattn_bwd_io;

typedef struct acattn_ce_problem {
  int32_t B, N, H;
  const float* out;
  const float* table;
  const int64_t* target;
  int32_t coef_is_scalar;
  float coef_scale;
} acattn_ce_problem;

int64_t acattn_full_sort_ce_workspace_bytes(const acattn_ce_problem* p);

int acattn_full_sort_ce_fwd(const acattn_ce_problem* p, void* workspace, float* lse, float* row_loss, void* stream);

int acattn_full_sort_ce_fwd_dir(const acattn_ce_problem* p, void* workspace, float* lse, float* row_loss, float* dir,
                                void* stream);

int acattn_full_sort_ce_bwd(const acattn_ce_problem* p, const float* lse, const float* coef, void* workspace,
                            float* d_out, float* d_table, void* stream);

#define ACATTN_CE_PRODUCTS_FP32 0
#define ACATTN_CE_PRODUCTS_DEFAULT 1
#define ACATTN_CE_PRODUCTS_ALL 2
int acattn_full_sort_ce_products(int mode);

#define ACATTN_LN_BWD_GRID 512
typedef struct acattn_ln_problem {
  int32_t rows, H;
  int32_t residual_rows;
  const float* z;
  const float* residual;
  const float* gamma;
  const float* beta;
  float eps;
  float p_drop;
  const uint8_t* keep;
  uint64_t seed;
  const uint64_t* seed_device;
} acattn_ln_problem;

int acattn_dropout_add_layernorm_fwd(const acattn_ln_problem* p, float* y, float* stats, void* stream);

int acattn_dropout_add_layernorm_bwd(const acattn_ln_problem* p, const float* dy, const float* stats, float* dz,
                                     float* dres, float* dgb_part, void* stream);

#define ACATTN_EMBED_BWD_CHUNKS 8
typedef struct acattn_embed_problem {
  int32_t rows, L, H;
  int64_t n_table_rows;
  const int64_t* idx;
  const float* table;
  const float* pos;
  const float* gamma;
  const float* beta;
  float eps;
  float p_drop;
  const uint8_t* keep;
  uint64_t seed;
  const uint64_t* seed_device;
  uint8_t* nonzero_out;
  int64_t hot_id_plus1;
} acattn_embed_problem;

int acattn_embed_layernorm_fwd(const acattn_embed_problem* p, float* y, float* stats, void* stream);

int acattn_embed_layernorm_bwd(const acattn_embed_problem* p, const float* dy, const float* stats, int64_t padding_idx,
                               float* d_table, float* d_pos_part, float* dgb_part, void* stream);

int acattn_sum_rows(const float* x, float* out, int32_t batch, int32_t R, int32_t C, void* stream);
int acattn_sum_rows_pair(const float* x1, float* out1, int32_t batch1, int32_t R1, int32_t C1, const float* x2, float* out2,
                         int32_t batch2, int32_t R2, int32_t C2, void* stream);

int acattn_dense_ce_fwd(const float* logits, int64_t rows, int64_t N, const int64_t* target, float* lse, float* row_loss,
                        void* stream);
int acattn_dense_ce_bwd(const float* logits, const float* lse, const int64_t* target, const float* coef, int64_t rows, int64_t N,
                        float* d_logits, void* stream);

#define ACATTN_MAX_COPIES 6
int acattn_step_inputs(const void* const* src, void* const* dst, const int64_t* bytes, int32_t n_copies, int64_t* counter,
                       const int64_t* item_length, int64_t* last_row, int32_t n_rows, void* stream);

#define ACATTN_PENALTY_WS_FLOATS 1024
int acattn_mask_penalty_fwd(const float* m, int64_t n, float* workspace, float* norm, void* stream);
int acattn_mask_penalty_bwd(const float* m, const float* norm, const float* d_norm, int64_t n, float* d_m, void* stream);

int acattn_mask_penalty_partial(const float* m, int64_t n, float* part, void* stream);
int acattn_attacked_loss_finish(const float* row_loss, int32_t B, const float* part, int32_t n_masks, int64_t mask_numel,
                                float weight, float* out, float* scale_buf, int32_t n_scale, void* stream);
int acattn_mask_penalty_bwd_scaled(const float* m, const float* norm, const float* d_loss, float scale, int64_t n, float* d_m,
                                   void* stream);
int acattn_mask_penalty_rows(const float* m, int32_t B, int32_t n_heads, int32_t L, float* pen, void* stream);
int acattn_attacked_loss_finish_rows(const float* row_loss, int32_t B, const float* const* pen, int32_t n_masks, int32_t count,
                                     float weight, float* out, float* scale_buf, int32_t n_scale, void* stream);
int acattn_mask_penalty_drows(const float* norms, const float* d_loss, float scale, int32_t count, float* const* d_pen,
                              int32_t n_masks, void* stream);
int acattn_mask_penalty_drows_dir(const float* norms, const float* d_loss, float scale, int32_t count, float* const* d_pen,
                                  int32_t n_masks, const float* direction, float* d_out, int32_t n_dir, void* stream);
#define ACATTN_MAX_MASKS 8
int acattn_mask_penalty_partial_multi(const float* const* m, int32_t n_masks, int64_t n, float* part, void* stream);
int acattn_mask_penalty_bwd_scaled_multi(const float* const* m, const float* norms, const float* d_loss, float scale, int64_t n,
                                         float* const* d_m, int32_t n_masks, void* stream);

int64_t acattn_linear_wgrad_workspace_bytes(int64_t M, int32_t K, int32_t N);
int acattn_linear_wgrad(const float* x, const float* dy, int64_t M, int32_t K, int32_t N, void* workspace, float* dw,
                        float* db, void* stream);

#define ACATTN_WGRAD_MAX_GROUP 8
int acattn_linear_wgrad_grouped(const float* const* x, const float* const* dy, const int32_t* K, const int32_t* N,
                                float* const* dw, float* const* db, int32_t n_items, int64_t M, void* workspace,
                                void* stream);

#define ACATTN_WGRAD_MAX_REDUCE 32
#define ACATTN_SUMROWS_MAX_DEFER 8
int acattn_linear_wgrad_grouped_partial(const float* const* x, const float* const* dy, const int32_t* K, const int32_t* N,
                                        const int32_t* want_bias, int32_t n_items, int64_t M, void* workspace, int32_t* n_partials,
                                        int64_t* w_offset, int64_t* b_offset, void* stream);
int acattn_linear_wgrad_reduce_many(const float* const* part_w, const float* const* part_b, const int32_t* K, const int32_t* N,
                                    const int32_t* n_partials, float* const* dw, float* const* db, int32_t n_items,
                                    const float* const* sum_x, float* const* sum_out, const int32_t* sum_R, const int32_t* sum_C,
                                    int32_t n_sums, void* stream);

typedef struct acattn_tail_problem {
  int32_t rows, H, I;
  const float* ctx;
  const float* x;
  const float* wd;
  const float* bd;
  const float* g1;
  const float* b1;
  const float* w1;
  const float* bb1;
  const float* w2;
  const float* bb2;
  const float* g2;
  const float* b2;
  float eps1, eps2;
  float p1, p2;
  const uint8_t* keep1;
  const uint8_t* keep2;
  uint64_t seed1, seed2;
  const uint64_t* seed_device;
  const int64_t* src_index;
  int32_t src_R, src_L;
  const void* split_planes;
} acattn_tail_problem;

typedef struct acattn_tail_saved {
  float* h1;
  float* st1;
  float* a;
  float* act;
  float* h3;
  float* st2;
  float* out;
  float* gelu_grad;
} acattn_tail_saved;

typedef struct acattn_tail_bwd_io {
  const float* d_out;
  float* d_ctx;
  float* d_x;
  float* d_h1;
  float* d_h2;
  float* d_h3;
  float* dgb_part;
  void* workspace;
} acattn_tail_bwd_io;

int acattn_layer_tail_supported(int32_t H, int32_t I);
int acattn_layer_tail_fwd(const acattn_tail_problem* p, const acattn_tail_saved* saved, void* stream);
int acattn_layer_tail_bwd(const acattn_tail_problem* p, const acattn_tail_saved* saved, const acattn_tail_bwd_io* io,
                          void* stream);
int32_t acattn_layer_tail_bwd_partial_rows(int32_t rows);
int32_t acattn_layer_tail_bwd_partial_rows_for(int32_t rows, int32_t H);
int64_t acattn_layer_tail_bwd_workspace_bytes(int32_t H, int32_t I);
int acattn_select_layer_tail_blocks(int nb);
int64_t acattn_layer_tail_split_bytes(int32_t H, int32_t I, int32_t rows);
int acattn_layer_tail_split_weights(const acattn_tail_problem* p, void* planes, void* stream);

typedef struct acattn_proj_problem {
  int32_t rows, H, G;
  const float* x;
  const float *wq, *bq;
  const float *wk, *bk;
  const float *wv, *bv;
  const float *waq, *baq;
  const float *wak, *bak;
  const float *wg, *bg;
  const float *w_order, *b_order, *w_dist, *b_dist;
  int32_t n_heads, L;
} acattn_proj_problem;

typedef struct acattn_proj_out {
  float *mq, *mk, *mv, *qa, *ka;
  float* gate;
  float* affine;
  int32_t gate_prob;
} acattn_proj_out;

typedef struct acattn_proj_bwd_io {
  const float *dmq, *dmk, *dmv, *dqa, *dka;
  const float* dgate;
  float *dmq_total, *dmk_total, *dx;
  const float* dx_init;
  void* workspace;
} acattn_proj_bwd_io;

int acattn_projections_supported(int32_t H, int32_t G);
int64_t acattn_projections_bwd_workspace_bytes(const acattn_proj_problem* p);
int acattn_projections_fwd(const acattn_proj_problem* p, const acattn_proj_out* out, void* stream);
int acattn_projections_bwd(const acattn_proj_problem* p, const acattn_proj_bwd_io* io, void* stream);
int acattn_projections_qkv_supported(int32_t H);
int acattn_projections_qkv_fwd(const acattn_proj_problem* p, const acattn_proj_out* out, void* stream);

#define ACATTN_LINEAR_PRODUCTS_FP32 0
#define ACATTN_LINEAR_PRODUCTS_DEFAULT 1
int acattn_linear_products(int mode);

#define ACATTN_ADAM_MAX_TENSORS 64
typedef struct acattn_adam_group {
  int32_t n_tensors;
  float* param[ACATTN_ADAM_MAX_TENSORS];
  const float* grad[ACATTN_ADAM_MAX_TENSORS];
  float* exp_avg[ACATTN_ADAM_MAX_TENSORS];
  float* exp_avg_sq[ACATTN_ADAM_MAX_TENSORS];
  float* step[ACATTN_ADAM_MAX_TENSORS];
  int64_t numel[ACATTN_ADAM_MAX_TENSORS];
} acattn_adam_group;
int acattn_adam_step(const acattn_adam_group* g, double lr, double beta1, double beta2, double eps, double weight_decay,
                     int32_t* done, void* stream);

int acattn_calibrated_attention_bwd_gate_summed(const acattn_problem* p, const acattn_bwd_io* io);
int acattn_calibrated_attention_bwd_pair_supported(const acattn_problem* p, const acattn_bwd_io* io);

int acattn_abi_version(void);

const char* acattn_last_error(void);

int64_t acattn_fwd_algorithmic_bytes(const acattn_problem* p);

int acattn_calibrated_attention_fwd(const acattn_problem* p, const acattn_fwd_out* out, void* stream);

int acattn_spatial_affines(const acattn_problem* p, float* affine, void* stream);

int acattn_calibrated_attention_bwd(const acattn_problem* p, const acattn_bwd_io* io, void* stream);

int64_t acattn_calibrated_attention_bwd_workspace_bytes(const acattn_problem* p);

typedef struct acattn_spatial_bwd_io {
  const float* d_ctx;
  float* dq;
  float* dk;
  float* dv;
  float* dw_order_part;
  float* dw_dist_part;
  float* dsmall_part;
  int32_t part_stride;
  int32_t n_read_rows;
  const int64_t* read_rows;
  void* workspace;
} acattn_spatial_bwd_io;
int acattn_spatial_attention_bwd(const acattn_problem* p, const acattn_spatial_bwd_io* io, void* stream);
int64_t acattn_spatial_attention_bwd_workspace_bytes(const acattn_problem* p);

int acattn_rng_materialize(int32_t B, int32_t n_heads, int32_t L, uint64_t seed, float p_drop, float* noise,
                           uint8_t* keep_after, uint8_t* keep_mask, uint8_t* keep_before, void* stream);

enum {
  ACATTN_FWD_AUTO = 0,
  ACATTN_FWD_STREAM = 1,
  ACATTN_FWD_STAGED = 2,
  ACATTN_FWD_GENERAL = 3
};
int acattn_select_forward_kernel(int which);

enum {
  ACATTN_BWD_AUTO = 0,
  ACATTN_BWD_STREAM = 1,
  ACATTN_BWD_ROW = 2
};
int acattn_select_backward_kernel(int which);

#ifdef __cplusplus
}
#endif
#endif
```

Before: 472,000 user-sequences/sec.

## Fold gradient zero-fills into tail and one-row attention backward kernels; share split weight planes

The tail backward kernel now writes zeros into the unpicked rows of d_ctx/d_x itself and stores the picked row directly, so the separate torch.zeros allocation and fill can be skipped. The one-row attention backward gets a per-sequence mode where one block runs all heads as separate waves, sums dgate across heads in LDS and writes the full dgate_logits slab, removing a separate zero launch and the atomic-style accumulation. Split weight planes are cached and reused between the adversarial and clean tail branches of a layer, so the split-weights launch runs once. The cost is extra kernel-side store work, more LDS per block, and a wider block. All of this sits behind an ACATTN_FOLD env switch that defaults on.

```diff
diff --git a/ac_tsr_amd/_lib.py b/ac_tsr_amd/_lib.py
--- a/ac_tsr_amd/_lib.py
+++ b/ac_tsr_amd/_lib.py
@@ -9,7 +9,7 @@
 LIB_PATH = os.environ.get("ACATTN_LIB") or os.path.join(CSRC, "libacattn.so")
 HEADER_PATH = os.path.join(os.path.dirname(_HERE), "include", "acattn.h")
 
-ABI_VERSION = 32
+ABI_VERSION = 33
 MAX_MASKS = 8
 NSTAT = 8
 MASK_STRUCTURED, MASK_DENSE_LL, MASK_DENSE_L = 0, 1, 2
@@ -118,7 +118,7 @@
 
 class TailBwdIO(C.Structure):
     _fields_ = [("d_out", _f), ("d_ctx", _f), ("d_x", _f), ("d_h1", _f), ("d_h2", _f), ("d_h3", _f), ("dgb_part", _f),
-                ("workspace", _f)]
+                ("workspace", _f), ("fill_unpicked", C.c_int32)]
 
 
 class EmbedProblem(C.Structure):
@@ -163,6 +163,7 @@
     "acattn_layer_tail_supported": (C.c_int, [C.c_int32, C.c_int32]),
     "acattn_layer_tail_fwd": (C.c_int, [C.POINTER(TailProblem), C.POINTER(TailSaved), C.c_void_p]),
     "acattn_layer_tail_bwd": (C.c_int, [C.POINTER(TailProblem), C.POINTER(TailSaved), C.POINTER(TailBwdIO), C.c_void_p]),
+    "acattn_layer_tail_bwd_fills": (C.c_int, [C.c_int32, C.c_int32, C.c_int32, C.c_int32]),
     "acattn_layer_tail_bwd_partial_rows": (C.c_int32, [C.c_int32]),
     "acattn_layer_tail_bwd_partial_rows_for": (C.c_int32, [C.c_int32, C.c_int32]),
     "acattn_layer_tail_bwd_workspace_bytes": (C.c_int64, [C.c_int32, C.c_int32]),
diff --git a/ac_tsr_amd/csrc/acattn_api.hip b/ac_tsr_amd/csrc/acattn_api.hip
--- a/ac_tsr_amd/csrc/acattn_api.hip
+++ b/ac_tsr_amd/csrc/acattn_api.hip
@@ -309,6 +309,9 @@
 
 int32_t acattn_layer_tail_bwd_partial_rows(int32_t rows) { return acattn_tail_bwd_partial_rows(rows); }
 int32_t acattn_layer_tail_bwd_partial_rows_for(int32_t rows, int32_t H) { return acattn_tail_bwd_partial_rows_h(rows, H); }
+int acattn_layer_tail_bwd_fills(int32_t H, int32_t I, int32_t rows, int32_t src_R) {
+  return acattn_tail_bwd_fills(H, I, rows, src_R) ? 1 : 0;
+}
 int64_t acattn_layer_tail_bwd_workspace_bytes(int32_t H, int32_t I) {
   return acattn_tail_supported(H, I) ? acattn_tail_bwd_ws_bytes(H, I) : -1;
 }
diff --git a/ac_tsr_amd/csrc/acattn_bwd_stream.hip b/ac_tsr_amd/csrc/acattn_bwd_stream.hip
--- a/ac_tsr_amd/csrc/acattn_bwd_stream.hip
+++ b/ac_tsr_amd/csrc/acattn_bwd_stream.hip
@@ -868,21 +868,35 @@
 #define OR_STAMP(k)
 #endif
 
+constexpr int kOneRowHeads = 4;
+template <int DH>
+constexpr int onerow_lds_floats() { return 8 * DH + 4 * 256 + 256; }
+
 template <int DH, bool ACC, bool SLICED>
-__global__ void __launch_bounds__(64) acattn_bwd_onerow_kernel(const acattn_problem P, const acattn_bwd_io IO) {
+__global__ void __launch_bounds__(64 * kOneRowHeads) acattn_bwd_onerow_kernel(const acattn_problem P, const acattn_bwd_io IO) {
 #ifdef ACATTN_ONEROW_STAMPS
   unsigned long long cyc_[8] = {}, last_ = 0;
 #endif
   OR_STAMP(-1);
   constexpr int D4 = DH / 4;
-  __shared__ __attribute__((aligned(16))) float vec[8][DH];
-  __shared__ __attribute__((aligned(16))) float col[4][256];
+  extern __shared__ __attribute__((aligned(16))) float onerow_lds[];
+  const bool per_seq = IO.dgate_summed == 2;
+  const int wave = __builtin_amdgcn_readfirstlane(threadIdx.x >> 6);
+  float* const lds = onerow_lds + wave * onerow_lds_floats<DH>();
+  float(*const vec)[DH] = (float(*)[DH])lds;
+  float(*const col)[256] = (float(*)[256])(lds + 8 * DH);
+  float* const dgl_row = lds + 8 * DH + 4 * 256;
   const int L = P.L, H = P.H, nh = P.n_heads;
   const int nT = (L + 15) >> 4;
   const bool causal = P.causal != 0;
   int b, h;
-  decode_block(blockIdx.x, P.B, nh, b, h);
-  const int lane = threadIdx.x;
+  if (per_seq) {
+    b = blockIdx.x;
+    h = wave;
+  } else {
+    decode_block(blockIdx.x, P.B, nh, b, h);
+  }
+  const int lane = threadIdx.x & 63;
   const size_t rowbase = (size_t)b * L, bh = (size_t)b * nh + h;
   const int hoff = h * DH;
   const int i = min(max((int)IO.read_rows[b], 0), L - 1);
@@ -1070,7 +1084,19 @@
     __builtin_amdgcn_sched_barrier(0);
   }
   OR_STAMP(3);
-  if (IO.dgate_logits && IO.dgate_summed) {
+  if (IO.dgate_logits && IO.dgate_summed && per_seq) {
+    if (slice == 0 && j0 < 256) *(f4*)(dgl_row + j0) = dgl;
+    __syncthreads();
+    float* gbase = IO.dgate_logits + (size_t)b * L * L;
+    for (int row = wave; row < L; row += nh) {
+      for (int j = lane; j < L; j += 64) {
+        float v = 0.f;
+        if (row == i)
+          for (int hh = 0; hh < nh; ++hh) v += onerow_lds[hh * onerow_lds_floats<DH>() + 8 * DH + 4 * 256 + j];
+        gbase[(size_t)row * L + j] = v;
+      }
+    }
+  } else if (IO.dgate_logits && IO.dgate_summed) {
     if (slice == 0) {
       float* grow = IO.dgate_logits + ((size_t)b * L + i) * L;
 #pragma unroll
@@ -1167,20 +1193,25 @@
 
 template <int DH>
 int launch_onerow(const acattn_problem& p, const acattn_bwd_io& io, bool accumulate, hipStream_t stream) {
-  const dim3 grid(p.B * p.n_heads), block(64);
-  if (io.dgate_logits && io.dgate_summed) {
+  const bool summed = io.dgate_logits && io.dgate_summed;
+  const bool per_seq = summed && p.n_heads <= kOneRowHeads && acattn_fold_enabled();
+  if (summed && !per_seq) {
     const int rc = acattn_launch_zero(io.dgate_logits, (size_t)p.B * p.L * p.L, stream);
     if (rc) return rc;
   }
+  const dim3 grid(per_seq ? p.B : p.B * p.n_heads), block(per_seq ? 64 * p.n_heads : 64);
+  const size_t lds = (size_t)(per_seq ? p.n_heads : 1) * onerow_lds_floats<DH>() * sizeof(float);
+  acattn_bwd_io kio = io;
+  kio.dgate_summed = summed ? (per_seq ? 2 : 1) : 0;
   if (p.L <= 64) {
     if (accumulate)
-      hipLaunchKernelGGL((acattn_bwd_onerow_kernel<DH, true, true>), grid, block, 0, stream, p, io);
+      hipLaunchKernelGGL((acattn_bwd_onerow_kernel<DH, true, true>), grid, block, lds, stream, p, kio);
     else
-      hipLaunchKernelGGL((acattn_bwd_onerow_kernel<DH, false, true>), grid, block, 0, stream, p, io);
+      hipLaunchKernelGGL((acattn_bwd_onerow_kernel<DH, false, true>), grid, block, lds, stream, p, kio);
   } else if (accumulate) {
-    hipLaunchKernelGGL((acattn_bwd_onerow_kernel<DH, true, false>), grid, block, 0, stream, p, io);
+    hipLaunchKernelGGL((acattn_bwd_onerow_kernel<DH, true, false>), grid, block, lds, stream, p, kio);
   } else {
-    hipLaunchKernelGGL((acattn_bwd_onerow_kernel<DH, false, false>), grid, block, 0, stream, p, io);
+    hipLaunchKernelGGL((acattn_bwd_onerow_kernel<DH, false, false>), grid, block, lds, stream, p, kio);
   }
   return (int)hipGetLastError();
 }
diff --git a/ac_tsr_amd/csrc/acattn_common.h b/ac_tsr_amd/csrc/acattn_common.h
--- a/ac_tsr_amd/csrc/acattn_common.h
+++ b/ac_tsr_amd/csrc/acattn_common.h
@@ -289,6 +289,7 @@
 bool acattn_tail_supported(int H, int I);
 int acattn_tail_bwd_partial_rows(int rows);
 int acattn_tail_bwd_partial_rows_h(int rows, int H);
+bool acattn_tail_bwd_fills(int H, int I, int rows, int src_R);
 int64_t acattn_tail_bwd_ws_bytes(int H, int I);
 int acattn_select_tail_nb(int nb);
 int64_t acattn_tail_split_bytes(int H, int I, int rows);
@@ -322,6 +323,7 @@
                                      float* d_m, hipStream_t stream);
 int acattn_launch_penalty_bwd(const float* m, const float* norm, const float* d_norm, int64_t n, float* d_m,
                               hipStream_t stream);
+bool acattn_fold_enabled();
 int acattn_launch_zero(float* p, size_t n, hipStream_t stream);
 int64_t acattn_ce6_rows_bytes(const acattn_ce_problem& p);
 int acattn_launch_ce6_sweep(const acattn_ce_problem& p, const float* lse, const float* coef, float* slab, float* d_table,
diff --git a/ac_tsr_amd/csrc/acattn_tail.hip b/ac_tsr_amd/csrc/acattn_tail.hip
--- a/ac_tsr_amd/csrc/acattn_tail.hip
+++ b/ac_tsr_amd/csrc/acattn_tail.hip
@@ -323,6 +323,27 @@
   }
 }
 
+template <int H>
+__device__ __forceinline__ bool fills_unpicked(const acattn_tail_problem& P, const acattn_tail_bwd_io& IO) {
+  return IO.fill_unpicked && P.src_index && P.src_R == 1;
+}
+template <int H>
+__device__ __forceinline__ void fill_unpicked_rows(const acattn_tail_problem& P, const acattn_tail_bwd_io& IO, int first, int count) {
+  constexpr int Q = H / 4;
+  const int n_piece = P.src_L * Q, n_threads = blockDim.x, last = min(first + count, P.rows);
+  const f4 z4 = {0.f, 0.f, 0.f, 0.f};
+  for (int s = first; s < last; ++s) {
+    const int pick = min(max((int)P.src_index[s], 0), P.src_L - 1);
+    f4* const dc = IO.d_ctx ? (f4*)(IO.d_ctx + (size_t)s * P.src_L * H) : nullptr;
+    f4* const dx = IO.d_x ? (f4*)(IO.d_x + (size_t)s * P.src_L * H) : nullptr;
+    for (int q = threadIdx.x; q < n_piece; q += n_threads) {
+      if (q / Q == pick) continue;
+      if (dc) dc[q] = z4;
+      if (dx) dx[q] = z4;
+    }
+  }
+}
+
 template <int H, int I, int NB, int NW = 1>
 __global__ void __launch_bounds__(64 * NW) tail_bwd_kernel(const acattn_tail_problem P, const acattn_tail_saved S,
                                                            const acattn_tail_bwd_io IO) {
@@ -333,6 +354,9 @@
   const Rows<NB> W = wave_rows<NB>(P);
   const uint64_t step = P.seed_device ? *P.seed_device : 0ull;
   float* part = IO.dgb_part ? IO.dgb_part + (size_t)blockIdx.x * 4 * H : nullptr;
+  const bool fill = fills_unpicked<H>(P, IO);
+  const bool add_rows = P.src_index != nullptr && !fill;
+  if (fill) fill_unpicked_rows<H>(P, IO, blockIdx.x * 16 * NB, 16 * NB);
 
   f4 a[NB][DT], dh3[NB][DT], da[NB][DT];
   {
@@ -447,7 +471,7 @@
         const size_t o = (size_t)W.row[nb] * H + 16 * t + 4 * g;
         dh1[nb][t] = dz[t] * keep[t];
         if (W.ok[nb]) {
-          if (IO.d_x) store_grad(IO.d_x + (size_t)W.src[nb] * H + 16 * t + 4 * g, dz[t], P.src_index != nullptr);
+          if (IO.d_x) store_grad(IO.d_x + (size_t)W.src[nb] * H + 16 * t + 4 * g, dz[t], add_rows);
           if (IO.d_h1) *(f4*)(IO.d_h1 + o) = dh1[nb][t];
         }
       }
@@ -482,7 +506,7 @@
     for (int nb = 0; nb < NB; ++nb)
       if (W.ok[nb])
 #pragma unroll
-        for (int nt = 0; nt < DT; ++nt) store_grad(IO.d_ctx + (size_t)W.src[nb] * H + 16 * nt + 4 * g, dc[nb][nt], P.src_index != nullptr);
+        for (int nt = 0; nt < DT; ++nt) store_grad(IO.d_ctx + (size_t)W.src[nb] * H + 16 * nt + 4 * g, dc[nb][nt], add_rows);
   }
 }
 
@@ -719,6 +743,9 @@
   const Rows<NB> W = wave_rows<NB>(P);
   const uint64_t step = P.seed_device ? *P.seed_device : 0ull;
   float* part = IO.dgb_part ? IO.dgb_part + (size_t)blockIdx.x * 4 * H : nullptr;
+  const bool fill = fills_unpicked<H>(P, IO);
+  const bool add_rows = P.src_index != nullptr && !fill;
+  if (fill) fill_unpicked_rows<H>(P, IO, blockIdx.x * 16 * NB, 16 * NB);
   const b8* planes = (const b8*)P.split_planes;
   const b8 *pw1 = planes + L::FWD_1, *pw1t = planes + L::BWD_1, *pw2t = planes + L::BWD_2;
 
@@ -853,7 +880,7 @@
         const size_t o = (size_t)W.row[nb] * H + 16 * t + 4 * g;
         dh1[nb][t] = dz[t] * keep[t];
         if (W.ok[nb]) {
-          if (IO.d_x) store_grad(IO.d_x + (size_t)W.src[nb] * H + 16 * t + 4 * g, dz[t], P.src_index != nullptr);
+          if (IO.d_x) store_grad(IO.d_x + (size_t)W.src[nb] * H + 16 * t + 4 * g, dz[t], add_rows);
           if (IO.d_h1) *(f4*)(IO.d_h1 + o) = dh1[nb][t];
         }
       }
@@ -876,7 +903,7 @@
     for (int nb = 0; nb < NB; ++nb)
       if (W.ok[nb])
 #pragma unroll
-        for (int nt = 0; nt < DT; ++nt) store_grad(IO.d_ctx + (size_t)W.src[nb] * H + 16 * nt + 4 * g, dc[nb][nt], P.src_index != nullptr);
+        for (int nt = 0; nt < DT; ++nt) store_grad(IO.d_ctx + (size_t)W.src[nb] * H + 16 * nt + 4 * g, dc[nb][nt], add_rows);
   }
 }
 
@@ -1924,6 +1951,10 @@
   return (H == 64 && (I == 256 || I == 128)) || (H == 128 && (I == 512 || I == 256)) || (H == 256 && I == 1024);
 }
 
+bool acattn_tail_bwd_fills(int H, int I, int rows, int src_R) {
+  return acattn_fold_enabled() && acattn_tail_supported(H, I) && H == 64 && rows > 0 && src_R == 1 && !staged64(rows);
+}
+
 int acattn_tail_bwd_partial_rows(int rows) { return (rows + rows_per_wave(rows) - 1) / rows_per_wave(rows); }
 int acattn_tail_bwd_partial_rows_h(int rows, int H) {
   return (H > 64 || staged64(rows)) ? (rows + 15) / 16 : acattn_tail_bwd_partial_rows(rows);
@@ -1960,6 +1991,10 @@
 
 int acattn_launch_tail_bwd(const acattn_tail_problem& p, const acattn_tail_saved& s, const acattn_tail_bwd_io& io,
                            hipStream_t stream) {
+  if (io.fill_unpicked && p.src_index && !acattn_tail_bwd_fills(p.H, p.I, p.rows, p.src_R)) {
+    acattn_set_error("layer tail backward: fill_unpicked is not honoured for this problem (ask acattn_layer_tail_bwd_fills)");
+    return -1;
+  }
   if (p.H == 64 && p.I == 256) return launch_bwd<64, 256>(p, s, io, stream);
   if (p.H == 64 && p.I == 128) return launch_bwd<64, 128>(p, s, io, stream);
   if (p.H == 128 && p.I == 512) return launch_wide_bwd<128, 512>(p, s, io, stream);
diff --git a/ac_tsr_amd/csrc/acattn_util.hip b/ac_tsr_amd/csrc/acattn_util.hip
--- a/ac_tsr_amd/csrc/acattn_util.hip
+++ b/ac_tsr_amd/csrc/acattn_util.hip
@@ -505,6 +505,11 @@
   return (int)hipGetLastError();
 }
 
+bool acattn_fold_enabled() {
+  static const bool on = getenv("ACATTN_FOLD") ? atoi(getenv("ACATTN_FOLD")) != 0 : true;
+  return on;
+}
+
 int acattn_launch_zero(float* p, size_t n, hipStream_t stream) {
   if (n == 0) return 0;
   static const bool use_memset = getenv("ACATTN_ZERO_MEMSET") && atoi(getenv("ACATTN_ZERO_MEMSET")) != 0;
diff --git a/ac_tsr_amd/layers.py b/ac_tsr_amd/layers.py
--- a/ac_tsr_amd/layers.py
+++ b/ac_tsr_amd/layers.py
@@ -180,15 +180,18 @@
         else:
             pick = lambda t: t
 
+        planes = []
+
         def branch(ctx_layer, keep_out, keep_ffn):
             one_launch = ctx_layer.is_cuda and tail.supported(att, self.feed_forward) and tail.fused_supported(att, self.feed_forward)
             fused = one_launch or (ctx_layer.is_cuda and torch.is_grad_enabled() and tail.supported(att, self.feed_forward))
             if one_launch and _rows is not None:
                 return tail.layer_tail(ctx_layer, hidden_res, att, self.feed_forward, pick(keep_out), pick(keep_ffn),
-                                       pick=_rows)
+                                       pick=_rows, shared_planes=planes)
             ctx_layer, keep_out, keep_ffn = pick(ctx_layer), pick(keep_out), pick(keep_ffn)
             if fused:
-                return tail.layer_tail(ctx_layer, residual, att, self.feed_forward, keep_out, keep_ffn)
+                return tail.layer_tail(ctx_layer, residual, att, self.feed_forward, keep_out, keep_ffn,
+                                       shared_planes=planes if one_launch else None)
             return self.feed_forward(att.output(ctx_layer, residual, keep_out), keep_ffn)
 
         attacked_feedforward_output = None
diff --git a/ac_tsr_amd/tail.py b/ac_tsr_amd/tail.py
--- a/ac_tsr_amd/tail.py
+++ b/ac_tsr_amd/tail.py
@@ -5,7 +5,7 @@
 import torch
 import torch.nn.functional as F
 
-from . import _lib, fused_ln, ops
+from . import _lib, attn_launch, fused_ln, ops
 from .ops import _ptr, _stream
 from .state import state_of
 
@@ -33,7 +33,7 @@
 class _FusedLayerTail(torch.autograd.Function):
     @staticmethod
     def forward(ctx, c, x, wd, bd, g1, b1, w1, bb1, w2, bb2, g2, b2, eps1, eps2, p1, p2, keep1, keep2, seed1, seed2,
-                seed_tensor, state, pick=None):
+                seed_tensor, state, pick=None, shared_planes=None):
         ctx.state = state
         c, x = c.contiguous(), x.contiguous()
         params = tuple(t.contiguous() for t in (wd, bd, g1, b1, w1, bb1, w2, bb2, g2, b2))
@@ -58,8 +58,14 @@
         planes = None
         nbytes = int(lib.acattn_layer_tail_split_bytes(H, I, rows))
         if nbytes > 0:
-            planes = new(nbytes // 4)
-            _lib.check(lib.acattn_layer_tail_split_weights(C.byref(p), _ptr(planes), _stream()), "layer_tail_split_weights")
+            weights = tuple((t.data_ptr(), t._version) for t in (params[0], params[4], params[6]))
+            if shared_planes and shared_planes[0][0] == (weights, nbytes, c.device):
+                planes = shared_planes[0][1]
+            else:
+                planes = new(nbytes // 4)
+                _lib.check(lib.acattn_layer_tail_split_weights(C.byref(p), _ptr(planes), _stream()), "layer_tail_split_weights")
+                if shared_planes is not None:
+                    shared_planes[:] = [((weights, nbytes, c.device), planes)]
             p.split_planes = _ptr(planes)
         sv = _lib.TailSaved()
         sv.h1, sv.st1, sv.a, sv.act, sv.h3, sv.st2, sv.out = (_ptr(t) for t in (h1, st1, a, act, h3, st2, out))
@@ -94,13 +100,17 @@
         sv.h1, sv.st1, sv.a, sv.act, sv.h3, sv.st2 = (_ptr(t) for t in (h1, st1, a, act, h3, st2))
         sv.gelu_grad = _ptr(dgelu) if dgelu.numel() else None
         io = _lib.TailBwdIO()
-        if pick is not None and need_c and need_x:
+        fills = pick is not None and bool(lib.acattn_layer_tail_bwd_fills(H, I, rows, pick.shape[-1]))
+        if fills or pick is None:
+            unwritten = attn_launch.allocator(c, attn_launch.POISON)
+            d_c = unwritten(*c.shape) if need_c else None
+            d_x = unwritten(*x.shape) if need_x else None
+        elif need_c and need_x:
             d_c, d_x = torch.zeros(2, *c.shape, device=c.device, dtype=c.dtype).unbind(0)
         else:
-            alloc = torch.zeros_like if pick is not None else torch.empty_like
-            d_c = alloc(c) if need_c else None
-            d_x = alloc(x) if need_x else None
-        io.d_out, io.d_ctx, io.d_x = _ptr(d_out), _ptr(d_c), _ptr(d_x)
+            d_c = torch.zeros_like(c) if need_c else None
+            d_x = torch.zeros_like(x) if need_x else None
+        io.d_out, io.d_ctx, io.d_x, io.fill_unpicked = _ptr(d_out), _ptr(d_c), _ptr(d_x), int(fills)
         d_h1 = d_h2 = d_h3 = part = None
         if want_params:
             d_h1, d_h2, d_h3 = new(rows, H), new(rows, I), new(rows, H)
@@ -119,7 +129,7 @@
             gb = ops.sum_rows0(part, ctx.state).view(4, H)
             grads = [gwd, gbd, gb[0], gb[1], gw1, gb1, gw2, gb2, gb[2], gb[3]]
             ctx.state.watch(gb, grads[2], grads[3], grads[8], grads[9])
-        return (d_c, d_x, *grads, None, None, None, None, None, None, None, None, None, None, None)
+        return (d_c, d_x, *grads, None, None, None, None, None, None, None, None, None, None, None, None)
 
 
 
@@ -180,7 +190,7 @@
     return FUSED_KERNEL and bool(_lib.load().acattn_layer_tail_supported(H, ffn.dense_1.out_features))
 
 
-def layer_tail(ctx_layer, input_tensor, att, ffn, keep_out=None, keep_ffn=None, pick=None):
+def layer_tail(ctx_layer, input_tensor, att, ffn, keep_out=None, keep_ffn=None, pick=None, shared_planes=None):
     training = att.training
     p1 = att.out_dropout.p if (training or keep_out is not None) else 0.0
     p2 = ffn.dropout.p if (training or keep_ffn is not None) else 0.0
@@ -191,7 +201,7 @@
     extra = ()
     node = _LayerTail
     if fused_supported(att, ffn):
-        node, extra = _FusedLayerTail, (pick,)
+        node, extra = _FusedLayerTail, (pick, shared_planes)
     else:
         assert pick is None, "row selection inside the tail needs the fused node"
     return node.apply(ctx_layer, input_tensor, att.dense.weight, att.dense.bias, att.LayerNorm.weight,
diff --git a/include/acattn.h b/include/acattn.h
--- a/include/acattn.h
+++ b/include/acattn.h
@@ -7,7 +7,7 @@
 extern "C" {
 #endif
 
-#define ACATTN_ABI_VERSION 32
+#define ACATTN_ABI_VERSION 33
 
 enum {
   ACATTN_MASK_STRUCTURED = 0,
@@ -267,12 +267,14 @@
   float* d_h3;
   float* dgb_part;
   void* workspace;
+  int32_t fill_unpicked;
 } acattn_tail_bwd_io;
 
 int acattn_layer_tail_supported(int32_t H, int32_t I);
 int acattn_layer_tail_fwd(const acattn_tail_problem* p, const acattn_tail_saved* saved, void* stream);
 int acattn_layer_tail_bwd(const acattn_tail_problem* p, const acattn_tail_saved* saved, const acattn_tail_bwd_io* io,
                           void* stream);
+int acattn_layer_tail_bwd_fills(int32_t H, int32_t I, int32_t rows, int32_t src_R);
 int32_t acattn_layer_tail_bwd_partial_rows(int32_t rows);
 int32_t acattn_layer_tail_bwd_partial_rows_for(int32_t rows, int32_t H);
 int64_t acattn_layer_tail_bwd_workspace_bytes(int32_t H, int32_t I);
```

Result: no change. 470,600 user-sequences/sec (-0.3%).
